# catree/InvCompCamTrack

Hardware: NVIDIA B200
Metric: GN pixel-residuals/s (higher is better)
Workload: dtype f32

## Files before the change

### __graft_entry__.py

```python
import os
import sys

ROOT = os.path.dirname(os.path.abspath(__file__))
if ROOT not in sys.path:
    sys.path.insert(0, ROOT)


def build():
    from invcompcamtrack_b200 import build as b
    b.build_library(force=bool(os.environ.get("ICT_FORCE_BUILD")))
    b.build_drivers()
    from oracle import oracle as O
    O.build("oracle")
    if os.path.isdir("/root/reference"):
        O.build("ref")
    import invcompcamtrack_b200 as ict
    ict.lib()


def smoke():
    import numpy as np
    import invcompcamtrack_b200 as ict
    sys.path.insert(0, os.path.join(ROOT, "tests"))
    from helpers import make_case, oracle_run, gpu_run, check_parity
    from oracle import oracle as O
    if ict.device_count() < 1:
        raise RuntimeError("smoke(): no CUDA device (libictrack has no CPU fallback)")
    ict.lib().ict_set_device(0)
    case = make_case(seed=7, w=320, h=240, psz=8, npts=100, lv_f=2)
    g = gpu_run(ict, case, sum_order=None)
    o = oracle_run(O.OracleLib(), case)
    for k in range(3):
        assert np.array_equal(g["pyr"][0][k], o["pyr"][0][k]), "pyramid differs from the oracle"
    assert np.array_equal(g["pt2d"], o["pt2d"]), "reference reprojection differs from the oracle"
    from helpers import assert_bit_identical
    assert_bit_identical(g, o)
    res = check_parity(g, o, case, min_same_iters=1.0, min_trans_ok=1.0)
    err = float(np.abs(g["p_out"][0] - case["p_gt"]).max())
    assert err < 5e-3, "tracker did not recover the ground-truth motion: %g" % err
    print("smoke ok:", res, "iters", g["iters"][0].tolist(), "err_vs_gt %.2e" % err, "launches", ict.launch_count())
    case32 = make_case(seed=8, w=640, h=384, psz=32, npts=4, lv_f=2, ntracks=8)
    o32 = oracle_run(O.OracleLib(), case32, trace_cap=40)
    gx = gpu_run(ict, case32, trace_cap=40, sum_order=None)
    assert_bit_identical(gx, o32)
    g32 = gpu_run(ict, case32, trace_cap=40, sum_order=0)
    r32 = check_parity(g32, o32, case32, gates=False)
    assert r32["jtr_first"] <= 1e-5, r32
    print("smoke psz32 ok: default kernel (K2r, reference order) bit-identical to the oracle on %d tracks; fast mode "
          "(K2v2) J^T r on identical inputs within %.1e of sum|sd*r| (gate 1e-5), %.0f%% identical iteration counts"
          % (case32["T"], r32["jtr_first"], 100 * r32["frac_same"]))


if __name__ == "__main__":
    build()
    if "--smoke" in sys.argv:
        smoke()
```

### invcompcamtrack_b200/build.py

```python
import os
import subprocess
import sys

HERE = os.path.dirname(os.path.abspath(__file__))
CSRC = os.path.join(HERE, "csrc")
LIB = os.path.join(HERE, "libictrack.so")
NVCC = os.environ.get("NVCC", "/usr/local/cuda/bin/nvcc")
NVCC_FLAGS = ["-gencode", "arch=compute_100a,code=sm_100a", "-lineinfo", "-O3", "-fmad=false", "-std=c++17",
              "-Xcompiler", "-fPIC", "-ccbin", "g++"] + os.environ.get("ICT_EXTRA_NVCC", "").split()
LIB_SOURCES = ["ict_kernels.cu", "ict_kernel_v2.cu", "ict_kernel_v8.cu", "ict_kernel_x.cu", "ict_kernel_x8.cu", "ict_kernel_r.cu", "ict_kernels_big.cu", "ict_hypotheses.cu", "ict_capi.cu"]
LIB_DEPS = LIB_SOURCES + ["ict_kernels.cuh", "ict_device.cuh", "ict_kernel_v2.cuh", "ict_kernel_v8.cuh", "ict_kernel_x.cuh", "ict_knobs.h", os.path.join("..", "..", "include", "ictrack.h")]


def _stale(target, deps):
    if not os.path.exists(target):
        return True
    t = os.path.getmtime(target)
    return any(os.path.getmtime(d) > t for d in deps if os.path.exists(d))


def build_library(force=False, verbose=False):
    deps = [os.path.join(CSRC, d) for d in LIB_DEPS]
    if not force and not _stale(LIB, deps):
        return LIB
    headers = [d for d in deps if not d.endswith(".cu")]
    objdir = os.path.join(HERE, "build")
    os.makedirs(objdir, exist_ok=True)
    jobs = []
    for src in LIB_SOURCES:
        obj = os.path.join(objdir, src.replace(".cu", ".o"))
        if force or _stale(obj, [os.path.join(CSRC, src)] + headers):
            cmd = [NVCC] + NVCC_FLAGS + (["-Xptxas=-v"] if verbose else []) + ["-c", os.path.join(CSRC, src), "-o", obj]
            jobs.append(cmd)
    if jobs:
        from concurrent.futures import ThreadPoolExecutor
        with ThreadPoolExecutor(max_workers=min(len(jobs), os.cpu_count() or 1)) as ex:
            for r in ex.map(lambda c: subprocess.run(c, capture_output=not verbose, text=True), jobs):
                if r.returncode:
                    raise RuntimeError("nvcc failed:\n%s\n%s" % (" ".join(r.args), (r.stderr or "")[-4000:]))
    objs = [os.path.join(objdir, src.replace(".cu", ".o")) for src in LIB_SOURCES]
    subprocess.run([NVCC, "-gencode", "arch=compute_100a,code=sm_100a", "-shared", "-o", LIB] + objs, check=True)
    return LIB


def build_drivers(force=False):
    host = os.path.join(CSRC, "host")
    out = []
    for name in ("run_track", "run_track_nposes"):
        src = os.path.join(host, name + ".cpp")
        if not os.path.exists(src):
            continue
        exe = os.path.join(HERE, "bin", name)
        deps = [src] + [os.path.join(host, f) for f in os.listdir(host)] + [LIB]
        if force or _stale(exe, deps):
            os.makedirs(os.path.dirname(exe), exist_ok=True)
            srcs = [src] + [os.path.join(host, f) for f in ("camera.cpp", "pose.cpp", "odometer.cpp", "utilities.cpp")]
            subprocess.run(["g++", "-O2", "-std=c++14", "-I", host, "-I", os.path.join(HERE, "..", "include"), "-o", exe]
                           + srcs + ["-L", HERE, "-lictrack", "-Wl,-rpath," + HERE, "-Wl,-rpath,$ORIGIN/.."], check=True)
        out.append(exe)
    return out


if __name__ == "__main__":
    force = "--force" in sys.argv
    print(build_library(force=force, verbose="-v" in sys.argv))
    for e in build_drivers(force=force):
        print(e)
```

### invcompcamtrack_b200/csrc/ict_capi.cu

```cuda
#include "ict_kernels.cuh"

#include <cuda.h>
#include <math.h>
#include <stdio.h>
#include <stdlib.h>
#include <string.h>
#include <string>
#include <vector>

using namespace ict;

static thread_local std::string g_err;
static int fail(int code, const std::string& msg) {
  g_err = msg;
  return code;
}
#define CU(expr)                                                                                       \
  do {                                                                                                 \
    cudaError_t _e = (expr);                                                                           \
    if (_e != cudaSuccess)                                                                             \
      return fail(ICT_ERR_CUDA, std::string(#expr) + ": " + cudaGetErrorString(_e));                   \
  } while (0)

static int require_device() {
  int n = 0;
  cudaError_t e = cudaGetDeviceCount(&n);
  if (e != cudaSuccess || n <= 0) {
    cudaGetLastError();
    return fail(ICT_ERR_NO_DEVICE, "no CUDA device: libictrack has no CPU fallback");
  }
  return ICT_OK;
}

struct DevBuf {
  void* p = nullptr;
  size_t cap = 0;
  cudaError_t reserve(size_t bytes) {
    if (bytes <= cap) return cudaSuccess;
    if (p) cudaFree(p);
    p = nullptr;
    cap = 0;
    cudaError_t e = cudaMalloc(&p, bytes);
    if (e == cudaSuccess) cap = bytes;
    return e;
  }
  void release() {
    if (p) cudaFree(p);
    p = nullptr;
    cap = 0;
  }
  template <typename T> T* as() const { return (T*)p; }
};

struct CopyLane {
  cudaStream_t s = nullptr;
  cudaEvent_t copied = nullptr, consumed = nullptr;
  bool have_consumed = false;
  cudaError_t begin() {
    cudaError_t e = cudaSuccess;
    if (!s) {
      e = cudaStreamCreateWithFlags(&s, cudaStreamNonBlocking);
      if (e == cudaSuccess) e = cudaEventCreateWithFlags(&copied, cudaEventDisableTiming);
      if (e == cudaSuccess) e = cudaEventCreateWithFlags(&consumed, cudaEventDisableTiming);
      if (e != cudaSuccess) return e;
    }
    if (have_consumed) e = cudaStreamWaitEvent(s, consumed, 0);
    return e;
  }
  cudaError_t publish(cudaStream_t user) {
    cudaError_t e = cudaEventRecord(copied, s);
    if (e == cudaSuccess) e = cudaStreamWaitEvent(user, copied, 0);
    return e;
  }
  cudaError_t done(cudaStream_t user) {
    if (!s) return cudaSuccess;
    cudaError_t e = cudaEventRecord(consumed, user);
    have_consumed = e == cudaSuccess;
    return e;
  }
  void release() {
    if (s) {
      cudaStreamSynchronize(s);
      cudaEventDestroy(copied);
      cudaEventDestroy(consumed);
      cudaStreamDestroy(s);
      s = nullptr;
    }
  }
};

extern "C" {

void ict_optparam_init(ict_optparam* op, int lv_f, int lv_l, int psz, int maxiter, float normdp_ratio, int donorm,
                       int dopatchnorm, int maxpttrack, int verbosity) {
  memset(op, 0, sizeof(*op));
  op->lv_f = lv_f;
  op->lv_l = lv_l;
  op->psz = psz;
  op->pszd2 = psz / 2;
  op->pszd2m3 = psz + op->pszd2 - 1;
  op->novals = psz * psz;
  op->maxiter = maxiter;
  op->normdp_ratio = normdp_ratio;
  op->donorm = donorm ? 1 : 0;
  op->dopatchnorm = dopatchnorm ? 1 : 0;
  const int r = maxpttrack % 4;
  op->maxpttrack = r > 0 ? maxpttrack + (4 - r) : maxpttrack;
  op->verbosity = verbosity;
}

int ict_version(void) { return ICT_VERSION; }
const char* ict_last_error(void) { return g_err.c_str(); }

int ict_device_count(void) {
  int n = 0;
  if (cudaGetDeviceCount(&n) != cudaSuccess) {
    cudaGetLastError();
    return 0;
  }
  return n;
}

int ict_set_device(int dev) {
  if (require_device()) return ICT_ERR_NO_DEVICE;
  CU(cudaSetDevice(dev));
  return ICT_OK;
}

int64_t ict_launch_count(int reset) { return launch_count(reset); }

int ict_camera_levels(int noscales, const float fc[2], const float cc[2], const int wh[2], int padding,
                      float* out) {
  if (noscales < 1 || noscales > ICT_MAX_LEVELS) return fail(ICT_ERR_BAD_ARG, "noscales out of range");
  for (int i = 0; i < noscales; ++i) {
    const float sc_fct = (float)(1 / pow(2, i));
    float* o = out + 8 * i;
    o[0] = sc_fct * fc[0];
    o[1] = sc_fct * fc[1];
    o[2] = sc_fct * cc[0];
    o[3] = sc_fct * cc[1];
    o[4] = sc_fct * (float)wh[0];
    o[5] = sc_fct * (float)wh[1];
    o[6] = o[4] + 2 * padding;
    o[7] = o[5] + 2 * padding;
  }
  return ICT_OK;
}

static void fill_cam(CamLevels& cam, int noscales, const float fc[2], const float cc[2], const int wh[2],
                     int padding) {
  float lv[8 * ICT_MAX_LEVELS];
  ict_camera_levels(noscales, fc, cc, wh, padding, lv);
  memset(&cam, 0, sizeof(cam));
  for (int l = 0; l < noscales; ++l) {
    cam.fx[l] = lv[8 * l + 0];
    cam.fy[l] = lv[8 * l + 1];
    cam.cx[l] = lv[8 * l + 2];
    cam.cy[l] = lv[8 * l + 3];
    cam.swo[l] = lv[8 * l + 4];
    cam.sho[l] = lv[8 * l + 5];
    cam.width[l] = (int)lv[8 * l + 6];
  }
}

int64_t ict_pyramid_layout(int w, int h, int lv_f, int pad, int64_t* level_off, int* sw, int* sh) {
  if (w <= 0 || h <= 0 || lv_f < 0 || lv_f >= ICT_MAX_LEVELS || pad < 0) return -1;
  if ((w % (1 << lv_f)) || (h % (1 << lv_f))) return -1;
  int64_t tot = 0;
  for (int l = 0; l <= lv_f; ++l) {
    const int a = (w >> l) + 2 * pad, b = (h >> l) + 2 * pad;
    if (level_off) level_off[l] = tot;
    if (sw) sw[l] = a;
    if (sh) sh[l] = b;
    tot += (int64_t)a * b;
  }
  return tot;
}

struct ict_frames {
  int nframes, w, h, lv_f, pad;
  int64_t plane_floats;
  int64_t level_off[ICT_MAX_LEVELS];
  int sw[ICT_MAX_LEVELS], sh[ICT_MAX_LEVELS];
  float *I, *dx, *dy;
  FrameDesc* desc;
  void* tmaps;
  bool tma_ok;
  DevBuf stage;
  CopyLane lane;
  bool view;
};

typedef CUresult (*ict_encode_tiled_fn)(CUtensorMap*, CUtensorMapDataType, cuuint32_t, void*, const cuuint64_t*,
                                        const cuuint64_t*, const cuuint32_t*, const cuuint32_t*, CUtensorMapInterleave,
                                        CUtensorMapSwizzle, CUtensorMapL2promotion, CUtensorMapFloatOOBfill);
static ict_encode_tiled_fn encode_tiled_fn() {
  static ict_encode_tiled_fn fn = nullptr;
  static bool tried = false;
  if (!tried) {
    tried = true;
    void* p = nullptr;
    cudaDriverEntryPointQueryResult qres;
    if (cudaGetDriverEntryPoint("cuTensorMapEncodeTiled", &p, cudaEnableDefault, &qres) == cudaSuccess &&
        qres == cudaDriverEntryPointSuccess)
      fn = (ict_encode_tiled_fn)p;
    else
      cudaGetLastError();
  }
  return fn;
}

#define ICT_TMA_BOX_W 40
#define ICT_TMA_BOX_H 17

static bool frames_make_tmaps(ict_frames* fs) {
  fs->tmaps = nullptr;
  fs->tma_ok = false;
  if (fs->pad != 32) return false;
  ict_encode_tiled_fn enc = encode_tiled_fn();
  if (!enc) return false;
  for (int l = 0; l <= fs->lv_f; ++l)
    if ((fs->sw[l] % 4) || (fs->level_off[l] % 4) || fs->sw[l] < ICT_TMA_BOX_W || fs->sh[l] < ICT_TMA_BOX_H) return false;
  if (fs->plane_floats % 4) return false;
  const size_t per_frame = 3 * ICT_MAX_LEVELS;
  std::vector<CUtensorMap> maps(per_frame * fs->nframes);
  memset(maps.data(), 0, sizeof(CUtensorMap) * maps.size());
  float* planes[3] = {fs->I, fs->dx, fs->dy};
  for (int f = 0; f < fs->nframes; ++f)
    for (int q = 0; q < 3; ++q)
      for (int l = 0; l <= fs->lv_f; ++l) {
        void* base = planes[q] + (size_t)f * fs->plane_floats + fs->level_off[l];
        const cuuint64_t dims[2] = {(cuuint64_t)fs->sw[l], (cuuint64_t)fs->sh[l]};
        const cuuint64_t strides[1] = {(cuuint64_t)fs->sw[l] * sizeof(float)};
        const cuuint32_t box[2] = {ICT_TMA_BOX_W, ICT_TMA_BOX_H};
        const cuuint32_t estr[2] = {1, 1};
        if (enc(&maps[(f * 3 + q) * ICT_MAX_LEVELS + l], CU_TENSOR_MAP_DATA_TYPE_FLOAT32, 2, base, dims, strides, box, estr,
                CU_TENSOR_MAP_INTERLEAVE_NONE, CU_TENSOR_MAP_SWIZZLE_NONE, CU_TENSOR_MAP_L2_PROMOTION_NONE,
                CU_TENSOR_MAP_FLOAT_OOB_FILL_NONE) != CUDA_SUCCESS)
          return false;
      }
  if (cudaMalloc(&fs->tmaps, sizeof(CUtensorMap) * maps.size()) != cudaSuccess) {
    cudaGetLastError();
    fs->tmaps = nullptr;
    return false;
  }
  if (cudaMemcpy(fs->tmaps, maps.data(), sizeof(CUtensorMap) * maps.size(), cudaMemcpyHostToDevice) != cudaSuccess) {
    cudaFree(fs->tmaps);
    fs->tmaps = nullptr;
    return false;
  }
  fs->tma_ok = true;
  return true;
}

ict_frames* ict_frames_create(int nframes, int w, int h, int lv_f, int pad) {
  if (require_device()) return nullptr;
  ict_frames* fs = new ict_frames();
  fs->nframes = nframes; fs->w = w; fs->h = h; fs->lv_f = lv_f; fs->pad = pad;
  fs->I = fs->dx = fs->dy = nullptr;
  fs->desc = nullptr;
  fs->tmaps = nullptr;
  fs->tma_ok = false;
  fs->view = false;
  fs->plane_floats = ict_pyramid_layout(w, h, lv_f, pad, fs->level_off, fs->sw, fs->sh);
  if (fs->plane_floats < 0 || nframes <= 0) {
    fail(ICT_ERR_BAD_ARG, "ict_frames_create: w,h must be divisible by 2^lv_f, nframes > 0");
    delete fs;
    return nullptr;
  }
  const size_t bytes = sizeof(float) * (size_t)fs->plane_floats * nframes;
  if (cudaMalloc(&fs->I, bytes) != cudaSuccess || cudaMalloc(&fs->dx, bytes) != cudaSuccess ||
      cudaMalloc(&fs->dy, bytes) != cudaSuccess || cudaMalloc(&fs->desc, sizeof(FrameDesc) * nframes) != cudaSuccess) {
    fail(ICT_ERR_NOMEM, "ict_frames_create: cudaMalloc failed");
    cudaGetLastError();
    ict_frames_destroy(fs);
    return nullptr;
  }
  frames_make_tmaps(fs);
  std::vector<FrameDesc> d(nframes);
  for (int f = 0; f < nframes; ++f) {
    memset(&d[f], 0, sizeof(FrameDesc));
    d[f].tmap = fs->tmaps ? (const char*)fs->tmaps + sizeof(CUtensorMap) * 3 * ICT_MAX_LEVELS * (size_t)f : nullptr;
    for (int l = 0; l <= lv_f; ++l) {
      d[f].I[l] = fs->I + (size_t)f * fs->plane_floats + fs->level_off[l];
      d[f].dx[l] = fs->dx + (size_t)f * fs->plane_floats + fs->level_off[l];
      d[f].dy[l] = fs->dy + (size_t)f * fs->plane_floats + fs->level_off[l];
    }
  }
  if (cudaMemcpy(fs->desc, d.data(), sizeof(FrameDesc) * nframes, cudaMemcpyHostToDevice) != cudaSuccess) {
    fail(ICT_ERR_CUDA, "ict_frames_create: descriptor upload failed");
    ict_frames_destroy(fs);
    return nullptr;
  }
  return fs;
}

void ict_frames_destroy(ict_frames* fs) {
  if (!fs) return;
  if (fs->I) cudaFree(fs->I);
  if (fs->dx) cudaFree(fs->dx);
  if (fs->dy) cudaFree(fs->dy);
  if (fs->desc) cudaFree(fs->desc);
  if (fs->tmaps) cudaFree(fs->tmaps);
  fs->stage.release();
  fs->lane.release();
  delete fs;
}

ict_frames* ict_frames_create_view(int nframes, int w, int h, int lv_f, int pad) {
  if (require_device()) return nullptr;
  ict_frames* fs = new ict_frames();
  fs->nframes = nframes; fs->w = w; fs->h = h; fs->lv_f = lv_f; fs->pad = pad;
  fs->I = fs->dx = fs->dy = nullptr;
  fs->desc = nullptr;
  fs->tmaps = nullptr;
  fs->tma_ok = true;
  fs->view = true;
  fs->plane_floats = ict_pyramid_layout(w, h, lv_f, pad, fs->level_off, fs->sw, fs->sh);
  if (fs->plane_floats < 0 || nframes <= 0 || cudaMalloc(&fs->desc, sizeof(FrameDesc) * nframes) != cudaSuccess) {
    fail(ICT_ERR_BAD_ARG, "ict_frames_create_view: bad geometry or allocation failure");
    cudaGetLastError();
    delete fs;
    return nullptr;
  }
  cudaMemset(fs->desc, 0, sizeof(FrameDesc) * nframes);
  return fs;
}

int ict_frames_alias(ict_frames* view, int idx, const ict_frames* src, int src_idx) {
  if (!view || !src || !view->view) return fail(ICT_ERR_BAD_ARG, "ict_frames_alias: first argument must be a view store");
  if (idx < 0 || idx >= view->nframes || src_idx < 0 || src_idx >= src->nframes)
    return fail(ICT_ERR_BAD_ARG, "ict_frames_alias: index out of range");
  if (view->w != src->w || view->h != src->h || view->lv_f != src->lv_f || view->pad != src->pad)
    return fail(ICT_ERR_BAD_ARG, "ict_frames_alias: geometry mismatch");
  CU(cudaMemcpyAsync(view->desc + idx, src->desc + src_idx, sizeof(FrameDesc), cudaMemcpyDeviceToDevice, 0));
  view->tma_ok = view->tma_ok && src->tma_ok;
  return ICT_OK;
}

static int frames_range_ok(const ict_frames* fs, int first, int count) {
  if (!fs) return fail(ICT_ERR_BAD_ARG, "null frame store");
  if (first < 0 || count < 0 || first + count > fs->nframes) return fail(ICT_ERR_BAD_ARG, "frame range out of bounds");
  return ICT_OK;
}

static int frames_build(ict_frames* fs, int first, int count, const float* f32, const unsigned char* u8,
                        cudaStream_t st) {
  if (fs->view) return fail(ICT_ERR_BAD_ARG, "a view store owns no pixels: build into the store it aliases");
  CU(launch_pyramid(f32, u8, count, fs->w, fs->h, fs->lv_f, fs->pad, fs->I + (size_t)first * fs->plane_floats,
                    fs->dx + (size_t)first * fs->plane_floats, fs->dy + (size_t)first * fs->plane_floats,
                    fs->plane_floats, fs->level_off, st));
  return ICT_OK;
}

int ict_frames_build_dev(ict_frames* fs, int first, int count, const float* imgs_dev, void* stream) {
  if (frames_range_ok(fs, first, count)) return ICT_ERR_BAD_ARG;
  return frames_build(fs, first, count, imgs_dev, nullptr, (cudaStream_t)stream);
}
int ict_frames_build_dev_u8(ict_frames* fs, int first, int count, const unsigned char* imgs_dev, void* stream) {
  if (frames_range_ok(fs, first, count)) return ICT_ERR_BAD_ARG;
  return frames_build(fs, first, count, nullptr, imgs_dev, (cudaStream_t)stream);
}

int ict_frames_upload(ict_frames* fs, int first, int count, const float* imgs) {
  if (frames_range_ok(fs, first, count)) return ICT_ERR_BAD_ARG;
  const size_t bytes = sizeof(float) * (size_t)fs->w * fs->h * count;
  CU(fs->stage.reserve(bytes));
  CU(cudaMemcpyAsync(fs->stage.p, imgs, bytes, cudaMemcpyHostToDevice, 0));
  return frames_build(fs, first, count, fs->stage.as<float>(), nullptr, 0);
}
int ict_frames_upload_u8(ict_frames* fs, int first, int count, const unsigned char* imgs) {
  if (frames_range_ok(fs, first, count)) return ICT_ERR_BAD_ARG;
  const size_t bytes = (size_t)fs->w * fs->h * count;
  CU(fs->stage.reserve(bytes));
  CU(cudaMemcpyAsync(fs->stage.p, imgs, bytes, cudaMemcpyHostToDevice, 0));
  return frames_build(fs, first, count, nullptr, fs->stage.as<unsigned char>(), 0);
}

int ict_frames_upload_planes(ict_frames* fs, int frame, const float* I, const float* dx, const float* dy) {
  if (frames_range_ok(fs, frame, 1)) return ICT_ERR_BAD_ARG;
  if (fs->view || !I) return fail(ICT_ERR_BAD_ARG, "ict_frames_upload_planes: needs an owning store and an intensity plane set");
  const size_t bytes = sizeof(float) * (size_t)fs->plane_floats, o = (size_t)frame * fs->plane_floats;
  CU(cudaMemcpyAsync(fs->I + o, I, bytes, cudaMemcpyHostToDevice, 0));
  if (dx) CU(cudaMemcpyAsync(fs->dx + o, dx, bytes, cudaMemcpyHostToDevice, 0));
  if (dy) CU(cudaMemcpyAsync(fs->dy + o, dy, bytes, cudaMemcpyHostToDevice, 0));
  CU(cudaStreamSynchronize(0));
  return ICT_OK;
}

int ict_frames_upload_u8_stream(ict_frames* fs, int first, int count, const unsigned char* imgs, void* stream) {
  if (frames_range_ok(fs, first, count)) return ICT_ERR_BAD_ARG;
  cudaStream_t st = (cudaStream_t)stream;
  const size_t per = (size_t)fs->w * fs->h;
  if (fs->stage.cap < per * fs->nframes) {
    CU(cudaDeviceSynchronize());
    CU(fs->stage.reserve(per * fs->nframes));
  }
  unsigned char* dst = fs->stage.as<unsigned char>() + per * first;
  CU(fs->lane.begin());
  CU(cudaMemcpyAsync(dst, imgs, per * count, cudaMemcpyHostToDevice, fs->lane.s));
  CU(fs->lane.publish(st));
  const int rc = frames_build(fs, first, count, nullptr, dst, st);
  if (rc) return rc;
  CU(fs->lane.done(st));
  return ICT_OK;
}

int ict_frames_download(ict_frames* fs, int frame, float* out_I, float* out_dx, float* out_dy) {
  if (frames_range_ok(fs, frame, 1)) return ICT_ERR_BAD_ARG;
  if (fs->view) return fail(ICT_ERR_BAD_ARG, "ict_frames_download: a view store owns no pixels");
  const size_t bytes = sizeof(float) * (size_t)fs->plane_floats, o = (size_t)frame * fs->plane_floats;
  if (out_I) CU(cudaMemcpy(out_I, fs->I + o, bytes, cudaMemcpyDeviceToHost));
  if (out_dx) CU(cudaMemcpy(out_dx, fs->dx + o, bytes, cudaMemcpyDeviceToHost));
  if (out_dy) CU(cudaMemcpy(out_dy, fs->dy + o, bytes, cudaMemcpyDeviceToHost));
  return ICT_OK;
}

int ict_pyramid_build(const float* img, int w, int h, int lv_f, int pad, float* out_I, float* out_dx,
                      float* out_dy) {
  if (require_device()) return ICT_ERR_NO_DEVICE;
  ict_frames* fs = ict_frames_create(1, w, h, lv_f, pad);
  if (!fs) return ICT_ERR_BAD_ARG;
  int rc = ict_frames_upload(fs, 0, 1, img);
  if (rc == ICT_OK) rc = ict_frames_download(fs, 0, out_I, out_dx, out_dy);
  ict_frames_destroy(fs);
  return rc;
}

struct ict_tracker {
  ict_optparam op;
  CamLevels cam;
  float fc[2], cc[2];
  int wh[2];
  int T = 0;
  int64_t total = 0;
  int max_pts = 0;
  std::vector<int64_t> h_off;
  bool have_2d = false;
  int sum_mode = 1;
  int eigen_packet = 4;
  int force_general = 0;
  int knob_no_k2r = 0, knob_seq_launches = 0;
  unsigned robust = 0;
  int keep_state = 0;
  bool state_valid = false;
  int seq_n = 0, seq_step = 0;
  const int *big_rf = nullptr, *big_nf = nullptr;
  DevBuf pt_off, pts, pt3d, norm, p_in, p_out, iters, npix, trace, pt2d, rf, nf, big, teacher, state;
  int teacher_cap = 0;
  static const int ICT_BIG_LANES = 4;
  cudaStream_t big_st[ICT_BIG_LANES] = {};
  cudaEvent_t big_ev[ICT_BIG_LANES + 1] = {};
  DevBuf big_lane[ICT_BIG_LANES];
  CopyLane lane;
  CopyLane lane_in;
};

static bool optparam_ok(const ict_optparam* op) {
  return op && op->psz >= 1 && op->lv_f >= op->lv_l && op->lv_l >= 0 && op->lv_f < ICT_MAX_LEVELS && op->maxpttrack >= 1 &&
         op->maxiter >= 0;
}

ict_tracker* ict_tracker_create(const ict_optparam* op, const float fc[2], const float cc[2], const int wh[2]) {
  if (require_device()) return nullptr;
  if (!optparam_ok(op) || !fc || !cc || !wh) {
    fail(ICT_ERR_BAD_ARG, "ict_tracker_create: bad optparam");
    return nullptr;
  }
  ict_tracker* tr = new ict_tracker();
  tr->op = *op;
  memcpy(tr->fc, fc, sizeof(tr->fc));
  memcpy(tr->cc, cc, sizeof(tr->cc));
  memcpy(tr->wh, wh, sizeof(tr->wh));
  fill_cam(tr->cam, op->lv_f + 1, fc, cc, wh, op->psz);
  return tr;
}

void ict_tracker_destroy(ict_tracker* tr) {
  if (!tr) return;
  DevBuf* b[] = {&tr->pt_off, &tr->pts, &tr->pt3d, &tr->norm, &tr->p_in, &tr->p_out, &tr->iters,
                 &tr->npix, &tr->trace, &tr->pt2d, &tr->rf, &tr->nf, &tr->big, &tr->teacher, &tr->state};
  for (DevBuf* x : b) x->release();
  for (int k = 0; k < ict_tracker::ICT_BIG_LANES; ++k) {
    tr->big_lane[k].release();
    if (tr->big_st[k]) cudaStreamDestroy(tr->big_st[k]);
  }
  for (int k = 0; k <= ict_tracker::ICT_BIG_LANES; ++k)
    if (tr->big_ev[k]) cudaEventDestroy(tr->big_ev[k]);
  tr->lane.release();
  tr->lane_in.release();
  delete tr;
}

int ict_tracker_set_optparam(ict_tracker* tr, const ict_optparam* op) {
  if (!tr || !op) return fail(ICT_ERR_BAD_ARG, "null argument");
  if (op->psz != tr->op.psz || op->lv_f != tr->op.lv_f)
    return fail(ICT_ERR_BAD_ARG, "psz and lv_f are fixed at creation (they size the camera and the pyramids)");
  if (!optparam_ok(op)) return fail(ICT_ERR_BAD_ARG, "ict_tracker_set_optparam: bad optparam (lv_l, maxpttrack or maxiter out of range)");
  tr->op = *op;
  tr->op.pszd2 = op->psz / 2;
  tr->op.pszd2m3 = op->psz + op->psz / 2 - 1;
  tr->op.novals = op->psz * op->psz;
  return ICT_OK;
}

int ict_tracker_set_teacher(ict_tracker* tr, const float* poses, int trace_cap) {
  if (!tr) return fail(ICT_ERR_BAD_ARG, "null argument");
  if (!poses || trace_cap <= 0) {
    tr->teacher_cap = 0;
    return ICT_OK;
  }
  if (tr->T <= 0) return fail(ICT_ERR_BAD_ARG, "no points set");
  const size_t bytes = sizeof(float) * 8 * (size_t)tr->T * trace_cap;
  CU(tr->teacher.reserve(bytes));
  CU(cudaMemcpy(tr->teacher.p, poses, bytes, cudaMemcpyHostToDevice));
  tr->teacher_cap = trace_cap;
  return ICT_OK;
}

int ict_tracker_set_robust(ict_tracker* tr, unsigned flags) {
  if (!tr || (flags & ~(ICT_ROBUST_FULL_STEP | ICT_ROBUST_COMPOSE | ICT_ROBUST_FLOOR)))
    return fail(ICT_ERR_BAD_ARG, "ict_tracker_set_robust: unknown flag");
  tr->robust = flags;
  return ICT_OK;
}

int ict_tracker_set_knob(ict_tracker* tr, const char* name, int value) {
  if (!tr || !name) return fail(ICT_ERR_BAD_ARG, "null argument");
  if (!strcmp(name, "no_k2r")) tr->knob_no_k2r = value ? 1 : 0;
  else if (!strcmp(name, "seq_launches")) tr->knob_seq_launches = value ? 1 : 0;
  else if (!strcmp(name, "keep_state")) { tr->keep_state = value ? 1 : 0; tr->state_valid = false; }
  else return fail(ICT_ERR_BAD_ARG, std::string("unknown knob: ") + name);
  return ICT_OK;
}

int ict_tracker_set_sum_order(ict_tracker* tr, int mode) {
  if (!tr || mode < 0 || mode > 3)
    return fail(ICT_ERR_BAD_ARG, "sum order must be 1 (reference order, 4-float packets, default), 3 (reference order, "
                                 "8-float packets), 0 (fast tree order) or 2");
  tr->sum_mode = (mode == 1 || mode == 3) ? 1 : 0;
  tr->eigen_packet = mode == 3 ? 8 : 4;
  tr->force_general = mode == 2 ? 1 : 0;
  return ICT_OK;
}

static int tracker_reserve(ict_tracker* tr, int T, int64_t total) {
  CU(tr->pt_off.reserve(sizeof(int64_t) * (size_t)(T + 1)));
  CU(tr->pt3d.reserve(sizeof(float) * 3 * (size_t)(total ? total : 1)));
  CU(tr->norm.reserve(sizeof(double) * 4 * (size_t)T));
  CU(tr->pt2d.reserve(sizeof(float) * 2 * (size_t)(total ? total : 1)));
  return ICT_OK;
}

int ict_tracker_set_points(ict_tracker* tr, int T, const int64_t* pt_off, double* pts, int mutate_caller) {
  if (!tr || T <= 0 || !pt_off || !pts) return fail(ICT_ERR_BAD_ARG, "ict_tracker_set_points: bad argument");
  const int64_t total = pt_off[T];
  int max_pts = 0;
  for (int t = 0; t < T; ++t) {
    const int64_t n = pt_off[t + 1] - pt_off[t];
    if (n < 0 || n > 0x7fffffff) return fail(ICT_ERR_BAD_ARG, "pt_off must be non-decreasing");
    if (n > max_pts) max_pts = (int)n;
  }
  if (tracker_reserve(tr, T, total)) return ICT_ERR_CUDA;
  CU(tr->pts.reserve(sizeof(double) * 3 * (size_t)(total ? total : 1)));
  CU(cudaMemcpyAsync(tr->pt_off.p, pt_off, sizeof(int64_t) * (size_t)(T + 1), cudaMemcpyHostToDevice, 0));
  CU(cudaMemcpyAsync(tr->pts.p, pts, sizeof(double) * 3 * (size_t)total, cudaMemcpyHostToDevice, 0));
  const bool mut = mutate_caller && tr->op.donorm;
  CU(launch_set_points(T, tr->pt_off.as<int64_t>(), tr->pts.as<double>(), mut ? tr->pts.as<double>() : nullptr,
                       tr->pt3d.as<float>(), tr->norm.as<double>(), tr->op.donorm, tr->op.maxpttrack, max_pts, 0));
  if (mut) CU(cudaMemcpy(pts, tr->pts.p, sizeof(double) * 3 * (size_t)total, cudaMemcpyDeviceToHost));
  tr->T = T;
  tr->total = total;
  tr->max_pts = max_pts;
  tr->h_off.assign(pt_off, pt_off + T + 1);
  tr->have_2d = false;
  tr->state_valid = false;
  return ICT_OK;
}

int ict_tracker_set_points_stream(ict_tracker* tr, int T, const int64_t* pt_off, const double* pts, void* stream) {
  if (!tr || T <= 0 || !pt_off || !pts) return fail(ICT_ERR_BAD_ARG, "ict_tracker_set_points_stream: bad argument");
  cudaStream_t st = (cudaStream_t)stream;
  const int64_t total = pt_off[T];
  int max_pts = 0;
  for (int t = 0; t < T; ++t) {
    const int64_t n = pt_off[t + 1] - pt_off[t];
    if (n < 0 || n > 0x7fffffff) return fail(ICT_ERR_BAD_ARG, "pt_off must be non-decreasing");
    if (n > max_pts) max_pts = (int)n;
  }
  if (tracker_reserve(tr, T, total)) return ICT_ERR_CUDA;
  CU(tr->pts.reserve(sizeof(double) * 3 * (size_t)(total ? total : 1)));
  CU(tr->lane.begin());
  CU(cudaMemcpyAsync(tr->pt_off.p, pt_off, sizeof(int64_t) * (size_t)(T + 1), cudaMemcpyHostToDevice, tr->lane.s));
  CU(cudaMemcpyAsync(tr->pts.p, pts, sizeof(double) * 3 * (size_t)total, cudaMemcpyHostToDevice, tr->lane.s));
  CU(tr->lane.publish(st));
  CU(launch_set_points(T, tr->pt_off.as<int64_t>(), tr->pts.as<double>(), nullptr, tr->pt3d.as<float>(),
                       tr->norm.as<double>(), tr->op.donorm, tr->op.maxpttrack, max_pts, st));
  CU(tr->lane.done(st));
  tr->T = T;
  tr->total = total;
  tr->max_pts = max_pts;
  tr->h_off.assign(pt_off, pt_off + T + 1);
  tr->have_2d = false;
  tr->state_valid = false;
  return ICT_OK;
}

int ict_tracker_set_points_dev(ict_tracker* tr, int T, const int64_t* pt_off_dev, const double* pts_dev,
                               int64_t total_pts, int max_pts, void* stream) {
  if (!tr || T <= 0 || !pt_off_dev || !pts_dev || max_pts <= 0)
    return fail(ICT_ERR_BAD_ARG, "ict_tracker_set_points_dev: bad argument");
  cudaStream_t st = (cudaStream_t)stream;
  if (tracker_reserve(tr, T, total_pts)) return ICT_ERR_CUDA;
  CU(cudaMemcpyAsync(tr->pt_off.p, pt_off_dev, sizeof(int64_t) * (size_t)(T + 1), cudaMemcpyDeviceToDevice, st));
  CU(launch_set_points(T, tr->pt_off.as<int64_t>(), pts_dev, nullptr, tr->pt3d.as<float>(), tr->norm.as<double>(),
                       tr->op.donorm, tr->op.maxpttrack, max_pts, st));
  tr->T = T;
  tr->total = total_pts;
  tr->max_pts = max_pts;
  tr->h_off.clear();
  tr->have_2d = false;
  tr->state_valid = false;
  return ICT_OK;
}

static int run_tracks(ict_tracker* tr, const ict_frames* fs, const int* rf_dev, const int* nf_dev, int fixed_ref,
                      int fixed_new, const double* p_in_dev, double* p_out_dev, int* iters_dev, float* trace_dev,
                      int trace_cap, long long* npix_dev, cudaStream_t st) {
  if (!tr || !fs) return fail(ICT_ERR_BAD_ARG, "null tracker / frame store");
  if (tr->T <= 0) return fail(ICT_ERR_BAD_ARG, "no points set: call ict_tracker_set_points first");
  if (fs->lv_f != tr->op.lv_f || fs->pad != tr->op.psz || fs->w != tr->wh[0] || fs->h != tr->wh[1])
    return fail(ICT_ERR_BAD_ARG, "frame store does not match the tracker (need lv_f, pad == psz, w, h equal)");
  if (!rf_dev && (fixed_ref < 0 || fixed_ref >= fs->nframes || fixed_new < 0 || fixed_new >= fs->nframes))
    return fail(ICT_ERR_BAD_ARG, "frame index out of range");
  TrackParams prm;
  memset(&prm, 0, sizeof(prm));
  prm.op = tr->op;
  prm.cam = tr->cam;
  prm.frames = fs->desc;
  prm.ref_frame = rf_dev;
  prm.new_frame = nf_dev;
  prm.fixed_ref = fixed_ref;
  prm.fixed_new = fixed_new;
  prm.pt_off = tr->pt_off.as<int64_t>();
  prm.pt3d = tr->pt3d.as<float>();
  prm.norm = tr->norm.as<double>();
  prm.p_in = p_in_dev;
  prm.p_out = p_out_dev;
  prm.iters = iters_dev;
  prm.trace = trace_dev;
  prm.trace_cap = trace_cap;
  prm.teacher = (trace_dev && tr->teacher_cap > 0 && tr->teacher_cap == trace_cap) ? tr->teacher.as<float>() : nullptr;
  prm.npixres = npix_dev;
  prm.pt2d_out = tr->pt2d.as<float>();
  prm.T = tr->T;
  prm.t0 = 0;
  prm.sum_mode = tr->sum_mode;
  prm.eigen_packet = tr->eigen_packet;
  prm.tma_ok = fs->tma_ok ? 1 : 0;
  prm.force_general = tr->force_general;
  prm.seq_n = tr->seq_n;
  prm.seq_step = tr->seq_step;
  prm.knob_no_k2r = tr->knob_no_k2r;
  prm.knob_seq_launches = tr->knob_seq_launches;
  prm.robust = tr->robust;
  if (tr->robust && !(tr->sum_mode == 0 && !tr->force_general && v8_supported(tr->op, tr->max_pts)))
    return fail(ICT_ERR_UNSUPPORTED, "robustness modes need the fast mode (sum order 0), psz 8 and at most 240 points per track");
  if (tr->keep_state) {
    if (!(tr->sum_mode == 1 && !tr->force_general && tr->op.psz == 8 && kx8_supported(tr->op, tr->max_pts)))
      return fail(ICT_ERR_UNSUPPORTED, "keep_state needs the reference summation order, psz 8 and at most 224 points per track");
    const int P = tr->max_pts < tr->op.maxpttrack ? tr->max_pts : tr->op.maxpttrack;
    prm.state_stride = (int64_t)(3 * 64 + 12) * P;
    const size_t bytes = sizeof(float) * (size_t)prm.state_stride * tr->T;
    if (tr->state.cap < bytes) tr->state_valid = false;
    CU(tr->state.reserve(bytes));
    prm.state = tr->state.as<float>();
    prm.state_load = tr->state_valid ? 1 : 0;
  }
  prm.dbg_skip_serial = ict_knob("ICT_DBG_SKIP_SERIAL") ? atoi(ict_knob("ICT_DBG_SKIP_SERIAL")) : 0;
  prm.serial_warp_last = ict_knob("ICT_SERIAL_WARP_LAST") ? 1 : 0;
  prm.v2_lu_setup = ict_knob("ICT_V2_LU") ? 1 : 0;
  if (track_fits_one_cta(tr->op, tr->max_pts, tr->sum_mode, tr->force_general)) {
    CU(launch_track(prm, tr->max_pts, st));
  } else {
    if (tr->h_off.empty()) return fail(ICT_ERR_UNSUPPORTED, "big tracks need host-side pt_off (use ict_tracker_set_points)");
    if (rf_dev) return fail(ICT_ERR_UNSUPPORTED, "big tracks take fixed ref/new frames (use ict_track_sequence or T=1)");
    size_t wb = 0;
    for (int t = 0; t < tr->T; ++t) {
      const size_t w = bigtrack_work_bytes(tr->op, tr->h_off[t + 1] - tr->h_off[t], tr->eigen_packet);
      wb = w > wb ? w : wb;
    }
    int nl = tr->T < ict_tracker::ICT_BIG_LANES ? tr->T : ict_tracker::ICT_BIG_LANES;
    while (nl > 1 && wb * (size_t)nl > ((size_t)2 << 30)) --nl;
    if (nl <= 1) {
      CU(tr->big.reserve(wb));
      for (int t = 0; t < tr->T; ++t) {
        const int64_t n = tr->h_off[t + 1] - tr->h_off[t];
        if (tr->big_rf) { prm.fixed_ref = tr->big_rf[t]; prm.fixed_new = tr->big_nf[t]; }
        CU(launch_track_big(prm, t, n, tr->big.p, st));
      }
    } else {
      for (int k = 0; k < nl; ++k) {
        if (!tr->big_st[k]) CU(cudaStreamCreateWithFlags(&tr->big_st[k], cudaStreamNonBlocking));
        CU(tr->big_lane[k].reserve(wb));
      }
      for (int k = 0; k <= nl; ++k)
        if (!tr->big_ev[k]) CU(cudaEventCreateWithFlags(&tr->big_ev[k], cudaEventDisableTiming));
      CU(cudaEventRecord(tr->big_ev[nl], st));
      for (int k = 0; k < nl; ++k) CU(cudaStreamWaitEvent(tr->big_st[k], tr->big_ev[nl], 0));
      for (int t = 0; t < tr->T; ++t) {
        const int k = t % nl;
        const int64_t n = tr->h_off[t + 1] - tr->h_off[t];
        if (tr->big_rf) { prm.fixed_ref = tr->big_rf[t]; prm.fixed_new = tr->big_nf[t]; }
        CU(launch_track_big(prm, t, n, tr->big_lane[k].p, tr->big_st[k]));
      }
      for (int k = 0; k < nl; ++k) {
        CU(cudaEventRecord(tr->big_ev[k], tr->big_st[k]));
        CU(cudaStreamWaitEvent(st, tr->big_ev[k], 0));
      }
    }
  }
  tr->have_2d = true;
  if (tr->keep_state) tr->state_valid = true;
  return ICT_OK;
}

int ict_track_batch_dev(ict_tracker* tr, const ict_frames* fs, const int* ref_frame_dev, const int* new_frame_dev,
                        const double* p_in_dev, double* p_out_dev, int* iters_dev, float* trace_dev, int trace_cap,
                        int64_t* npixres_dev, void* stream) {
  if (!ref_frame_dev || !new_frame_dev || !p_in_dev || !p_out_dev) return fail(ICT_ERR_BAD_ARG, "null device pointer");
  return run_tracks(tr, fs, ref_frame_dev, new_frame_dev, -1, -1, p_in_dev, p_out_dev, iters_dev, trace_dev,
                    trace_dev ? trace_cap : 0, (long long*)npixres_dev, (cudaStream_t)stream);
}

int ict_track_batch(ict_tracker* tr, const ict_frames* fs, const int* ref_frame, const int* new_frame,
                    const double* p_in, double* p_out, int* iters, float* trace, int trace_cap, int64_t* npixres) {
  if (!tr || !fs || !ref_frame || !new_frame || !p_in || !p_out) return fail(ICT_ERR_BAD_ARG, "null argument");
  const int T = tr->T;
  if (T <= 0) return fail(ICT_ERR_BAD_ARG, "no points set");
  const int L = tr->op.lv_f - tr->op.lv_l + 1;
  for (int t = 0; t < T; ++t)
    if (ref_frame[t] < 0 || ref_frame[t] >= fs->nframes || new_frame[t] < 0 || new_frame[t] >= fs->nframes)
      return fail(ICT_ERR_BAD_ARG, "frame index out of range");
  CU(tr->rf.reserve(sizeof(int) * (size_t)T));
  CU(tr->nf.reserve(sizeof(int) * (size_t)T));
  CU(tr->p_in.reserve(sizeof(double) * 6 * (size_t)T));
  CU(tr->p_out.reserve(sizeof(double) * 6 * (size_t)T));
  CU(tr->iters.reserve(sizeof(int) * (size_t)T * L));
  CU(tr->npix.reserve(sizeof(long long) * (size_t)T));
  if (trace && trace_cap > 0) CU(tr->trace.reserve(sizeof(float) * ICT_TRACE_FLOATS * (size_t)T * trace_cap));
  CU(cudaMemcpyAsync(tr->rf.p, ref_frame, sizeof(int) * (size_t)T, cudaMemcpyHostToDevice, 0));
  CU(cudaMemcpyAsync(tr->nf.p, new_frame, sizeof(int) * (size_t)T, cudaMemcpyHostToDevice, 0));
  CU(cudaMemcpyAsync(tr->p_in.p, p_in, sizeof(double) * 6 * (size_t)T, cudaMemcpyHostToDevice, 0));
  const bool big = !track_fits_one_cta(tr->op, tr->max_pts, tr->sum_mode, tr->force_general);
  int rc;
  if (big) {
    tr->big_rf = ref_frame;
    tr->big_nf = new_frame;
    rc = run_tracks(tr, fs, nullptr, nullptr, ref_frame[0], new_frame[0], tr->p_in.as<double>(), tr->p_out.as<double>(),
                    tr->iters.as<int>(), trace && trace_cap > 0 ? tr->trace.as<float>() : nullptr, trace_cap,
                    tr->npix.as<long long>(), 0);
    tr->big_rf = tr->big_nf = nullptr;
  } else {
    rc = run_tracks(tr, fs, tr->rf.as<int>(), tr->nf.as<int>(), -1, -1, tr->p_in.as<double>(), tr->p_out.as<double>(),
                    tr->iters.as<int>(), trace && trace_cap > 0 ? tr->trace.as<float>() : nullptr, trace_cap,
                    tr->npix.as<long long>(), 0);
  }
  if (rc) return rc;
  CU(cudaMemcpyAsync(p_out, tr->p_out.p, sizeof(double) * 6 * (size_t)T, cudaMemcpyDeviceToHost, 0));
  if (iters) CU(cudaMemcpyAsync(iters, tr->iters.p, sizeof(int) * (size_t)T * L, cudaMemcpyDeviceToHost, 0));
  if (npixres) CU(cudaMemcpyAsync(npixres, tr->npix.p, sizeof(long long) * (size_t)T, cudaMemcpyDeviceToHost, 0));
  if (trace && trace_cap > 0)
    CU(cudaMemcpyAsync(trace, tr->trace.p, sizeof(float) * ICT_TRACE_FLOATS * (size_t)T * trace_cap,
                       cudaMemcpyDeviceToHost, 0));
  CU(cudaStreamSynchronize(0));
  return ICT_OK;
}

int ict_track_batch_stream(ict_tracker* tr, const ict_frames* fs, const int* ref_frame, const int* new_frame,
                           const double* p_in, double* p_out, int* iters, int64_t* npixres, void* stream) {
  if (!tr || !fs || !ref_frame || !new_frame || !p_in || !p_out) return fail(ICT_ERR_BAD_ARG, "null argument");
  cudaStream_t st = (cudaStream_t)stream;
  const int T = tr->T;
  if (T <= 0) return fail(ICT_ERR_BAD_ARG, "no points set");
  if (!track_fits_one_cta(tr->op, tr->max_pts, tr->sum_mode, tr->force_general))
    return fail(ICT_ERR_UNSUPPORTED, "stream variant handles tracks that fit one CTA");
  for (int t = 0; t < T; ++t)
    if (ref_frame[t] < 0 || ref_frame[t] >= fs->nframes || new_frame[t] < 0 || new_frame[t] >= fs->nframes)
      return fail(ICT_ERR_BAD_ARG, "frame index out of range");
  const int L = tr->op.lv_f - tr->op.lv_l + 1;
  CU(tr->rf.reserve(sizeof(int) * (size_t)T));
  CU(tr->nf.reserve(sizeof(int) * (size_t)T));
  CU(tr->p_in.reserve(sizeof(double) * 6 * (size_t)T));
  CU(tr->p_out.reserve(sizeof(double) * 6 * (size_t)T));
  CU(tr->iters.reserve(sizeof(int) * (size_t)T * L));
  CU(tr->npix.reserve(sizeof(long long) * (size_t)T));
  CU(tr->lane_in.begin());
  CU(cudaMemcpyAsync(tr->rf.p, ref_frame, sizeof(int) * (size_t)T, cudaMemcpyHostToDevice, tr->lane_in.s));
  CU(cudaMemcpyAsync(tr->nf.p, new_frame, sizeof(int) * (size_t)T, cudaMemcpyHostToDevice, tr->lane_in.s));
  CU(cudaMemcpyAsync(tr->p_in.p, p_in, sizeof(double) * 6 * (size_t)T, cudaMemcpyHostToDevice, tr->lane_in.s));
  CU(tr->lane_in.publish(st));
  const int rc = run_tracks(tr, fs, tr->rf.as<int>(), tr->nf.as<int>(), -1, -1, tr->p_in.as<double>(),
                            tr->p_out.as<double>(), tr->iters.as<int>(), nullptr, 0, tr->npix.as<long long>(), st);
  if (rc) return rc;
  CU(tr->lane.done(st));
  CU(tr->lane_in.done(st));
  CU(cudaMemcpyAsync(p_out, tr->p_out.p, sizeof(double) * 6 * (size_t)T, cudaMemcpyDeviceToHost, st));
  if (iters) CU(cudaMemcpyAsync(iters, tr->iters.p, sizeof(int) * (size_t)T * L, cudaMemcpyDeviceToHost, st));
  if (npixres) CU(cudaMemcpyAsync(npixres, tr->npix.p, sizeof(long long) * (size_t)T, cudaMemcpyDeviceToHost, st));
  return ICT_OK;
}

int ict_track_sequence(ict_tracker* tr, const ict_frames* fs, int first, int nsteps, int step, const double* p_in,
                       double* poses_out, int* iters, int64_t* npixres) {
  if (!tr || !fs || !p_in || !poses_out || nsteps < 0 || (step != 1 && step != -1))
    return fail(ICT_ERR_BAD_ARG, "ict_track_sequence: bad argument");
  const int T = tr->T;
  if (T <= 0) return fail(ICT_ERR_BAD_ARG, "no points set");
  const int L = tr->op.lv_f - tr->op.lv_l + 1;
  const int last = first + nsteps * step;
  if (first < 0 || first >= fs->nframes || last < 0 || last >= fs->nframes)
    return fail(ICT_ERR_BAD_ARG, "frame range out of bounds");
  CU(tr->p_out.reserve(sizeof(double) * 6 * (size_t)T * (nsteps + 1)));
  CU(tr->iters.reserve(sizeof(int) * (size_t)T * L * (nsteps ? nsteps : 1)));
  CU(tr->npix.reserve(sizeof(long long) * (size_t)T * (nsteps ? nsteps : 1)));
  double* chain = tr->p_out.as<double>();
  CU(cudaMemcpyAsync(chain, p_in, sizeof(double) * 6 * (size_t)T, cudaMemcpyHostToDevice, 0));
  if (nsteps > 1 && track_chain_in_one_launch(tr->op, tr->max_pts, tr->sum_mode, tr->force_general, tr->knob_seq_launches)) {
    tr->seq_n = nsteps;
    tr->seq_step = step;
    int rc = run_tracks(tr, fs, nullptr, nullptr, first, first + step, chain, chain + (size_t)6 * T, tr->iters.as<int>(),
                        nullptr, 0, tr->npix.as<long long>(), 0);
    tr->seq_n = tr->seq_step = 0;
    if (rc) return rc;
  } else {
    for (int k = 0; k < nsteps; ++k) {
      const int fr = first + k * step;
      int rc = run_tracks(tr, fs, nullptr, nullptr, fr, fr + step, chain + (size_t)k * 6 * T,
                          chain + (size_t)(k + 1) * 6 * T, tr->iters.as<int>() + (size_t)k * T * L, nullptr, 0,
                          tr->npix.as<long long>() + (size_t)k * T, 0);
      if (rc) return rc;
    }
  }
  CU(cudaMemcpyAsync(poses_out, chain, sizeof(double) * 6 * (size_t)T * (nsteps + 1), cudaMemcpyDeviceToHost, 0));
  if (iters && nsteps)
    CU(cudaMemcpyAsync(iters, tr->iters.p, sizeof(int) * (size_t)T * L * nsteps, cudaMemcpyDeviceToHost, 0));
  if (npixres && nsteps)
    CU(cudaMemcpyAsync(npixres, tr->npix.p, sizeof(long long) * (size_t)T * nsteps, cudaMemcpyDeviceToHost, 0));
  CU(cudaStreamSynchronize(0));
  return ICT_OK;
}

int ict_tracker_reproject(ict_tracker* tr, const double* p_in, float* pt2d_out) {
  if (!tr || !p_in) return fail(ICT_ERR_BAD_ARG, "null argument");
  if (tr->T <= 0) return fail(ICT_ERR_BAD_ARG, "no points set");
  CU(tr->p_in.reserve(sizeof(double) * 6 * (size_t)tr->T));
  CU(cudaMemcpyAsync(tr->p_in.p, p_in, sizeof(double) * 6 * (size_t)tr->T, cudaMemcpyHostToDevice, 0));
  TrackParams prm;
  memset(&prm, 0, sizeof(prm));
  prm.op = tr->op;
  prm.cam = tr->cam;
  prm.pt_off = tr->pt_off.as<int64_t>();
  prm.pt3d = tr->pt3d.as<float>();
  prm.norm = tr->norm.as<double>();
  prm.p_in = tr->p_in.as<double>();
  prm.pt2d_out = tr->pt2d.as<float>();
  prm.T = tr->T;
  CU(launch_reproject(prm, 0));
  tr->have_2d = true;
  if (pt2d_out) CU(cudaMemcpy(pt2d_out, tr->pt2d.p, sizeof(float) * 2 * (size_t)tr->total, cudaMemcpyDeviceToHost));
  return ICT_OK;
}

int ict_tracker_get_2dpoints(ict_tracker* tr, float* out) {
  if (!tr || !out) return fail(ICT_ERR_BAD_ARG, "null argument");
  if (!tr->have_2d) return fail(ICT_ERR_BAD_ARG, "no SetPose has run yet");
  CU(cudaMemcpy(out, tr->pt2d.p, sizeof(float) * 2 * (size_t)tr->total, cudaMemcpyDeviceToHost));
  return ICT_OK;
}

int ict_track_pair(const ict_optparam* op, const float fc[2], const float cc[2], const int wh[2], const float* imgA,
                   const float* imgB, double* pt3d, int npts, const double p_in[6], double p_out[6], int* iters,
                   float* trace, int trace_cap) {
  if (require_device()) return ICT_ERR_NO_DEVICE;
  if (!op || !imgA || !imgB || !pt3d || npts <= 0) return fail(ICT_ERR_BAD_ARG, "ict_track_pair: bad argument");
  ict_frames* fs = ict_frames_create(2, wh[0], wh[1], op->lv_f, op->psz);
  if (!fs) return ICT_ERR_BAD_ARG;
  ict_tracker* tr = ict_tracker_create(op, fc, cc, wh);
  int rc = tr ? ICT_OK : ICT_ERR_BAD_ARG;
  if (rc == ICT_OK) rc = ict_frames_upload(fs, 0, 1, imgA);
  if (rc == ICT_OK) rc = ict_frames_upload(fs, 1, 1, imgB);
  const int64_t off[2] = {0, npts};
  if (rc == ICT_OK) rc = ict_tracker_set_points(tr, 1, off, pt3d, 1);
  const int rf = 0, nf = 1;
  if (rc == ICT_OK) rc = ict_track_batch(tr, fs, &rf, &nf, p_in, p_out, iters, trace, trace_cap, nullptr);
  ict_tracker_destroy(tr);
  ict_frames_destroy(fs);
  return rc;
}

int ict_pose_hypotheses(const float fc[2], const float cc[2], int npts, const double* pt2d, const double* pt3d, int nsamples,
                        const int* sample_idx, const double p_init[6], double inlthresh, int maxiter, double* out_pose,
                        int* out_status, int* out_ninl, unsigned char* out_inlmask) {
  if (require_device()) return ICT_ERR_NO_DEVICE;
  if (!fc || !cc || !pt2d || !pt3d || !sample_idx || !p_init || !out_pose || !out_status || npts < 4 || nsamples < 0 ||
      !(inlthresh > 0) || maxiter < 1)
    return fail(ICT_ERR_BAD_ARG, "ict_pose_hypotheses: bad argument");
  if (nsamples == 0) return ICT_OK;
  DevBuf d2, d3, ds, dp, dst, dn, dm;
  cudaError_t e = d2.reserve(sizeof(double) * 2 * npts);
  if (e == cudaSuccess) e = d3.reserve(sizeof(double) * 3 * npts);
  if (e == cudaSuccess) e = ds.reserve(sizeof(int) * 4 * (size_t)nsamples);
  if (e == cudaSuccess) e = dp.reserve(sizeof(double) * 6 * (size_t)nsamples);
  if (e == cudaSuccess) e = dst.reserve(sizeof(int) * (size_t)nsamples);
  if (e == cudaSuccess) e = dn.reserve(sizeof(int) * (size_t)nsamples);
  if (e == cudaSuccess) e = dm.reserve((size_t)nsamples * npts);
  if (e == cudaSuccess) e = cudaMemcpyAsync(d2.p, pt2d, sizeof(double) * 2 * npts, cudaMemcpyHostToDevice, 0);
  if (e == cudaSuccess) e = cudaMemcpyAsync(d3.p, pt3d, sizeof(double) * 3 * npts, cudaMemcpyHostToDevice, 0);
  if (e == cudaSuccess) e = cudaMemcpyAsync(ds.p, sample_idx, sizeof(int) * 4 * (size_t)nsamples, cudaMemcpyHostToDevice, 0);
  const double fcd[2] = {fc[0], fc[1]}, ccd[2] = {cc[0], cc[1]};
  if (e == cudaSuccess)
    e = launch_hypotheses(fcd, ccd, npts, d2.as<double>(), d3.as<double>(), nsamples, ds.as<int>(), p_init, inlthresh, maxiter,
                          dp.as<double>(), dst.as<int>(), dn.as<int>(), dm.as<unsigned char>(), 0);
  if (e == cudaSuccess) e = cudaMemcpyAsync(out_pose, dp.p, sizeof(double) * 6 * (size_t)nsamples, cudaMemcpyDeviceToHost, 0);
  if (e == cudaSuccess) e = cudaMemcpyAsync(out_status, dst.p, sizeof(int) * (size_t)nsamples, cudaMemcpyDeviceToHost, 0);
  if (e == cudaSuccess && out_ninl) e = cudaMemcpyAsync(out_ninl, dn.p, sizeof(int) * (size_t)nsamples, cudaMemcpyDeviceToHost, 0);
  if (e == cudaSuccess && out_inlmask) e = cudaMemcpyAsync(out_inlmask, dm.p, (size_t)nsamples * npts, cudaMemcpyDeviceToHost, 0);
  if (e == cudaSuccess) e = cudaStreamSynchronize(0);
  int rc = ICT_OK;
  if (e != cudaSuccess) rc = fail(ICT_ERR_CUDA, std::string("ict_pose_hypotheses: ") + cudaGetErrorString(e));
  DevBuf* all[] = {&d2, &d3, &ds, &dp, &dst, &dn, &dm};
  for (DevBuf* b : all) b->release();
  return rc;
}

int ict_get_patches(const ict_frames* fs, int frame, int level, const ict_optparam* op, int npatch, const float* mids,
                    float* out_I, float* out_dx, float* out_dy) {
  if (!fs || !op || !mids || npatch < 0) return fail(ICT_ERR_BAD_ARG, "ict_get_patches: null argument");
  if (frames_range_ok(fs, frame, 1)) return ICT_ERR_BAD_ARG;
  if (fs->view || !fs->I) return fail(ICT_ERR_BAD_ARG, "ict_get_patches: needs a store that owns its pixels (not a view)");
  if (level < 0 || level > fs->lv_f) return fail(ICT_ERR_BAD_ARG, "ict_get_patches: level out of range");
  if (op->psz < 1 || op->psz > fs->pad) return fail(ICT_ERR_BAD_ARG, "ict_get_patches: psz must be 1..padding of the store");
  if (npatch == 0) return ICT_OK;
  const float swo = (float)(fs->sw[level] - 2 * fs->pad), sho = (float)(fs->sh[level] - 2 * fs->pad);
  for (int i = 0; i < npatch; ++i)
    if (!(mids[2 * i] >= 0 && mids[2 * i + 1] >= 0 && mids[2 * i] <= swo && mids[2 * i + 1] <= sho))
      return fail(ICT_ERR_BAD_ARG, "ict_get_patches: a centre lies outside [0, swo] x [0, sho] of the level");
  const size_t n = (size_t)op->psz * op->psz, tot = n * npatch;
  DevBuf dm, dout;
  cudaError_t e = dm.reserve(sizeof(float) * 2 * npatch);
  if (e == cudaSuccess) e = dout.reserve(sizeof(float) * 3 * tot);
  float* o = dout.as<float>();
  if (e == cudaSuccess) e = cudaMemcpyAsync(dm.p, mids, sizeof(float) * 2 * npatch, cudaMemcpyHostToDevice, 0);
  const size_t po = (size_t)frame * fs->plane_floats + fs->level_off[level];
  if (e == cudaSuccess)
    e = launch_get_patches(fs->I + po, fs->dx + po, fs->dy + po, fs->sw[level], op->psz, op->psz / 2, op->dopatchnorm ? 1 : 0,
                           npatch, dm.as<float>(), out_I ? o : nullptr, out_dx ? o + tot : nullptr, out_dy ? o + 2 * tot : nullptr, 0);
  if (e == cudaSuccess && out_I) e = cudaMemcpyAsync(out_I, o, sizeof(float) * tot, cudaMemcpyDeviceToHost, 0);
  if (e == cudaSuccess && out_dx) e = cudaMemcpyAsync(out_dx, o + tot, sizeof(float) * tot, cudaMemcpyDeviceToHost, 0);
  if (e == cudaSuccess && out_dy) e = cudaMemcpyAsync(out_dy, o + 2 * tot, sizeof(float) * tot, cudaMemcpyDeviceToHost, 0);
  if (e == cudaSuccess) e = cudaStreamSynchronize(0);
  int rc = ICT_OK;
  if (e != cudaSuccess) rc = fail(ICT_ERR_CUDA, std::string("ict_get_patches: ") + cudaGetErrorString(e));
  dm.release();
  dout.release();
  return rc;
}

int ict_ncc_score(ict_tracker* tr, const ict_frames* fs, int frame_b, int frame_r, int frame_f, int nback, int nfwd,
                  const float* pt2d_back, const float* pt2d_refe, const float* pt2d_forw, float* out_corr) {
  if (!tr || !fs || !pt2d_back || !pt2d_refe || !pt2d_forw || !out_corr) return fail(ICT_ERR_BAD_ARG, "null argument");
  if (tr->T <= 0 || tr->h_off.empty()) return fail(ICT_ERR_BAD_ARG, "no points set");
  if (fs->view || !fs->I) return fail(ICT_ERR_BAD_ARG, "ict_ncc_score: needs a store that owns its pixels (not a view)");
  if (fs->lv_f != tr->op.lv_f || fs->pad != tr->op.psz || fs->w != tr->wh[0] || fs->h != tr->wh[1])
    return fail(ICT_ERR_BAD_ARG, "frame store does not match the tracker (need lv_f, pad == psz, w, h equal)");
  if (nback < 0 || nfwd < 0 || nback + nfwd == 0) return fail(ICT_ERR_BAD_ARG, "ict_ncc_score: nback + nfwd must be positive");
  if (frames_range_ok(fs, frame_b, 1) || frames_range_ok(fs, frame_r, 1) || frames_range_ok(fs, frame_f, 1))
    return ICT_ERR_BAD_ARG;
  const size_t total = (size_t)tr->total;
  DevBuf in, out;
  int rc = ICT_OK;
  cudaError_t e = in.reserve(sizeof(float) * 6 * total);
  if (e == cudaSuccess) e = out.reserve(sizeof(float) * total);
  float* d = in.as<float>();
  if (e == cudaSuccess) e = cudaMemcpyAsync(d, pt2d_back, sizeof(float) * 2 * total, cudaMemcpyHostToDevice, 0);
  if (e == cudaSuccess) e = cudaMemcpyAsync(d + 2 * total, pt2d_refe, sizeof(float) * 2 * total, cudaMemcpyHostToDevice, 0);
  if (e == cudaSuccess) e = cudaMemcpyAsync(d + 4 * total, pt2d_forw, sizeof(float) * 2 * total, cudaMemcpyHostToDevice, 0);
  const int l = tr->op.lv_l;
  const size_t fo = (size_t)fs->plane_floats;
  if (e == cudaSuccess)
    e = launch_ncc(tr->op, tr->cam, fs->I + frame_b * fo + fs->level_off[l], fs->I + frame_r * fo + fs->level_off[l],
                   fs->I + frame_f * fo + fs->level_off[l], nback, nfwd, tr->pt_off.as<int64_t>(), tr->T, d, d + 2 * total,
                   d + 4 * total, out.as<float>(), 0);
  if (e == cudaSuccess) e = cudaMemcpy(out_corr, out.p, sizeof(float) * total, cudaMemcpyDeviceToHost);
  if (e != cudaSuccess) rc = fail(ICT_ERR_CUDA, std::string("ict_ncc_score: ") + cudaGetErrorString(e));
  in.release();
  out.release();
  return rc;
}

}
```

### invcompcamtrack_b200/csrc/ict_kernel_r.cu

```cuda
#include <cuda.h>

#include "ict_kernels.cuh"
#include "ict_device.cuh"
#include "ict_kernel_x.cuh"

namespace ict {

void count_launch_external();

#define KR_WROW 40
#define KR_WIN_BYTES (17 * KR_WROW * 4)
#define KR_SLOT_BYTES 2816
#define KR_NSLOT 5

#define KR_MAXU 16
#define KR_SD_BYTES_PER_POINT (6 * 1024 * 4)

__device__ __forceinline__ void tma_load_2d(void* dst, const void* tmap, int x, int y, unsigned long long* bar) {
  asm volatile(
      "cp.async.bulk.tensor.2d.shared::cluster.global.tile.mbarrier::complete_tx::bytes [%0], [%1, {%2, %3}], [%4];" ::"r"(
          ict_saddr(dst)),
      "l"(tmap), "r"(x), "r"(y), "r"(ict_saddr(bar))
      : "memory");
}
__device__ __forceinline__ void mbar_expect_tx_only(unsigned long long* b, unsigned bytes) {
  asm volatile("mbarrier.expect_tx.relaxed.cta.shared::cta.b64 [%0], %1;" ::"r"(ict_saddr(b)), "r"(bytes) : "memory");
}
__device__ __forceinline__ void mbar_wait_backoff(unsigned long long* b, unsigned parity) {
  unsigned done = 0;
  for (int tries = 0;; ++tries) {
    asm volatile(
        "{\n"
        ".reg .pred P1;\n"
        "mbarrier.try_wait.parity.shared::cta.b64 P1, [%1], %2;\n"
        "selp.u32 %0, 1, 0, P1;\n"
        "}\n"
        : "=r"(done)
        : "r"(ict_saddr(b)), "r"(parity)
        : "memory");
    if (done) break;
    if (tries >= 4) __nanosleep(40);
  }
}
__device__ __forceinline__ void fence_proxy_async() { asm volatile("fence.proxy.async.shared::cta;" ::: "memory"); }
__device__ __forceinline__ void tmap_acquire(const void* tmap) {
  asm volatile("fence.proxy.tensormap::generic.acquire.sys [%0], 128;" ::"l"(tmap) : "memory");
}

struct __align__(16) KrShared {
  unsigned long long win_full[KR_MAXU];
  unsigned long long slot_free[KR_MAXU];
  unsigned long long gat_full[2];
  unsigned pd_flag[KR_MAXU];
  unsigned b_flag;
  unsigned pad_[3];
  float G[12];
  float p[8];
  float sum[8];
  float dp[8];
  float Hsum[24];
  Lu6 f;
  float4 npl[8];
  float4 rpl[8];
  int nx[8], ny[8], nvis[8];
  int rx[8], ry[8], rvis[8];
  float X[8], Y[8], Z[8], Xc[8], Yc[8], Zc[8];
  int cont[2], it, nv;
};

__device__ __forceinline__ void kr_patch_place(float mx, float my, int* x0, int* y0, float4* w) {
  const int pos0 = (int)ceilf(mx + .00001f);
  const int pos1 = (int)ceilf(my + .00001f);
  const int pos2 = (int)floorf(mx);
  const int pos3 = (int)floorf(my);
  const float r0 = mx - (float)pos2;
  const float r1 = my - (float)pos3;
  w->x = r0 * r1;
  w->y = (1 - r0) * r1;
  w->z = r0 * (1 - r1);
  w->w = (1 - r0) * (1 - r1);
  *x0 = pos0 + 16;
  *y0 = pos1 + 16;
}

__device__ __forceinline__ void kr_sample16(const float* win, int lane, const float4 w, float* out) {
  float a0 = win[lane + 1], b0 = win[lane];
#pragma unroll
  for (int r = 0; r < 16; ++r) {
    const float a1 = win[(r + 1) * KR_WROW + lane + 1], b1 = win[(r + 1) * KR_WROW + lane];
    out[r] = ((w.x * a1 + w.y * b1) + w.z * a0) + w.w * b0;
    a0 = a1;
    b0 = b1;
  }
}

__device__ __forceinline__ unsigned ld_acquire_s(const unsigned* p) {
  unsigned v;
  asm volatile("ld.acquire.cta.shared.u32 %0, [%1];" : "=r"(v) : "r"(ict_saddr(p)) : "memory");
  return v;
}
__device__ __forceinline__ void st_release_s(unsigned* p, unsigned v) {
  asm volatile("st.release.cta.shared.u32 [%0], %1;" ::"r"(ict_saddr(p)), "r"(v) : "memory");
}

struct KrRows8 {
  float4 v[8];
};
__device__ __forceinline__ float4 lds128v(const float4* p) {
  float4 v;
  asm volatile("ld.shared.v4.f32 {%0, %1, %2, %3}, [%4];" : "=f"(v.x), "=f"(v.y), "=f"(v.z), "=f"(v.w) : "r"(ict_saddr(p)));
  return v;
}
struct KrLoad8 {
  float4 a[8], b[8];
};
__device__ __forceinline__ void kr_load8(const float4* a4, int astride, const float4* b4, int bstride, KrLoad8& o) {
#pragma unroll
  for (int r = 0; r < 8; ++r) { o.a[r] = lds128v(a4 + r * astride); o.b[r] = lds128v(b4 + r * bstride); }
}
__device__ __forceinline__ void kr_mul8(const KrLoad8& l, KrRows8& o) {
#pragma unroll
  for (int r = 0; r < 8; ++r)
    o.v[r] = make_float4(l.a[r].x * l.b[r].x, l.a[r].y * l.b[r].y, l.a[r].z * l.b[r].z, l.a[r].w * l.b[r].w);
}
__device__ __forceinline__ void kr_add8(const KrRows8& p, float& acc) {
#pragma unroll
  for (int r = 0; r < 8; ++r) {
    acc = acc + p.v[r].x;
    acc = acc + p.v[r].y;
    acc = acc + p.v[r].z;
    acc = acc + p.v[r].w;
  }
}

template <int NPROD, int UPP>
__global__ void __launch_bounds__((NPROD + 2) * 32, NPROD == 4 ? 2 : 1) k_track_r(const TrackParams prm) {
  extern __shared__ unsigned char smem_raw[];
  const int t = blockIdx.x + prm.t0;
  const ict_optparam& op = prm.op;
  const int tid = threadIdx.x, nt = blockDim.x, lane = tid & 31, warp = tid >> 5;
  const int64_t off = prm.pt_off[t];
  const int n_in = (int)(prm.pt_off[t + 1] - off);
  const int P = min(n_in, op.maxpttrack);
  const int U = 2 * P;
  const bool donorm = op.donorm != 0;

  unsigned char* base = smem_raw + ((128u - (ict_saddr(smem_raw) & 127u)) & 127u);
  float* s_sd = reinterpret_cast<float*>(base);
  const int Pcap = prm.r_pcap;
  unsigned char* s_slots = base + (size_t)Pcap * KR_SD_BYTES_PER_POINT;
  KrShared& S = *reinterpret_cast<KrShared*>(s_slots + KR_NSLOT * KR_SLOT_BYTES);
  float(*s_AB)[12] = reinterpret_cast<float(*)[12]>(s_slots);

  const int rf = prm.ref_frame ? prm.ref_frame[t] : prm.fixed_ref;
  const int nf = prm.new_frame ? prm.new_frame[t] : prm.fixed_new;
  const char* tm_ref = reinterpret_cast<const char*>(prm.frames[rf].tmap);
  const char* tm_new = reinterpret_cast<const char*>(prm.frames[nf].tmap);
  const bool chainA = warp == 0, prod = warp >= 2;
  const int pw = warp - 2;

  {
    const float4 z4 = make_float4(0.f, 0.f, 0.f, 0.f);
    float4* sd4 = reinterpret_cast<float4*>(s_sd);
    for (int e = tid; e < P * (KR_SD_BYTES_PER_POINT / 16); e += nt) sd4[e] = z4;
    const float* q = prm.pt3d + 3 * off;
    for (int i = tid; i < P; i += nt) {
      S.X[i] = q[i];
      S.Y[i] = q[n_in + i];
      S.Z[i] = q[2 * (int64_t)n_in + i];
    }
  }
  if (tid == 0)
    setpose_se3(prm.p_in + 6 * (int64_t)t, donorm, prm.norm + 4 * (int64_t)t, prm.norm[4 * (int64_t)t + 3], S.p, S.G);
  if (tid >= 32 && tid < 32 + KR_MAXU) {
    mbar_init(&S.win_full[tid - 32], 1);
    S.pd_flag[tid - 32] = 0u;
    mbar_init(&S.slot_free[tid - 32], 2);

  }
  if (tid == 64) {
    mbar_init(&S.gat_full[0], 1);
    mbar_init(&S.gat_full[1], 1);
    S.b_flag = 0u;

  }
  mbar_fence_init();
  __syncthreads();
  for (int i = tid; i < P; i += nt) {
    const float X = S.X[i], Y = S.Y[i], Z = S.Z[i];
    const float xc = S.G[0] * X + S.G[1] * Y + S.G[2] * Z + S.G[3];
    const float yc = S.G[4] * X + S.G[5] * Y + S.G[6] * Z + S.G[7];
    const float zc = S.G[8] * X + S.G[9] * Y + S.G[10] * Z + S.G[11];
    S.Xc[i] = xc;
    S.Yc[i] = yc;
    S.Zc[i] = zc;
    if (prm.pt2d_out) {
      const int l = op.lv_l;
      prm.pt2d_out[2 * off + i] = (xc / zc) * prm.cam.fx[l] + prm.cam.cx[l];
      prm.pt2d_out[2 * off + n_in + i] = (yc / zc) * prm.cam.fy[l] + prm.cam.cy[l];
    }
  }
  __syncthreads();

  float* trace = prm.trace ? prm.trace + (int64_t)t * prm.trace_cap * ICT_TRACE_FLOATS : nullptr;
  int trace_n = 0;
  float normdp_init = 1e-10f;
  int nvsum = 0;
  unsigned gi = 0;
  unsigned lvl = 0;
  float refv[UPP][16];
#pragma unroll
  for (int s = 0; s < UPP; ++s)
#pragma unroll
    for (int r = 0; r < 16; ++r) refv[s][r] = 0.0f;
  const int perm = 4 * (lane & 7) + (lane >> 3);

  for (int sl = op.lv_f; sl >= op.lv_l; --sl, ++lvl) {
    const float fx = prm.cam.fx[sl], fy = prm.cam.fy[sl], cx = prm.cam.cx[sl], cy = prm.cam.cy[sl];
    const float swo = prm.cam.swo[sl], sho = prm.cam.sho[sl];
    const void* tmI = tm_ref + 128 * (0 * ICT_MAX_LEVELS + sl);
    const void* tmDx = tm_ref + 128 * (1 * ICT_MAX_LEVELS + sl);
    const void* tmDy = tm_ref + 128 * (2 * ICT_MAX_LEVELS + sl);
    const void* tmN = tm_new + 128 * (0 * ICT_MAX_LEVELS + sl);

    long long lt0 = 0, lt1 = 0, lt2 = 0, lt3 = 0, lt4 = 0;
    if (chainA && trace) lt0 = clock64();
    if (warp == 0) {
      tmap_acquire(tmI);
      tmap_acquire(tmDx);
      tmap_acquire(tmDy);
      tmap_acquire(tmN);
    } else if (prod && lane == 0) {
      tmap_acquire(tmN);
    }

    auto place_and_issue = [&]() {
      int v = 0;
      if (lane < P) {
        const float X = S.X[lane], Y = S.Y[lane], Z = S.Z[lane];
        const float tx = S.G[0] * X + S.G[1] * Y + S.G[2] * Z + S.G[3];
        const float ty = S.G[4] * X + S.G[5] * Y + S.G[6] * Z + S.G[7];
        const float tz = S.G[8] * X + S.G[9] * Y + S.G[10] * Z + S.G[11];
        const float mx = (tx / tz) * fx + cx, my = (ty / tz) * fy + cy;
        v = (mx >= 0) & (my >= 0) & (mx <= swo) & (my <= sho);
        int x0 = 0, y0 = 0;
        float4 w = make_float4(0.f, 0.f, 0.f, 0.f);
        if (v) kr_patch_place(mx, my, &x0, &y0, &w);
        S.npl[lane] = w;
        S.nx[lane] = x0;
        S.ny[lane] = y0;
        S.nvis[lane] = v;
      }
      const int nv = __popc(__ballot_sync(0xffffffffu, v));
      if (lane == 0) S.nv = nv;
      __syncwarp();
      if (lane < U && lane < KR_NSLOT) {
        const int pp = lane >> 1, half = lane & 1;
        if (S.nvis[pp]) {
          fence_proxy_async();
          mbar_expect_tx(&S.win_full[lane], KR_WIN_BYTES);
          tma_load_2d(s_slots + lane * KR_SLOT_BYTES, tmN, (S.nx[pp] - 1) & ~3, S.ny[pp] - 1 + 16 * half, &S.win_full[lane]);
        } else {
          mbar_arrive(&S.win_full[lane]);
        }
      }
    };

    if (tid < P) {
      const int i = tid;
      const float xc = S.Xc[i], yc = S.Yc[i], zc = S.Zc[i];
      const float mx = (xc / zc) * fx + cx, my = (yc / zc) * fy + cy;
      const int vis = (mx >= 0) & (my >= 0) & (mx <= swo) & (my <= sho);
      int x0 = 0, y0 = 0;
      float4 w = make_float4(0.f, 0.f, 0.f, 0.f);
      if (vis) {
        kr_patch_place(mx, my, &x0, &y0, &w);
        float c[10];
        sd_coefs(xc, yc, zc, fx, fy, c);
        float* ab = s_AB[i];
        ab[0] = c[0]; ab[1] = 0.0f; ab[2] = c[2]; ab[3] = c[4]; ab[4] = c[6]; ab[5] = c[8];
        ab[6] = 0.0f; ab[7] = c[1]; ab[8] = c[3]; ab[9] = c[5]; ab[10] = c[7]; ab[11] = c[9];
      }
      S.rpl[i] = w;
      S.rx[i] = x0;
      S.ry[i] = y0;
      S.rvis[i] = vis;
    }
    fence_proxy_async();
    __syncthreads();
    if (warp == 0) {
      if (lane < U && S.rvis[lane >> 1]) {
        const int pp = lane >> 1, half = lane & 1;
        unsigned char* dst = reinterpret_cast<unsigned char*>(s_sd) + (size_t)pp * KR_SD_BYTES_PER_POINT + half * 3 * KR_SLOT_BYTES;
        const int x = (S.rx[pp] - 1) & ~3, y = S.ry[pp] - 1 + 16 * half;
        fence_proxy_async();
        unsigned long long* bar = &S.gat_full[pp >> 2];
        mbar_expect_tx_only(bar, 3u * KR_WIN_BYTES);
        tma_load_2d(dst, tmI, x, y, bar);
        tma_load_2d(dst + KR_SLOT_BYTES, tmDx, x, y, bar);
        tma_load_2d(dst + 2 * KR_SLOT_BYTES, tmDy, x, y, bar);
      }
      __syncwarp();
      if (lane < 2) mbar_arrive(&S.gat_full[lane]);
    }
    if (chainA && trace) lt1 = clock64();
    float gx[UPP][16], gy[UPP][16];
    if (prod) {
      mbar_wait(&S.gat_full[0], lvl & 1);
      mbar_wait(&S.gat_full[1], lvl & 1);
#pragma unroll
      for (int s = 0; s < UPP; ++s) {
        const int u = pw + NPROD * s;
        if (u < U && S.rvis[u >> 1]) {
          const int pp = u >> 1, half = u & 1;
          const float* win = s_sd + (size_t)pp * (KR_SD_BYTES_PER_POINT / 4) + half * 3 * (KR_SLOT_BYTES / 4) +
                             ((S.rx[pp] - 1) & 3);
          const float4 w = S.rpl[pp];
          kr_sample16(win, lane, w, refv[s]);
          kr_sample16(win + KR_SLOT_BYTES / 4, lane, w, gx[s]);
          kr_sample16(win + 2 * (KR_SLOT_BYTES / 4), lane, w, gy[s]);
        }
      }
    }
    __syncthreads();
    if (prod) {
#pragma unroll
      for (int s = 0; s < UPP; ++s) {
        const int u = pw + NPROD * s;
        if (u < U && S.rvis[u >> 1]) {
          const int pp = u >> 1, half = u & 1;
          float ab[12];
#pragma unroll
          for (int k = 0; k < 12; ++k) ab[k] = s_AB[pp][k];
          float* dst = s_sd + (size_t)pp * 6 * 1024 + half * 16 * 32 + perm;
#pragma unroll
          for (int r = 0; r < 16; ++r) {
            float sd[6];
            kx_sd(gx[s][r], gy[s][r], ab, sd);
#pragma unroll
            for (int k = 0; k < 6; ++k) dst[k * 1024 + r * 32] = sd[k];
          }
        }
      }
    }
    __syncthreads();

    if (chainA && trace) lt2 = clock64();
    if (warp < 3) {
      const int c = lane & 7, g = min(lane >> 3, 2);
      auto qidx = [](int a, int b) { return a * 6 - (a * (a - 1)) / 2 + (b - a); };
      const float4* sd4 = reinterpret_cast<const float4*>(s_sd) + c;
      if (warp == 0) {
        const int px = 2 * g, py = 2 * g + 1;
        const float4* X4 = sd4 + px * 256;
        const float4* Y4 = sd4 + py * 256;
        float a1 = -0.0f, a2 = -0.0f, a3 = -0.0f;
        for (int i = 0; i < P; ++i) {
#pragma unroll 8
          for (int r = 0; r < 32; ++r) {
            const float4 x = X4[i * 1536 + r * 8], y = Y4[i * 1536 + r * 8];
            a1 = a1 + x.x * x.x; a2 = a2 + x.x * y.x; a3 = a3 + y.x * y.x;
            a1 = a1 + x.y * x.y; a2 = a2 + x.y * y.y; a3 = a3 + y.y * y.y;
            a1 = a1 + x.z * x.z; a2 = a2 + x.z * y.z; a3 = a3 + y.z * y.z;
            a1 = a1 + x.w * x.w; a2 = a2 + x.w * y.w; a3 = a3 + y.w * y.w;
          }
        }
        const float r1 = kx_finish(a1), r2 = kx_finish(a2), r3 = kx_finish(a3);
        if ((lane & 7) == 0 && lane < 24) {
          S.Hsum[qidx(px, px)] = r1;
          S.Hsum[qidx(px, py)] = r2;
          S.Hsum[qidx(py, py)] = r3;
        }
      } else {
        const int px = (g < 2 ? 0 : 2) + (warp - 1), pz = g == 0 ? 2 : 4;
        const float4* X4 = sd4 + px * 256;
        const float4* Z4 = sd4 + pz * 256;
        const float4* W4 = Z4 + 256;
        float a1 = -0.0f, a2 = -0.0f;
        for (int i = 0; i < P; ++i) {
#pragma unroll 8
          for (int r = 0; r < 32; ++r) {
            const float4 x = X4[i * 1536 + r * 8], z = Z4[i * 1536 + r * 8], w = W4[i * 1536 + r * 8];
            a1 = a1 + x.x * z.x; a2 = a2 + x.x * w.x;
            a1 = a1 + x.y * z.y; a2 = a2 + x.y * w.y;
            a1 = a1 + x.z * z.z; a2 = a2 + x.z * w.z;
            a1 = a1 + x.w * z.w; a2 = a2 + x.w * w.w;
          }
        }
        const float r1 = kx_finish(a1), r2 = kx_finish(a2);
        if ((lane & 7) == 0 && lane < 24) {
          S.Hsum[qidx(px, pz)] = r1;
          S.Hsum[qidx(px, pz + 1)] = r2;
        }
      }
    }
    fence_proxy_async();
    __syncthreads();
    if (chainA && trace) lt3 = clock64();
    if (chainA) {
      lu6_factor_warp(S.Hsum, S.f);

      normdp_init = 1e-10f;
      const int cont0 = (0 < op.maxiter) & ((1e-10f / 1e-10f) > op.normdp_ratio);
      if (lane == 0) {
        S.it = 0;
        S.cont[gi & 1u] = cont0;
      }
      if (cont0) place_and_issue();
      if (trace) lt4 = clock64();
    }
    __syncthreads();

    int it = 0;
    while (S.cont[gi & 1u]) {
      const unsigned par = gi & 1u;
      if (prod) {
#pragma unroll
        for (int s = 0; s < UPP; ++s) {
          const int u = pw + NPROD * s;
          if (u < U) {
            const int pp = u >> 1, half = u & 1;
            float* win = reinterpret_cast<float*>(s_slots + (u % KR_NSLOT) * KR_SLOT_BYTES);
            const int vis = S.nvis[pp];
            if (u >= KR_NSLOT) {
              if (lane == 0) {
                mbar_wait_relaxed(&S.slot_free[u - KR_NSLOT], par);
                if (vis) {
                  fence_proxy_async();
                  mbar_expect_tx(&S.win_full[u], KR_WIN_BYTES);
                  tma_load_2d(win, tmN, (S.nx[pp] - 1) & ~3, S.ny[pp] - 1 + 16 * half, &S.win_full[u]);
                } else {
                  mbar_arrive(&S.win_full[u]);
                }
              }
              __syncwarp();
            }
            if (vis) {
              const float4 w = S.npl[pp];
              const float* wsh = win + ((S.nx[pp] - 1) & 3);
              mbar_wait_backoff(&S.win_full[u], par);
              float a[17], b[17];
#pragma unroll
              for (int r = 0; r < 17; ++r) {
                a[r] = wsh[r * KR_WROW + lane + 1];
                b[r] = wsh[r * KR_WROW + lane];
              }
              __syncwarp();
#pragma unroll
              for (int r = 0; r < 16; ++r) {
                const float pn = ((w.x * a[r + 1] + w.y * b[r + 1]) + w.z * a[r]) + w.w * b[r];
                win[r * KR_WROW + perm] = refv[s][r] - pn;
              }
            } else {
#pragma unroll
              for (int r = 0; r < 16; ++r) win[r * KR_WROW + perm] = 0.0f;
            }
            __syncwarp();
            if (lane == 0) st_release_s(&S.pd_flag[u], gi + 1u);
          }
        }
      } else {
        const int c = lane & 7;
        const int k = chainA ? (lane >> 3) : 4 + ((lane >> 3) & 1);
        const float4* sdk = reinterpret_cast<const float4*>(s_sd) + k * 256 + c;
        float acc = -0.0f;
        long long t_c0 = 0, t_c1 = 0, w0 = 0;
        const unsigned want = gi + 1u;
        if (chainA && trace) t_c0 = clock64();
        while (ld_acquire_s(&S.pd_flag[0]) != want) {}
        if (chainA && trace) w0 = clock64() - t_c0;
#pragma unroll 1
        for (int u = 0; u < U; ++u) {
          const float4* pd4 = reinterpret_cast<const float4*>(s_slots + (u % KR_NSLOT) * KR_SLOT_BYTES) + c;
          const float4* sd4 = sdk + (u >> 1) * 1536 + (u & 1) * 128;
          unsigned nf = want;
#pragma unroll
          for (int h = 0; h < 2; ++h) {
            float4 sv[8], dv[8];
#pragma unroll
            for (int r = 0; r < 8; ++r) {
              sv[r] = sd4[(8 * h + r) * 8];
              dv[r] = pd4[(8 * h + r) * (KR_WROW / 4)];
            }
            if (h == 1 && u + 1 < U) nf = ld_acquire_s(&S.pd_flag[u + 1]);
#pragma unroll
            for (int r = 0; r < 8; ++r) {
              acc = acc + sv[r].x * dv[r].x;
              acc = acc + sv[r].y * dv[r].y;
              acc = acc + sv[r].z * dv[r].z;
              acc = acc + sv[r].w * dv[r].w;
            }
          }
          __syncwarp();
          if (lane == 0) mbar_arrive(&S.slot_free[u]);
          while (nf != want) nf = ld_acquire_s(&S.pd_flag[u + 1]);
        }
        const float res = kx_finish(acc);
        if (!chainA) {
          if ((lane & 7) == 0 && lane < 16) S.sum[4 + (lane >> 3)] = res;
          __syncwarp();
          if (lane == 0) st_release_s(&S.b_flag, want);
        } else {
          if ((lane & 7) == 0) S.sum[lane >> 3] = res;
          float lu[36];
#pragma unroll
          for (int j = 0; j < 36; ++j) lu[j] = S.f.lu[j];
          const int lu_rank = S.f.rank;
          while (ld_acquire_s(&S.b_flag) != want) {}
          if (trace) t_c1 = clock64();
          __syncwarp();
          float sumsd[6], dp[6], pr[6], Gr[12];
#pragma unroll
          for (int j = 0; j < 6; ++j) sumsd[j] = S.sum[j];
          lu6_solve_regs(lu, lu_rank, S.f.pr, S.f.qd, S.sum, S.dp);
          __syncwarp();
          const long long t_s1 = trace ? clock64() : 0;
#pragma unroll
          for (int j = 0; j < 6; ++j) { dp[j] = S.dp[j]; pr[j] = S.p[j] + dp[j]; }
          Gr[3] = Gr[7] = Gr[11] = 0.0f;
          se3_exp_f(Gr, pr);
          const long long t_s2 = trace ? clock64() : 0;
          const float normdp = ((fabsf(dp[0]) + fabsf(dp[2])) + (fabsf(dp[1]) + fabsf(dp[3]))) +
                               (fabsf(dp[4]) + fabsf(dp[5]));
          __syncwarp();
          if (lane < 6) S.p[lane] = pr[lane];
          if (lane < 12) S.G[lane] = Gr[lane];
          if (it == 0) normdp_init = normdp;
          const int cont = (it + 1 < op.maxiter) & ((normdp / normdp_init) > op.normdp_ratio);
          nvsum += S.nv;
          if (lane == 0) {
            if (trace && trace_n < prm.trace_cap) {
              float* rec = trace + (int64_t)ICT_TRACE_FLOATS * trace_n;
              rec[0] = (float)sl;
              rec[1] = (float)it;
              for (int j = 0; j < 6; ++j) { rec[2 + j] = sumsd[j]; rec[8 + j] = dp[j]; }
              rec[14] = normdp;
              rec[15] = (float)S.nv;
              for (int j = 16; j < ICT_TRACE_FLOATS; ++j) rec[j] = 0.0f;
              rec[16] = (float)w0;
              rec[17] = (float)(t_s1 - t_c1);
              if (it != 0) rec[18] = (float)(t_s2 - t_s1);
              if (it == 0) {
                rec[19] = (float)(lt1 - lt0);
                rec[20] = (float)(lt2 - lt1);
                rec[21] = (float)(lt3 - lt2);
                rec[18] = (float)(lt4 - lt3);
              }
              rec[22] = (float)(clock64() - t_c1);
              rec[23] = (float)(t_c1 - t_c0);
            }
            S.it = it + 1;
            S.cont[(gi + 1u) & 1u] = cont;
          }
          if (trace && trace_n < prm.trace_cap) ++trace_n;
          __syncwarp();
          if (cont) place_and_issue();
        }
      }
      __syncthreads();
      ++it;
      ++gi;
    }
    if (chainA && lane == 0 && prm.iters) prm.iters[(int64_t)t * (op.lv_f - op.lv_l + 1) + (op.lv_f - sl)] = S.it;
  }

  if (chainA && lane == 0) {
    getpose_se3(S.p, S.G, donorm, prm.norm + 4 * (int64_t)t, prm.norm[4 * (int64_t)t + 3], prm.p_out + 6 * (int64_t)t);
    if (prm.npixres) prm.npixres[t] = (long long)nvsum * 1024;
    if (trace)
      for (int k = trace_n; k < prm.trace_cap; ++k) {
        float* rec = trace + (int64_t)ICT_TRACE_FLOATS * k;
        for (int j = 0; j < ICT_TRACE_FLOATS; ++j) rec[j] = 0.0f;
        rec[0] = -1.0f;
      }
  }
}

static int kr_pcap(const ict_optparam& op, int max_pts) { return max_pts < op.maxpttrack ? max_pts : op.maxpttrack; }

size_t kr_smem_bytes(const ict_optparam& op, int max_pts) {
  return (size_t)kr_pcap(op, max_pts) * KR_SD_BYTES_PER_POINT + KR_NSLOT * KR_SLOT_BYTES + sizeof(KrShared) + 128;
}

bool kr_supported(const ict_optparam& op, int max_pts, int tma_ok) {
  const int P = kr_pcap(op, max_pts);
  return tma_ok && op.psz == 32 && !op.dopatchnorm && P >= 1 && P <= 8 &&
         kr_smem_bytes(op, max_pts) <= (size_t)ICT_TRACK_SMEM_LIMIT;
}

template <int NPROD, int UPP>
static cudaError_t launch_track_r_t(const TrackParams& prm, size_t smem, cudaStream_t stream) {
  static bool attr_dev[64] = {};
  int dev_ = 0;
  cudaGetDevice(&dev_);
  bool& attr_set = attr_dev[dev_ & 63];
  if (!attr_set) {
    cudaError_t e = cudaFuncSetAttribute(k_track_r<NPROD, UPP>, cudaFuncAttributeMaxDynamicSharedMemorySize, ICT_TRACK_SMEM_LIMIT);
    if (e == cudaSuccess)
      e = cudaFuncSetAttribute(k_track_r<NPROD, UPP>, cudaFuncAttributePreferredSharedMemoryCarveout, 100);
    if (e != cudaSuccess) return e;
    attr_set = true;
  }
  k_track_r<NPROD, UPP><<<prm.T, (NPROD + 2) * 32, smem, stream>>>(prm);
  count_launch_external();
  return cudaGetLastError();
}

cudaError_t launch_track_r(const TrackParams& prm_in, int max_pts, cudaStream_t stream) {
  if (prm_in.T <= 0) return cudaSuccess;
  if (!kr_supported(prm_in.op, max_pts, prm_in.tma_ok)) return cudaErrorInvalidConfiguration;
  TrackParams prm = prm_in;
  prm.r_pcap = kr_pcap(prm.op, max_pts);
  const size_t smem = kr_smem_bytes(prm.op, max_pts);
  if (prm.r_pcap <= 4) return launch_track_r_t<4, 2>(prm, smem, stream);
  return launch_track_r_t<8, 2>(prm, smem, stream);
}

}
```

### invcompcamtrack_b200/csrc/ict_kernels.cu

```cuda
#include "ict_kernels.cuh"
#include "ict_device.cuh"

#include <atomic>
#include <cstdlib>

namespace ict {

static std::atomic<long long> g_launches{0};
int64_t launch_count(int reset) {
  long long v = g_launches.load();
  if (reset) g_launches.store(0);
  return v;
}
#define COUNT_LAUNCH() g_launches.fetch_add(1)
void count_launch_external() { g_launches.fetch_add(1); }

template <typename SrcT>
__global__ void __launch_bounds__(256) k_pyr_level0(const SrcT* __restrict__ src, int w, int h, int pad,
                                                    float* __restrict__ I, float* __restrict__ dx,
                                                    float* __restrict__ dy, int64_t plane_stride) {
  const int sw = w + 2 * pad, sh = h + 2 * pad;
  const int X = blockIdx.x * blockDim.x + threadIdx.x;
  const int Y = blockIdx.y * blockDim.y + threadIdx.y;
  if (X >= sw || Y >= sh) return;
  const SrcT* s = src + (int64_t)blockIdx.z * w * h;
  const int x = X - pad, y = Y - pad;
  const int xc = min(max(x, 0), w - 1), yc = min(max(y, 0), h - 1);
  const float v = (float)s[(int64_t)yc * w + xc];
  const bool inside = (x >= 0) & (x < w) & (y >= 0) & (y < h);
  float gx = 0.0f, gy = 0.0f;
  if (inside) {
    if (x > 0 && x < w - 1) gx = (float)s[(int64_t)y * w + x + 1] - (float)s[(int64_t)y * w + x - 1];
    if (y > 0 && y < h - 1) gy = (float)s[(int64_t)(y + 1) * w + x] - (float)s[(int64_t)(y - 1) * w + x];
  }
  const int64_t o = (int64_t)blockIdx.z * plane_stride + (int64_t)Y * sw + X;
  I[o] = v;
  dx[o] = gx;
  dy[o] = gy;
}

__device__ __forceinline__ float mean4(const float* __restrict__ Ip, int swp, int pad, int x, int y) {
  const float* r0 = Ip + (int64_t)(2 * y + pad) * swp + 2 * x + pad;
  const float2 a = make_float2(__ldg(r0), __ldg(r0 + 1));
  const float2 c = make_float2(__ldg(r0 + swp), __ldg(r0 + swp + 1));
  return ((a.x + a.y) + (c.x + c.y)) * 0.25f;
}

__global__ void __launch_bounds__(256) k_pyr_levelN(float* __restrict__ I, float* __restrict__ dx,
                                                    float* __restrict__ dy, int64_t plane_stride, int64_t off_prev,
                                                    int swp, int64_t off_cur, int lw, int lh, int pad) {
  const int sw = lw + 2 * pad, sh = lh + 2 * pad;
  const int X = blockIdx.x * blockDim.x + threadIdx.x;
  const int Y = blockIdx.y * blockDim.y + threadIdx.y;
  if (X >= sw || Y >= sh) return;
  const float* Ip = I + (int64_t)blockIdx.z * plane_stride + off_prev;
  const int x = X - pad, y = Y - pad;
  const int xc = min(max(x, 0), lw - 1), yc = min(max(y, 0), lh - 1);
  const float v = mean4(Ip, swp, pad, xc, yc);
  const bool inside = (x >= 0) & (x < lw) & (y >= 0) & (y < lh);
  float gx = 0.0f, gy = 0.0f;
  if (inside) {
    if (x > 0 && x < lw - 1) gx = mean4(Ip, swp, pad, x + 1, y) - mean4(Ip, swp, pad, x - 1, y);
    if (y > 0 && y < lh - 1) gy = mean4(Ip, swp, pad, x, y + 1) - mean4(Ip, swp, pad, x, y - 1);
  }
  const int64_t o = (int64_t)blockIdx.z * plane_stride + off_cur + (int64_t)Y * sw + X;
  I[o] = v;
  dx[o] = gx;
  dy[o] = gy;
}

__device__ __forceinline__ void ld4(const float* p, float* v) {
  const float4 t = __ldg(reinterpret_cast<const float4*>(p));
  v[0] = t.x; v[1] = t.y; v[2] = t.z; v[3] = t.w;
}
__device__ __forceinline__ void ld4(const unsigned char* p, float* v) {
  const uchar4 t = __ldg(reinterpret_cast<const uchar4*>(p));
  v[0] = (float)t.x; v[1] = (float)t.y; v[2] = (float)t.z; v[3] = (float)t.w;
}

template <typename SrcT>
__global__ void __launch_bounds__(256) k_pyr_level0_v4(const SrcT* __restrict__ src, int w, int h, int pad,
                                                       float* __restrict__ I, float* __restrict__ dx,
                                                       float* __restrict__ dy, int64_t plane_stride) {
  const int sw = w + 2 * pad, sh = h + 2 * pad;
  const int X = (blockIdx.x * blockDim.x + threadIdx.x) * 4;
  const int Y = blockIdx.y * blockDim.y + threadIdx.y;
  if (X >= sw || Y >= sh) return;
  const SrcT* s = src + (int64_t)blockIdx.z * w * h;
  const int x = X - pad, y = Y - pad;
  const int yc = min(max(y, 0), h - 1);
  const bool yin = (y >= 0) & (y < h);
  float vi[4], gx[4] = {0.f, 0.f, 0.f, 0.f}, gy[4] = {0.f, 0.f, 0.f, 0.f};
  if (x < 0 || x >= w) {
    const float e = (float)s[(int64_t)yc * w + (x < 0 ? 0 : w - 1)];
    vi[0] = vi[1] = vi[2] = vi[3] = e;
  } else {
    const SrcT* row = s + (int64_t)yc * w + x;
    ld4(row, vi);
    if (yin) {
      const float left = x > 0 ? (float)row[-1] : 0.0f, right = x + 4 < w ? (float)row[4] : 0.0f;
      gx[0] = x > 0 ? vi[1] - left : 0.0f;
      gx[1] = vi[2] - vi[0];
      gx[2] = vi[3] - vi[1];
      gx[3] = x + 4 < w ? right - vi[2] : 0.0f;
      if (y > 0 && y < h - 1) {
        float up[4], dn[4];
        ld4(row - w, up);
        ld4(row + w, dn);
#pragma unroll
        for (int k = 0; k < 4; ++k) gy[k] = dn[k] - up[k];
      }
    }
  }
  const int64_t o = (int64_t)blockIdx.z * plane_stride + (int64_t)Y * sw + X;
  *reinterpret_cast<float4*>(I + o) = make_float4(vi[0], vi[1], vi[2], vi[3]);
  *reinterpret_cast<float4*>(dx + o) = make_float4(gx[0], gx[1], gx[2], gx[3]);
  *reinterpret_cast<float4*>(dy + o) = make_float4(gy[0], gy[1], gy[2], gy[3]);
}

__device__ __forceinline__ void mean4x4(const float* __restrict__ Ip, int swp, int pad, int x, int y, float* v) {
  const float* r0 = Ip + (int64_t)(2 * y + pad) * swp + 2 * x + pad;
  float a[8], c[8];
  ld4(r0, a); ld4(r0 + 4, a + 4);
  ld4(r0 + swp, c); ld4(r0 + swp + 4, c + 4);
#pragma unroll
  for (int k = 0; k < 4; ++k) v[k] = ((a[2 * k] + a[2 * k + 1]) + (c[2 * k] + c[2 * k + 1])) * 0.25f;
}

__global__ void __launch_bounds__(256) k_pyr_levelN_v4(float* __restrict__ I, float* __restrict__ dx,
                                                       float* __restrict__ dy, int64_t plane_stride, int64_t off_prev,
                                                       int swp, int64_t off_cur, int lw, int lh, int pad) {
  const int sw = lw + 2 * pad, sh = lh + 2 * pad;
  const int X = (blockIdx.x * blockDim.x + threadIdx.x) * 4;
  const int Y = blockIdx.y * blockDim.y + threadIdx.y;
  if (X >= sw || Y >= sh) return;
  const float* Ip = I + (int64_t)blockIdx.z * plane_stride + off_prev;
  const int x = X - pad, y = Y - pad;
  const int yc = min(max(y, 0), lh - 1);
  const bool yin = (y >= 0) & (y < lh);
  float vi[4], gx[4] = {0.f, 0.f, 0.f, 0.f}, gy[4] = {0.f, 0.f, 0.f, 0.f};
  if (x < 0 || x >= lw) {
    const float e = mean4(Ip, swp, pad, x < 0 ? 0 : lw - 1, yc);
    vi[0] = vi[1] = vi[2] = vi[3] = e;
  } else {
    mean4x4(Ip, swp, pad, x, yc, vi);
    if (yin) {
      gx[0] = x > 0 ? vi[1] - mean4(Ip, swp, pad, x - 1, y) : 0.0f;
      gx[1] = vi[2] - vi[0];
      gx[2] = vi[3] - vi[1];
      gx[3] = x + 4 < lw ? mean4(Ip, swp, pad, x + 4, y) - vi[2] : 0.0f;
      if (y > 0 && y < lh - 1) {
        float up[4], dn[4];
        mean4x4(Ip, swp, pad, x, y - 1, up);
        mean4x4(Ip, swp, pad, x, y + 1, dn);
#pragma unroll
        for (int k = 0; k < 4; ++k) gy[k] = dn[k] - up[k];
      }
    }
  }
  const int64_t o = (int64_t)blockIdx.z * plane_stride + off_cur + (int64_t)Y * sw + X;
  *reinterpret_cast<float4*>(I + o) = make_float4(vi[0], vi[1], vi[2], vi[3]);
  *reinterpret_cast<float4*>(dx + o) = make_float4(gx[0], gx[1], gx[2], gx[3]);
  *reinterpret_cast<float4*>(dy + o) = make_float4(gy[0], gy[1], gy[2], gy[3]);
}

cudaError_t launch_pyramid(const float* src_f32, const unsigned char* src_u8, int count, int w, int h, int lv_f,
                           int pad, float* I, float* dx, float* dy, int64_t plane_floats,
                           const int64_t* level_off, cudaStream_t stream) {
  if (count <= 0) return cudaSuccess;
  const dim3 blk(32, 8, 1);
  const bool vec = (pad % 4 == 0) && ((w >> lv_f) % 4 == 0) && (plane_floats % 4 == 0) &&
                   (((uintptr_t)I | (uintptr_t)dx | (uintptr_t)dy) % 16 == 0) &&
                   (src_u8 ? ((uintptr_t)src_u8 % 4 == 0) : ((uintptr_t)src_f32 % 16 == 0));
  for (int z0 = 0; z0 < count; z0 += 65535) {
    const int zc = min(count - z0, 65535);
    float* Iz = I + (int64_t)z0 * plane_floats;
    float* dxz = dx + (int64_t)z0 * plane_floats;
    float* dyz = dy + (int64_t)z0 * plane_floats;
    {
      const int sw = w + 2 * pad, sh = h + 2 * pad;
      if (vec) {
        const dim3 grd((sw / 4 + 31) / 32, (sh + 7) / 8, zc);
        if (src_u8)
          k_pyr_level0_v4<unsigned char><<<grd, blk, 0, stream>>>(src_u8 + (int64_t)z0 * w * h, w, h, pad, Iz, dxz, dyz,
                                                                   plane_floats);
        else
          k_pyr_level0_v4<float><<<grd, blk, 0, stream>>>(src_f32 + (int64_t)z0 * w * h, w, h, pad, Iz, dxz, dyz,
                                                           plane_floats);
      } else {
        const dim3 grd((sw + 31) / 32, (sh + 7) / 8, zc);
        if (src_u8)
          k_pyr_level0<unsigned char><<<grd, blk, 0, stream>>>(src_u8 + (int64_t)z0 * w * h, w, h, pad, Iz, dxz, dyz,
                                                                plane_floats);
        else
          k_pyr_level0<float><<<grd, blk, 0, stream>>>(src_f32 + (int64_t)z0 * w * h, w, h, pad, Iz, dxz, dyz,
                                                        plane_floats);
      }
      COUNT_LAUNCH();
    }
    for (int l = 1; l <= lv_f; ++l) {
      const int lw = w >> l, lh = h >> l;
      const int sw = lw + 2 * pad, sh = lh + 2 * pad;
      if (vec) {
        const dim3 grd((sw / 4 + 31) / 32, (sh + 7) / 8, zc);
        k_pyr_levelN_v4<<<grd, blk, 0, stream>>>(Iz, dxz, dyz, plane_floats, level_off[l - 1],
                                                 (w >> (l - 1)) + 2 * pad, level_off[l], lw, lh, pad);
      } else {
        const dim3 grd((sw + 31) / 32, (sh + 7) / 8, zc);
        k_pyr_levelN<<<grd, blk, 0, stream>>>(Iz, dxz, dyz, plane_floats, level_off[l - 1], (w >> (l - 1)) + 2 * pad,
                                              level_off[l], lw, lh, pad);
      }
      COUNT_LAUNCH();
    }
  }
  return cudaGetLastError();
}

#define ICT_SEQ_LIMIT 8192

__global__ void __launch_bounds__(256) k_set_points(int T, const int64_t* __restrict__ pt_off,
                                                    const double* pts, double* pts_mut,
                                                    float* __restrict__ pt3d, double* __restrict__ norm,
                                                    int donorm, int maxpttrack) {
  const int t = blockIdx.x;
  if (t >= T) return;
  const int64_t off = pt_off[t];
  const int n_in = (int)(pt_off[t + 1] - off);
  const int P = min(n_in, maxpttrack);
  const double* p1 = pts + 3 * off;
  const double* p2 = p1 + n_in;
  const double* p3 = p2 + n_in;
  float* q1 = pt3d + 3 * off;
  float* q2 = q1 + n_in;
  float* q3 = q2 + n_in;
  __shared__ double s_norm[4];
  __shared__ double s_red[3][8];
  const int tid = threadIdx.x, nt = blockDim.x;
  if (!donorm) {
    for (int i = tid; i < P; i += nt) {
      q1[i] = (float)p1[i];
      q2[i] = (float)p2[i];
      q3[i] = (float)p3[i];
    }
    if (tid < 4) norm[4 * (int64_t)t + tid] = 0.0;
    return;
  }
  if (P <= ICT_SEQ_LIMIT) {
    if (tid == 0) {
      const double nd = (double)P;
      double m0 = 0, m1 = 0, m2 = 0, var = 0;
      for (int i = 0; i < P; ++i) m0 += p1[i];
      for (int i = 0; i < P; ++i) m1 += p2[i];
      for (int i = 0; i < P; ++i) m2 += p3[i];
      m0 /= nd;
      m1 /= nd;
      m2 /= nd;
      for (int i = 0; i < P; ++i) {
        const double a = p1[i] - m0, b = p2[i] - m1, c = p3[i] - m2;
        var += a * a + b * b + c * c;
      }
      var /= nd;
      s_norm[0] = m0; s_norm[1] = m1; s_norm[2] = m2; s_norm[3] = var;
    }
  } else {
    double a[3] = {0, 0, 0};
    for (int i = tid; i < P; i += nt) { a[0] += p1[i]; a[1] += p2[i]; a[2] += p3[i]; }
    for (int k = 0; k < 3; ++k) {
      for (int o = 16; o > 0; o >>= 1) a[k] += __shfl_down_sync(0xffffffffu, a[k], o);
      if ((tid & 31) == 0) s_red[k][tid >> 5] = a[k];
    }
    __syncthreads();
    if (tid == 0)
      for (int k = 0; k < 3; ++k) {
        double s = 0;
        for (int wv = 0; wv < (nt >> 5); ++wv) s += s_red[k][wv];
        s_norm[k] = s / (double)P;
      }
    __syncthreads();
    double v = 0;
    for (int i = tid; i < P; i += nt) {
      const double x = p1[i] - s_norm[0], y = p2[i] - s_norm[1], z = p3[i] - s_norm[2];
      v += x * x + y * y + z * z;
    }
    for (int o = 16; o > 0; o >>= 1) v += __shfl_down_sync(0xffffffffu, v, o);
    __syncthreads();
    if ((tid & 31) == 0) s_red[0][tid >> 5] = v;
    __syncthreads();
    if (tid == 0) {
      double s = 0;
      for (int wv = 0; wv < (nt >> 5); ++wv) s += s_red[0][wv];
      s_norm[3] = s / (double)P;
    }
  }
  __syncthreads();
  const double m0 = s_norm[0], m1 = s_norm[1], m2 = s_norm[2], var = s_norm[3];
  for (int i = tid; i < P; i += nt) {
    const double a = p1[i] - m0, b = p2[i] - m1, c = p3[i] - m2;
    q1[i] = (float)(a / var);
    q2[i] = (float)(b / var);
    q3[i] = (float)(c / var);
    if (pts_mut) {
      pts_mut[3 * off + i] = a;
      pts_mut[3 * off + n_in + i] = b;
      pts_mut[3 * off + 2 * (int64_t)n_in + i] = c;
    }
  }
  if (tid < 4) norm[4 * (int64_t)t + tid] = s_norm[tid];
}

cudaError_t launch_set_points(int T, const int64_t* pt_off, const double* pts, double* pts_mut, float* pt3d,
                              double* norm, int donorm, int maxpttrack, int max_pts, cudaStream_t stream) {
  (void)max_pts;
  if (T <= 0) return cudaSuccess;
  k_set_points<<<T, 256, 0, stream>>>(T, pt_off, pts, pts_mut, pt3d, norm, donorm, maxpttrack);
  COUNT_LAUNCH();
  return cudaGetLastError();
}

struct TrackShared {
  float G[12];
  float p[6];
  float Hsum[21];
  float part[32 * 21];
  Lu6 lu;
  float normdp, normdp_init;
  int cont, it, nvis;
  long long npix;
};

template <int PSZ>
__device__ __forceinline__ void elem_split(int e, int n, int psz, int& i, int& r, int& c) {
  if constexpr (PSZ > 0) {
    i = e / (PSZ * PSZ);
    const int rem = e - i * (PSZ * PSZ);
    r = rem / PSZ;
    c = rem - r * PSZ;
  } else {
    i = e / n;
    const int rem = e - i * n;
    r = rem / psz;
    c = rem - r * psz;
  }
}

template <bool EX, int W>
__device__ __forceinline__ void patch_means(const float* buf, float* s_mean, const int* s_vis, int visbit, int P,
                                            int n, int tid, int nt) {
  if (EX) {
    for (int i = tid; i < P; i += nt) {
      if (!(s_vis[i] & visbit)) continue;
      const float* b = buf + i * n;
      s_mean[i] = eigen_sum_serial<W>([&](int e) { return b[e]; }, n) / n;
    }
  } else {
    const int lane = tid & 31, warp = tid >> 5, nw = nt >> 5;
    for (int i = warp; i < P; i += nw) {
      if (!(s_vis[i] & visbit)) continue;
      float s = 0.0f;
      for (int k = lane; k < n; k += 32) s = s + buf[i * n + k];
      s = warp_sum(s);
      if (lane == 0) s_mean[i] = s / n;
    }
  }
}

template <int PSZ, int MODE>
__global__ void __launch_bounds__(256) k_track(const TrackParams prm) {
  constexpr bool PN = (MODE & 1) != 0;
  constexpr bool EX = (MODE & 2) != 0;
  constexpr int PK = (MODE & 4) ? 8 : 4;
  constexpr int NCH = 2 * PK;
  extern __shared__ __align__(16) float smem[];
  __shared__ TrackShared S;
  __shared__ float s_chain[21 * NCH];

  const int t = blockIdx.x + prm.t0;
  const ict_optparam& op = prm.op;
  const int tid = threadIdx.x, nt = blockDim.x, lane = tid & 31, warp = tid >> 5, nw = nt >> 5;
  const int psz = PSZ > 0 ? PSZ : op.psz;
  const int n = PSZ > 0 ? PSZ * PSZ : op.novals;
  const int pszd2 = op.pszd2;
  const int64_t off = prm.pt_off[t];
  const int n_in = (int)(prm.pt_off[t + 1] - off);
  const int P = min(n_in, op.maxpttrack);
  const int E = P * n;
  const int Nfull = op.maxpttrack * n;
  const int Epad = (E + 3) & ~3;
  const bool donorm = op.donorm != 0;
  const bool patchnorm = PN && (op.dopatchnorm != 0);

  float* s_ref = smem;
  float* s_gx = s_ref + Epad;
  float* s_gy = s_gx + Epad;
  float* s_new = s_gy + Epad;
  float* s_ptf = MODE ? s_new + Epad : s_new;
  float* s_X = s_ptf;
  float* s_Y = s_X + P;
  float* s_Z = s_Y + P;
  float* s_Xc = s_Z + P;
  float* s_Yc = s_Xc + P;
  float* s_Zc = s_Yc + P;
  float* s_coef = s_Zc + P;
  float* s_w = s_coef + 10 * P;
  float* s_mean = s_w + 4 * P;
  int* s_base = (int*)(s_mean + P);
  int* s_vis = s_base + P;

  const int rf = prm.ref_frame ? prm.ref_frame[t] : prm.fixed_ref;
  const int nf = prm.new_frame ? prm.new_frame[t] : prm.fixed_new;
  const FrameDesc* fr_ref = prm.frames + rf;
  const FrameDesc* fr_new = prm.frames + nf;

  for (int e = tid; e < Epad; e += nt) { s_ref[e] = 0.0f; s_gx[e] = 0.0f; s_gy[e] = 0.0f; }
  {
    const float* q = prm.pt3d + 3 * off;
    for (int i = tid; i < P; i += nt) {
      s_X[i] = q[i];
      s_Y[i] = q[n_in + i];
      s_Z[i] = q[2 * (int64_t)n_in + i];
      s_vis[i] = 0;
#pragma unroll
      for (int k = 0; k < 10; ++k) s_coef[k * P + i] = 0.0f;
    }
  }
  if (tid == 0) {
    setpose_se3(prm.p_in + 6 * (int64_t)t, donorm, prm.norm + 4 * (int64_t)t, prm.norm[4 * (int64_t)t + 3], S.p,
                S.G);
    S.npix = 0;
    S.nvis = 0;
  }
  __syncthreads();
  for (int i = tid; i < P; i += nt) {
    const float X = s_X[i], Y = s_Y[i], Z = s_Z[i];
    const float xc = S.G[0] * X + S.G[1] * Y + S.G[2] * Z + S.G[3];
    const float yc = S.G[4] * X + S.G[5] * Y + S.G[6] * Z + S.G[7];
    const float zc = S.G[8] * X + S.G[9] * Y + S.G[10] * Z + S.G[11];
    s_Xc[i] = xc;
    s_Yc[i] = yc;
    s_Zc[i] = zc;
    if (prm.pt2d_out) {
      const int l = op.lv_l;
      prm.pt2d_out[2 * off + i] = (xc / zc) * prm.cam.fx[l] + prm.cam.cx[l];
      prm.pt2d_out[2 * off + n_in + i] = (yc / zc) * prm.cam.fy[l] + prm.cam.cy[l];
    }
  }
  __syncthreads();

  float* trace = prm.trace ? prm.trace + (int64_t)t * prm.trace_cap * ICT_TRACE_FLOATS : nullptr;
  int trace_n = 0;

  auto sd_at = [&](int q, int e) -> float {
    const int i = PSZ > 0 ? e / (PSZ * PSZ) : e / n;
    const float gx = s_gx[e], gy = s_gy[e];
    switch (q) {
      case 0: return gx * s_coef[0 * P + i];
      case 1: return gy * s_coef[1 * P + i];
      case 2: return gx * s_coef[2 * P + i] + gy * s_coef[3 * P + i];
      case 3: return gx * s_coef[4 * P + i] + gy * s_coef[5 * P + i];
      case 4: return gx * s_coef[6 * P + i] + gy * s_coef[7 * P + i];
      default: return gx * s_coef[8 * P + i] + gy * s_coef[9 * P + i];
    }
  };

  for (int sl = op.lv_f; sl >= op.lv_l; --sl) {
    const float fx = prm.cam.fx[sl], fy = prm.cam.fy[sl], cx = prm.cam.cx[sl], cy = prm.cam.cy[sl];
    const float swo = prm.cam.swo[sl], sho = prm.cam.sho[sl];
    const int width = prm.cam.width[sl];
    const float* __restrict__ Iref = fr_ref->I[sl];
    const float* __restrict__ Dxr = fr_ref->dx[sl];
    const float* __restrict__ Dyr = fr_ref->dy[sl];
    const float* __restrict__ Inew = fr_new->I[sl];

    for (int i = tid; i < P; i += nt) {
      const float xc = s_Xc[i], yc = s_Yc[i], zc = s_Zc[i];
      const float mx = (xc / zc) * fx + cx;
      const float my = (yc / zc) * fy + cy;
      const bool out = !((mx >= 0) & (my >= 0) & (mx <= swo) & (my <= sho));
      if (out) {
        s_vis[i] = 0;
      } else {
        s_vis[i] = 1;
        const PatchPlace q = patch_place(mx, my, pszd2, width);
        s_base[i] = q.base;
        s_w[i] = q.w0; s_w[P + i] = q.w1; s_w[2 * P + i] = q.w2; s_w[3 * P + i] = q.w3;
        float c[10];
        sd_coefs(xc, yc, zc, fx, fy, c);
#pragma unroll
        for (int k = 0; k < 10; ++k) s_coef[k * P + i] = c[k];
      }
    }
    __syncthreads();
    for (int e = tid; e < E; e += nt) {
      int i, r, c;
      elem_split<PSZ>(e, n, psz, i, r, c);
      if (s_vis[i] & 1) {
        const int addr = s_base[i] + r * width + c;
        const float w0 = s_w[i], w1 = s_w[P + i], w2 = s_w[2 * P + i], w3 = s_w[3 * P + i];
        s_ref[e] = bilin4(Iref, addr, width, w0, w1, w2, w3);
        s_gx[e] = bilin4(Dxr, addr, width, w0, w1, w2, w3);
        s_gy[e] = bilin4(Dyr, addr, width, w0, w1, w2, w3);
      }
    }
    if (patchnorm) {
      __syncthreads();
      patch_means<EX, PK>(s_ref, s_mean, s_vis, 1, P, n, tid, nt);
      __syncthreads();
      for (int e = tid; e < E; e += nt) {
        const int i = e / n;
        if (s_vis[i] & 1) s_ref[e] = s_ref[e] - s_mean[i];
      }
    }
    if (EX) {
      __syncthreads();
      const int as2 = (Nfull / NCH) * NCH;
      for (int qc = tid; qc < 21 * NCH; qc += nt) {
        const int q = qc / NCH, c = qc % NCH;
        int a = 0, b = 0, k = 0;
        for (int aa = 0; aa < 6; ++aa)
          for (int bb = aa; bb < 6; ++bb) { if (k == q) { a = aa; b = bb; } ++k; }
        s_chain[qc] = eigen_chain<PK>([&](int e) { return sd_at(a, e) * sd_at(b, e); }, c, as2, E);
      }
      __syncthreads();
      if (tid < 21) {
        int a = 0, b = 0, k = 0;
        for (int aa = 0; aa < 6; ++aa)
          for (int bb = aa; bb < 6; ++bb) { if (k == tid) { a = aa; b = bb; } ++k; }
        S.Hsum[tid] = eigen_finish<PK>(s_chain + NCH * tid, [&](int e) { return sd_at(a, e) * sd_at(b, e); }, Nfull, E);
      }
    } else {
      float acc[21];
#pragma unroll
      for (int k = 0; k < 21; ++k) acc[k] = 0.0f;
      for (int e = tid; e < E; e += nt) {
        int i, r, c;
        elem_split<PSZ>(e, n, psz, i, r, c);
        float cf[10], sd[6];
#pragma unroll
        for (int k = 0; k < 10; ++k) cf[k] = s_coef[k * P + i];
        sd_values(s_gx[e], s_gy[e], cf, sd);
        int k = 0;
#pragma unroll
        for (int a = 0; a < 6; ++a)
#pragma unroll
          for (int b = a; b < 6; ++b) { acc[k] = acc[k] + sd[a] * sd[b]; ++k; }
      }
#pragma unroll
      for (int k = 0; k < 21; ++k) {
        const float v = warp_sum(acc[k]);
        if (lane == 0) S.part[warp * 21 + k] = v;
      }
      __syncthreads();
      if (tid < 21) {
        float s = S.part[tid];
        for (int wv = 1; wv < nw; ++wv) s = s + S.part[wv * 21 + tid];
        S.Hsum[tid] = s;
      }
    }
    __syncthreads();
    if (warp == 0) lu6_factor_warp(S.Hsum, S.lu);
    if (tid == 0) {
      S.normdp_init = 1e-10f;
      S.normdp = 1e-10f;
      S.it = 0;
      S.cont = (0 < op.maxiter) & ((S.normdp / S.normdp_init) > op.normdp_ratio);
    }
    __syncthreads();

    while (S.cont) {
      for (int i = tid; i < P; i += nt) {
        const float X = s_X[i], Y = s_Y[i], Z = s_Z[i];
        const float tx = S.G[0] * X + S.G[1] * Y + S.G[2] * Z + S.G[3];
        const float ty = S.G[4] * X + S.G[5] * Y + S.G[6] * Z + S.G[7];
        const float tz = S.G[8] * X + S.G[9] * Y + S.G[10] * Z + S.G[11];
        const float mx = (tx / tz) * fx + cx;
        const float my = (ty / tz) * fy + cy;
        const bool out = !((mx >= 0) & (my >= 0) & (mx <= swo) & (my <= sho));
        if (out) {
          s_vis[i] &= ~2;
        } else {
          s_vis[i] |= 2;
          const PatchPlace q = patch_place(mx, my, pszd2, width);
          s_base[i] = q.base;
          s_w[i] = q.w0; s_w[P + i] = q.w1; s_w[2 * P + i] = q.w2; s_w[3 * P + i] = q.w3;
          atomicAdd(&S.nvis, 1);
        }
      }
      __syncthreads();
      if (patchnorm) {
        for (int e = tid; e < E; e += nt) {
          int i, r, c;
          elem_split<PSZ>(e, n, psz, i, r, c);
          if (s_vis[i] & 2)
            s_new[e] = bilin4(Inew, s_base[i] + r * width + c, width, s_w[i], s_w[P + i], s_w[2 * P + i],
                              s_w[3 * P + i]);
        }
        __syncthreads();
        patch_means<EX, PK>(s_new, s_mean, s_vis, 2, P, n, tid, nt);
        __syncthreads();
      }
      if (EX) {
        for (int e = tid; e < E; e += nt) {
          int i, r, c;
          elem_split<PSZ>(e, n, psz, i, r, c);
          float pd = 0.0f;
          if (s_vis[i] & 2) {
            float pn;
            if (patchnorm)
              pn = s_new[e] - s_mean[i];
            else
              pn = bilin4(Inew, s_base[i] + r * width + c, width, s_w[i], s_w[P + i], s_w[2 * P + i], s_w[3 * P + i]);
            pd = s_ref[e] - pn;
          }
          s_new[e] = pd;
        }
        __syncthreads();
        const int as2 = (Nfull / NCH) * NCH;
        if (tid < 6 * NCH) {
          const int q = tid / NCH, c = tid % NCH;
          s_chain[tid] = eigen_chain<PK>([&](int e) { return sd_at(q, e) * s_new[e]; }, c, as2, E);
        }
        __syncthreads();
        if (tid < 6)
          S.part[tid] = eigen_finish<PK>(s_chain + NCH * tid, [&](int e) { return sd_at(tid, e) * s_new[e]; }, Nfull, E);
      } else {
        float acc[6];
#pragma unroll
        for (int k = 0; k < 6; ++k) acc[k] = 0.0f;
        for (int e = tid; e < E; e += nt) {
          int i, r, c;
          elem_split<PSZ>(e, n, psz, i, r, c);
          if (s_vis[i] & 2) {
            float pn;
            if (patchnorm)
              pn = s_new[e] - s_mean[i];
            else
              pn = bilin4(Inew, s_base[i] + r * width + c, width, s_w[i], s_w[P + i], s_w[2 * P + i], s_w[3 * P + i]);
            const float pd = s_ref[e] - pn;
            float cf[10], sd[6];
#pragma unroll
            for (int k = 0; k < 10; ++k) cf[k] = s_coef[k * P + i];
            sd_values(s_gx[e], s_gy[e], cf, sd);
#pragma unroll
            for (int k = 0; k < 6; ++k) acc[k] = acc[k] + sd[k] * pd;
          }
        }
#pragma unroll
        for (int k = 0; k < 6; ++k) {
          const float v = warp_sum(acc[k]);
          if (lane == 0) S.part[warp * 6 + k] = v;
        }
      }
      __syncthreads();
      if (tid == 0) {
        float sumsd[6], dp[6];
        for (int k = 0; k < 6; ++k) {
          float s = S.part[k];
          if (!EX)
            for (int wv = 1; wv < nw; ++wv) s = s + S.part[wv * 6 + k];
          sumsd[k] = s;
        }
        lu6_solve(S.lu, sumsd, dp);
        for (int k = 0; k < 6; ++k) S.p[k] += dp[k];
        se3_exp<float>(S.G, S.p);
        const float normdp = ((fabsf(dp[0]) + fabsf(dp[2])) + (fabsf(dp[1]) + fabsf(dp[3]))) +
                             (fabsf(dp[4]) + fabsf(dp[5]));
        if (S.it == 0) S.normdp_init = normdp;
        S.normdp = normdp;
        if (trace && trace_n < prm.trace_cap) {
          float* rec = trace + (int64_t)ICT_TRACE_FLOATS * trace_n++;
          rec[0] = (float)sl;
          rec[1] = (float)S.it;
          for (int k = 0; k < 6; ++k) { rec[2 + k] = sumsd[k]; rec[8 + k] = dp[k]; }
          rec[14] = normdp;
          rec[15] = (float)S.nvis;
          for (int k = 16; k < ICT_TRACE_FLOATS; ++k) rec[k] = 0.0f;
        }
        S.npix += (long long)S.nvis * n;
        S.nvis = 0;
        S.it += 1;
        S.cont = (S.it < op.maxiter) & ((S.normdp / S.normdp_init) > op.normdp_ratio);
      }
      __syncthreads();
    }
    if (tid == 0 && prm.iters) prm.iters[(int64_t)t * (op.lv_f - op.lv_l + 1) + (op.lv_f - sl)] = S.it;
  }

  if (tid == 0) {
    getpose_se3(S.p, S.G, donorm, prm.norm + 4 * (int64_t)t, prm.norm[4 * (int64_t)t + 3],
                prm.p_out + 6 * (int64_t)t);
    if (prm.npixres) prm.npixres[t] = S.npix;
    if (trace)
      for (int k = trace_n; k < prm.trace_cap; ++k) {
        float* rec = trace + (int64_t)ICT_TRACE_FLOATS * k;
        for (int j = 0; j < ICT_TRACE_FLOATS; ++j) rec[j] = 0.0f;
        rec[0] = -1.0f;
      }
  }
}

__global__ void __launch_bounds__(128) k_reproject(const TrackParams prm) {
  __shared__ float s_p[6], s_G[12];
  const int t = blockIdx.x + prm.t0;
  const ict_optparam& op = prm.op;
  const int64_t off = prm.pt_off[t];
  const int n_in = (int)(prm.pt_off[t + 1] - off);
  const int P = min(n_in, op.maxpttrack);
  if (threadIdx.x == 0)
    setpose_se3(prm.p_in + 6 * (int64_t)t, op.donorm != 0, prm.norm + 4 * (int64_t)t, prm.norm[4 * (int64_t)t + 3], s_p,
                s_G);
  __syncthreads();
  const float* q = prm.pt3d + 3 * off;
  const int l = op.lv_l;
  for (int i = threadIdx.x; i < P; i += blockDim.x) {
    const float X = q[i], Y = q[n_in + i], Z = q[2 * (int64_t)n_in + i];
    const float xc = s_G[0] * X + s_G[1] * Y + s_G[2] * Z + s_G[3];
    const float yc = s_G[4] * X + s_G[5] * Y + s_G[6] * Z + s_G[7];
    const float zc = s_G[8] * X + s_G[9] * Y + s_G[10] * Z + s_G[11];
    prm.pt2d_out[2 * off + i] = (xc / zc) * prm.cam.fx[l] + prm.cam.cx[l];
    prm.pt2d_out[2 * off + n_in + i] = (yc / zc) * prm.cam.fy[l] + prm.cam.cy[l];
  }
}

cudaError_t launch_reproject(const TrackParams& prm, cudaStream_t stream) {
  if (prm.T <= 0) return cudaSuccess;
  k_reproject<<<prm.T, 128, 0, stream>>>(prm);
  COUNT_LAUNCH();
  return cudaGetLastError();
}


struct FastShared {
  float G[12];
  float p[6];
  float sum[8];
  float dp[6];
  float part[8 * 24];
  float Hsum[21];
  Lu6 lu;
  float normdp, normdp_init, lvl_cycles;
  int cont, it;
  long long npix;
};

template <int PSZ, int KTMAX, int MINB>
__global__ void __launch_bounds__(256, MINB) k_track_fast(const TrackParams prm) {
  constexpr int N = PSZ * PSZ;
  constexpr int KT = (N / 32 < KTMAX) ? N / 32 : KTMAX;
  constexpr int GE = 32 * KT;
  constexpr int GPP = N / GE;
  extern __shared__ __align__(16) float smem[];
  __shared__ FastShared S;

  const int t = blockIdx.x + prm.t0;
  const ict_optparam& op = prm.op;
  const int tid = threadIdx.x, nt = blockDim.x, lane = tid & 31, warp = tid >> 5, nw = nt >> 5;
  const int pszd2 = PSZ / 2;
  const int64_t off = prm.pt_off[t];
  const int n_in = (int)(prm.pt_off[t + 1] - off);
  const int P = min(n_in, op.maxpttrack);
  const int E = P * N;
  const bool donorm = op.donorm != 0;

  float* s_ref = smem;
  float* s_gx = s_ref + E;
  float* s_gy = s_gx + E;
  float* s_X = s_gy + E;
  float* s_Y = s_X + P;
  float* s_Z = s_Y + P;
  float* s_Xc = s_Z + P;
  float* s_Yc = s_Xc + P;
  float* s_Zc = s_Yc + P;
  float* s_coef = s_Zc + P;

  const int rf = prm.ref_frame ? prm.ref_frame[t] : prm.fixed_ref;
  const int nf = prm.new_frame ? prm.new_frame[t] : prm.fixed_new;
  const FrameDesc* fr_ref = prm.frames + rf;
  const FrameDesc* fr_new = prm.frames + nf;

  const int swarp = prm.serial_warp_last ? nw - 1 : 0;

  const int G_all = P * GPP;
  const int gpw = (G_all + nw - 1) / nw;
  const int g_lo = min(warp * gpw, G_all), g_hi = min(g_lo + gpw, G_all);

  for (int e = tid; e < E; e += nt) { s_ref[e] = 0.0f; s_gx[e] = 0.0f; s_gy[e] = 0.0f; }
  {
    const float* q = prm.pt3d + 3 * off;
    for (int i = tid; i < P; i += nt) {
      s_X[i] = q[i];
      s_Y[i] = q[n_in + i];
      s_Z[i] = q[2 * (int64_t)n_in + i];
#pragma unroll
      for (int k = 0; k < 10; ++k) s_coef[i * 10 + k] = 0.0f;
    }
  }
  if (tid == 0) {
    setpose_se3(prm.p_in + 6 * (int64_t)t, donorm, prm.norm + 4 * (int64_t)t, prm.norm[4 * (int64_t)t + 3], S.p,
                S.G);
    S.npix = 0;
  }
  __syncthreads();
  for (int i = tid; i < P; i += nt) {
    const float X = s_X[i], Y = s_Y[i], Z = s_Z[i];
    const float xc = S.G[0] * X + S.G[1] * Y + S.G[2] * Z + S.G[3];
    const float yc = S.G[4] * X + S.G[5] * Y + S.G[6] * Z + S.G[7];
    const float zc = S.G[8] * X + S.G[9] * Y + S.G[10] * Z + S.G[11];
    s_Xc[i] = xc;
    s_Yc[i] = yc;
    s_Zc[i] = zc;
    if (prm.pt2d_out) {
      const int l = op.lv_l;
      prm.pt2d_out[2 * off + i] = (xc / zc) * prm.cam.fx[l] + prm.cam.cx[l];
      prm.pt2d_out[2 * off + n_in + i] = (yc / zc) * prm.cam.fy[l] + prm.cam.cy[l];
    }
  }
  __syncthreads();

  float* trace = prm.trace ? prm.trace + (int64_t)t * prm.trace_cap * ICT_TRACE_FLOATS : nullptr;
  int trace_n = 0;

  for (int sl = op.lv_f; sl >= op.lv_l; --sl) {
    const float fx = prm.cam.fx[sl], fy = prm.cam.fy[sl], cx = prm.cam.cx[sl], cy = prm.cam.cy[sl];
    const float swo = prm.cam.swo[sl], sho = prm.cam.sho[sl];
    const int width = prm.cam.width[sl];
    const float* __restrict__ Iref = fr_ref->I[sl];
    const float* __restrict__ Dxr = fr_ref->dx[sl];
    const float* __restrict__ Dyr = fr_ref->dy[sl];
    const float* __restrict__ Inew = fr_new->I[sl];

    {
      float acc[21];
#pragma unroll
      for (int k = 0; k < 21; ++k) acc[k] = 0.0f;
      int cur = -1;
      bool vis = false;
      PatchPlace pl = {0, 0.f, 0.f, 0.f, 0.f};
      float cf[10];
#pragma unroll
      for (int k = 0; k < 10; ++k) cf[k] = 0.0f;
      float sxx = 0.0f, sxy = 0.0f, syy = 0.0f;
      for (int g = g_lo; g < g_hi; ++g) {
        const int i = g / GPP, gp = g - i * GPP;
        if (i != cur) {
          fold_hessian(acc, cf, sxx, sxy, syy);
          sxx = sxy = syy = 0.0f;
          cur = i;
          const float xc = s_Xc[i], yc = s_Yc[i], zc = s_Zc[i];
          const float mx = (xc / zc) * fx + cx, my = (yc / zc) * fy + cy;
          vis = (mx >= 0) & (my >= 0) & (mx <= swo) & (my <= sho);
          if (vis) {
            pl = patch_place(mx, my, pszd2, width);
            sd_coefs(xc, yc, zc, fx, fy, cf);
            if (gp == 0) {
#pragma unroll
              for (int k = 0; k < 10; ++k)
                if (lane == k) s_coef[i * 10 + k] = cf[k];
            }
          } else {
#pragma unroll
            for (int k = 0; k < 10; ++k) cf[k] = s_coef[i * 10 + k];
          }
        }
        const int ebase = i * N + gp * GE + lane;
        if (vis) {
          if (PSZ == 32) {
            const int a0 = pl.base + (gp * KT) * width + lane;
            float ci = __ldg(Iref + a0 - width), di = __ldg(Iref + a0 - width - 1);
            float cx_ = __ldg(Dxr + a0 - width), dx_ = __ldg(Dxr + a0 - width - 1);
            float cy_ = __ldg(Dyr + a0 - width), dy_ = __ldg(Dyr + a0 - width - 1);
#pragma unroll
            for (int j = 0; j < KT; ++j) {
              const int a = a0 + j * width;
              const float ai = __ldg(Iref + a), bi = __ldg(Iref + a - 1);
              const float ax = __ldg(Dxr + a), bx = __ldg(Dxr + a - 1);
              const float ay = __ldg(Dyr + a), by = __ldg(Dyr + a - 1);
              s_ref[ebase + 32 * j] = ((pl.w0 * ai + pl.w1 * bi) + pl.w2 * ci) + pl.w3 * di;
              s_gx[ebase + 32 * j] = ((pl.w0 * ax + pl.w1 * bx) + pl.w2 * cx_) + pl.w3 * dx_;
              s_gy[ebase + 32 * j] = ((pl.w0 * ay + pl.w1 * by) + pl.w2 * cy_) + pl.w3 * dy_;
              ci = ai; di = bi; cx_ = ax; dx_ = bx; cy_ = ay; dy_ = by;
            }
          } else {
#pragma unroll
            for (int j = 0; j < KT; ++j) {
              const int q = gp * GE + 32 * j + lane, r = q / PSZ, c = q - r * PSZ;
              const int a = pl.base + r * width + c;
              s_ref[ebase + 32 * j] = bilin4(Iref, a, width, pl.w0, pl.w1, pl.w2, pl.w3);
              s_gx[ebase + 32 * j] = bilin4(Dxr, a, width, pl.w0, pl.w1, pl.w2, pl.w3);
              s_gy[ebase + 32 * j] = bilin4(Dyr, a, width, pl.w0, pl.w1, pl.w2, pl.w3);
            }
          }
        }
#pragma unroll
        for (int j = 0; j < KT; ++j) {
          const float gx = s_gx[ebase + 32 * j], gy = s_gy[ebase + 32 * j];
          sxx = sxx + gx * gx;
          sxy = sxy + gx * gy;
          syy = syy + gy * gy;
        }
      }
      fold_hessian(acc, cf, sxx, sxy, syy);
      warp_sum_store<21>(acc, &S.part[warp * 24]);
    }
    __syncthreads();
    if (warp == swarp) {
      const long long t_lv0 = trace ? clock64() : 0;
      if (lane < 21) {
        float v[8];
#pragma unroll
        for (int wv = 0; wv < 8; ++wv) v[wv] = wv < nw ? S.part[wv * 24 + lane] : 0.0f;
        float s = v[0];
#pragma unroll
        for (int wv = 1; wv < 8; ++wv) s = wv < nw ? s + v[wv] : s;
        S.Hsum[lane] = s;
      }
      __syncwarp();
      lu6_factor_warp(S.Hsum, S.lu);
      if (lane == 0) {
        S.normdp_init = 1e-10f;
        S.normdp = 1e-10f;
        S.it = 0;
        S.cont = (0 < op.maxiter) & ((S.normdp / S.normdp_init) > op.normdp_ratio);
        S.lvl_cycles = (float)(clock64() - t_lv0);
      }
    }
    __syncthreads();

    while (S.cont) {
      const long long t_it0 = trace ? clock64() : 0;
      float Gm[12];
#pragma unroll
      for (int k = 0; k < 12; ++k) Gm[k] = S.G[k];
      float acc[6];
#pragma unroll
      for (int k = 0; k < 6; ++k) acc[k] = 0.0f;
      int nvis = 0;
      int cur = -1;
      bool vis = false;
      PatchPlace pl = {0, 0.f, 0.f, 0.f, 0.f};
      float cf[10];
#pragma unroll
      for (int k = 0; k < 10; ++k) cf[k] = 0.0f;
      float ax = 0.0f, ay = 0.0f;
      for (int g = g_lo; g < g_hi; ++g) {
        const int i = g / GPP, gp = g - i * GPP;
        if (i != cur) {
          fold_jtr(acc, cf, ax, ay);
          ax = ay = 0.0f;
          cur = i;
          const float X = s_X[i], Y = s_Y[i], Z = s_Z[i];
          const float tx = Gm[0] * X + Gm[1] * Y + Gm[2] * Z + Gm[3];
          const float ty = Gm[4] * X + Gm[5] * Y + Gm[6] * Z + Gm[7];
          const float tz = Gm[8] * X + Gm[9] * Y + Gm[10] * Z + Gm[11];
          const float mx = (tx / tz) * fx + cx, my = (ty / tz) * fy + cy;
          vis = (mx >= 0) & (my >= 0) & (mx <= swo) & (my <= sho);
          if (vis) {
            pl = patch_place(mx, my, pszd2, width);
#pragma unroll
            for (int k = 0; k < 10; ++k) cf[k] = s_coef[i * 10 + k];
            nvis += (gp == 0);
          }
        }
        if (!vis) continue;
        const int ebase = i * N + gp * GE + lane;
        if (PSZ == 32) {
          const int a0 = pl.base + (gp * KT) * width + lane;
          float c_ = __ldg(Inew + a0 - width), d_ = __ldg(Inew + a0 - width - 1);
#pragma unroll
          for (int j = 0; j < KT; ++j) {
            const float a_ = __ldg(Inew + a0 + j * width), b_ = __ldg(Inew + a0 + j * width - 1);
            const float pn = ((pl.w0 * a_ + pl.w1 * b_) + pl.w2 * c_) + pl.w3 * d_;
            c_ = a_; d_ = b_;
            const float pd = s_ref[ebase + 32 * j] - pn;
            ax = ax + s_gx[ebase + 32 * j] * pd;
            ay = ay + s_gy[ebase + 32 * j] * pd;
          }
        } else {
#pragma unroll
          for (int j = 0; j < KT; ++j) {
            const int q = gp * GE + 32 * j + lane, r = q / PSZ, c = q - r * PSZ;
            const float pn = bilin4(Inew, pl.base + r * width + c, width, pl.w0, pl.w1, pl.w2, pl.w3);
            const float pd = s_ref[ebase + 32 * j] - pn;
            ax = ax + s_gx[ebase + 32 * j] * pd;
            ay = ay + s_gy[ebase + 32 * j] * pd;
          }
        }
      }
      fold_jtr(acc, cf, ax, ay);
      warp_sum6_store(acc, &S.part[warp * 24]);
      if (lane == 0) S.part[warp * 24 + 6] = (float)nvis;
      const long long t_par = trace ? clock64() : 0;
      __syncthreads();
      if (warp == swarp) {
        const long long t_ser0 = trace ? clock64() : 0;
        if (lane < 7) {
          float v[8];
#pragma unroll
          for (int wv = 0; wv < 8; ++wv) v[wv] = wv < nw ? S.part[wv * 24 + lane] : 0.0f;
          float s = v[0];
#pragma unroll
          for (int wv = 1; wv < 8; ++wv) s = wv < nw ? s + v[wv] : s;
          S.sum[lane] = s;
        }
        __syncwarp();
        const bool fullrank = S.lu.rank == 6;
        if (fullrank) {
          const float x = lu6_solve_warp_rcp(S.lu, S.sum);
          if (lane < 6) S.dp[lane] = x;
          __syncwarp();
        }
        if (lane == 0 && prm.dbg_skip_serial) {
          S.it += 1;
          S.cont = S.it < op.maxiter;
        } else if (lane == 0) {
          if (!fullrank) lu6_solve(S.lu, S.sum, S.dp);
          float dp[6], pr[6], Gr[12];
#pragma unroll
          for (int k = 0; k < 6; ++k) { dp[k] = S.dp[k]; pr[k] = S.p[k] + dp[k]; S.p[k] = pr[k]; }
          Gr[3] = Gr[7] = Gr[11] = 0.0f;
          se3_exp_f32_series(Gr, pr);
#pragma unroll
          for (int k = 0; k < 12; ++k) S.G[k] = Gr[k];
          const float normdp = ((fabsf(dp[0]) + fabsf(dp[2])) + (fabsf(dp[1]) + fabsf(dp[3]))) +
                               (fabsf(dp[4]) + fabsf(dp[5]));
          if (S.it == 0) S.normdp_init = normdp;
          S.normdp = normdp;
          const int nv = (int)S.sum[6];
          if (trace && trace_n < prm.trace_cap) {
            float* rec = trace + (int64_t)ICT_TRACE_FLOATS * trace_n++;
            rec[0] = (float)sl;
            rec[1] = (float)S.it;
            for (int k = 0; k < 6; ++k) { rec[2 + k] = S.sum[k]; rec[8 + k] = dp[k]; }
            rec[14] = normdp;
            rec[15] = (float)nv;
            for (int k = 16; k < ICT_TRACE_FLOATS; ++k) rec[k] = 0.0f;
            rec[21] = S.lvl_cycles;
            rec[22] = (float)(clock64() - t_ser0);
            rec[23] = (float)(t_par - t_it0);
          }
          S.npix += (long long)nv * N;
          S.it += 1;
          S.cont = (S.it < op.maxiter) & ((S.normdp / S.normdp_init) > op.normdp_ratio);
        }
      }
      __syncthreads();
    }
    if (tid == 0 && prm.iters) prm.iters[(int64_t)t * (op.lv_f - op.lv_l + 1) + (op.lv_f - sl)] = S.it;
  }

  if (tid == 0) {
    getpose_se3(S.p, S.G, donorm, prm.norm + 4 * (int64_t)t, prm.norm[4 * (int64_t)t + 3],
                prm.p_out + 6 * (int64_t)t);
    if (prm.npixres) prm.npixres[t] = S.npix;
    if (trace)
      for (int k = trace_n; k < prm.trace_cap; ++k) {
        float* rec = trace + (int64_t)ICT_TRACE_FLOATS * k;
        for (int j = 0; j < ICT_TRACE_FLOATS; ++j) rec[j] = 0.0f;
        rec[0] = -1.0f;
      }
  }
}

static size_t fast_smem_bytes(const ict_optparam& op, int max_pts) {
  const size_t P = (size_t)(max_pts < op.maxpttrack ? max_pts : op.maxpttrack);
  return sizeof(float) * (3 * P * op.novals + 16 * P);
}

template <int PSZ, int KTMAX, int MINB>
static cudaError_t launch_track_fast_v(const TrackParams& prm, size_t smem, int nt, cudaStream_t stream) {
  static bool attr_dev[64] = {};
  int dev_ = 0;
  cudaGetDevice(&dev_);
  bool& attr_set = attr_dev[dev_ & 63];
  if (!attr_set) {
    cudaError_t e = cudaFuncSetAttribute(k_track_fast<PSZ, KTMAX, MINB>, cudaFuncAttributeMaxDynamicSharedMemorySize,
                                         ICT_TRACK_SMEM_LIMIT);
    if (e == cudaSuccess)
      e = cudaFuncSetAttribute(k_track_fast<PSZ, KTMAX, MINB>, cudaFuncAttributePreferredSharedMemoryCarveout, 100);
    if (e != cudaSuccess) return e;
    attr_set = true;
  }
  k_track_fast<PSZ, KTMAX, MINB><<<prm.T, nt, smem, stream>>>(prm);
  COUNT_LAUNCH();
  return cudaGetLastError();
}

template <int PSZ>
static cudaError_t launch_track_fast_t(const TrackParams& prm, size_t smem, int nt, cudaStream_t stream) {
  static int variant = -1;
  if (variant < 0) {
    const char* e = ict_knob("ICT_FAST_VARIANT");
    variant = e ? atoi(e) : 4;
  }
  if (PSZ == 32) {
    switch (variant) {
      case 0: return launch_track_fast_v<PSZ, 4, 4>(prm, smem, nt, stream);
      case 1: return launch_track_fast_v<PSZ, 4, 3>(prm, smem, nt, stream);
      case 2: return launch_track_fast_v<PSZ, 8, 4>(prm, smem, nt, stream);
      case 3: return launch_track_fast_v<PSZ, 8, 3>(prm, smem, nt, stream);
      case 5: return launch_track_fast_v<PSZ, 16, 3>(prm, smem, nt, stream);
      default: return launch_track_fast_v<PSZ, 16, 4>(prm, smem, nt, stream);
    }
  }
  return launch_track_fast_v<PSZ, 4, 4>(prm, smem, nt, stream);
}

size_t track_smem_bytes(const ict_optparam& op, int max_pts, int sum_mode) {
  const int P = max_pts < op.maxpttrack ? max_pts : op.maxpttrack;
  const size_t E = (size_t)P * op.novals;
  const size_t Epad = (E + 3) & ~(size_t)3;
  const size_t planes = (op.dopatchnorm || sum_mode) ? 4 : 3;
  return sizeof(float) * (planes * Epad + (size_t)23 * P) + 16;
}

template <int PSZ, int MODE>
static cudaError_t launch_track_t(const TrackParams& prm, size_t smem, int nt, cudaStream_t stream) {
  static bool attr_dev[64] = {};
  int dev_ = 0;
  cudaGetDevice(&dev_);
  bool& attr_set = attr_dev[dev_ & 63];
  if (!attr_set) {
    cudaError_t e = cudaFuncSetAttribute(k_track<PSZ, MODE>, cudaFuncAttributeMaxDynamicSharedMemorySize,
                                         ICT_TRACK_SMEM_LIMIT);
    if (e != cudaSuccess) return e;
    attr_set = true;
  }
  k_track<PSZ, MODE><<<prm.T, nt, smem, stream>>>(prm);
  COUNT_LAUNCH();
  return cudaGetLastError();
}

template <int PSZ>
static cudaError_t launch_track_p(const TrackParams& prm, size_t smem, int nt, int mode, cudaStream_t stream) {
  switch (mode) {
    case 0: return launch_track_t<PSZ, 0>(prm, smem, nt, stream);
    case 1: return launch_track_t<PSZ, 1>(prm, smem, nt, stream);
    case 2: return launch_track_t<PSZ, 2>(prm, smem, nt, stream);
    case 3: return launch_track_t<PSZ, 3>(prm, smem, nt, stream);
    case 6: return launch_track_t<PSZ, 6>(prm, smem, nt, stream);
    default: return launch_track_t<PSZ, 7>(prm, smem, nt, stream);
  }
}

bool track_fits_one_cta(const ict_optparam& op, int max_pts, int sum_mode, int force_general) {
  if (track_smem_bytes(op, max_pts, sum_mode) <= (size_t)ICT_TRACK_SMEM_LIMIT) return true;
  if (force_general) return false;
  if (sum_mode) return !ict_knob("ICT_EXACT_V1") && kx8_supported(op, max_pts);
  return !ict_knob("ICT_FAST_V1") && v8_supported(op, max_pts);
}

bool track_chain_in_one_launch(const ict_optparam& op, int max_pts, int sum_mode, int force_general, int per_frame_launches) {
  return sum_mode == 0 && !force_general && !per_frame_launches && !ict_knob("ICT_FAST_V1") &&
         v8_supported(op, max_pts);
}

cudaError_t launch_track(const TrackParams& prm, int max_pts, cudaStream_t stream) {
  if (prm.T <= 0) return cudaSuccess;
  if (prm.seq_n > 1 && !track_chain_in_one_launch(prm.op, max_pts, prm.sum_mode, prm.force_general, prm.knob_seq_launches))
    return cudaErrorInvalidConfiguration;
  const size_t smem = track_smem_bytes(prm.op, max_pts, prm.sum_mode);
  if (!track_fits_one_cta(prm.op, max_pts, prm.sum_mode, prm.force_general)) return cudaErrorInvalidConfiguration;
  const int P = max_pts < prm.op.maxpttrack ? max_pts : prm.op.maxpttrack;
  const long long E = (long long)P * prm.op.novals;
  int nt = E >= 2048 ? 256 : (E >= 512 ? 128 : 64);
  const int mode = (prm.op.dopatchnorm ? 1 : 0) | (prm.sum_mode ? 2 : 0) | (prm.sum_mode && prm.eigen_packet == 8 ? 4 : 0);
  if (const char* e = ict_knob("ICT_NT")) nt = atoi(e);
  if ((mode & 2) == 0 && !prm.force_general && !ict_knob("ICT_FAST_V1") && v8_supported(prm.op, max_pts))
    return launch_track_v8(prm, max_pts, stream);
  if (mode == 0 && !prm.force_general && prm.op.psz == 32 && !ict_knob("ICT_FAST_V1") &&
      v2_smem_bytes(prm.op, max_pts) <= (size_t)ICT_TRACK_SMEM_LIMIT)
    return launch_track_v2(prm, max_pts, stream);
  if (mode == 0 && !prm.force_general && (prm.op.psz == 8 || prm.op.psz == 16 || prm.op.psz == 32)) {
    const size_t fsm = fast_smem_bytes(prm.op, max_pts);
    switch (prm.op.psz) {
      case 8: return launch_track_fast_t<8>(prm, fsm, nt, stream);
      case 16: return launch_track_fast_t<16>(prm, fsm, nt, stream);
      default: return launch_track_fast_t<32>(prm, fsm, nt, stream);
    }
  }
  if ((mode & 2) && !prm.force_general && !ict_knob("ICT_EXACT_V1") && kx8_supported(prm.op, max_pts))
    return launch_track_x8(prm, max_pts, stream);
  if (mode == 2 && !prm.force_general && !prm.knob_no_k2r && !ict_knob("ICT_EXACT_V1") &&
      kr_supported(prm.op, max_pts, prm.tma_ok))
    return launch_track_r(prm, max_pts, stream);
  if (mode == 2 && !prm.force_general && prm.op.psz == 32 && !ict_knob("ICT_EXACT_V1") &&
      kx_smem_bytes(prm.op, max_pts) <= (size_t)ICT_TRACK_SMEM_LIMIT)
    return launch_track_x(prm, max_pts, stream);
  const int ntx = (mode & 2) && nt < 192 ? 192 : nt;
  switch (prm.op.psz) {
    case 8: return launch_track_p<8>(prm, smem, ntx, mode, stream);
    case 16: return launch_track_p<16>(prm, smem, ntx, mode, stream);
    case 32: return launch_track_p<32>(prm, smem, ntx, mode, stream);
    default: return launch_track_p<0>(prm, smem, ntx, mode, stream);
  }
}

}
```

### invcompcamtrack_b200/csrc/ict_kernels.cuh

```cuda
#pragma once
#include <cuda_runtime.h>
#include <stdint.h>
#include "../../include/ictrack.h"
#include "ict_knobs.h"

namespace ict {

struct CamLevels {
  float fx[ICT_MAX_LEVELS], fy[ICT_MAX_LEVELS], cx[ICT_MAX_LEVELS], cy[ICT_MAX_LEVELS];
  float swo[ICT_MAX_LEVELS], sho[ICT_MAX_LEVELS];
  int width[ICT_MAX_LEVELS];
};

struct FrameDesc {
  const float* I[ICT_MAX_LEVELS];
  const float* dx[ICT_MAX_LEVELS];
  const float* dy[ICT_MAX_LEVELS];
  const void* tmap;
};

struct TrackParams {
  ict_optparam op;
  CamLevels cam;
  const FrameDesc* frames;
  const int* ref_frame;
  const int* new_frame;
  int fixed_ref, fixed_new;
  const int64_t* pt_off;
  const float* pt3d;
  const double* norm;
  const double* p_in;
  double* p_out;
  int* iters;
  float* trace;
  int trace_cap;
  const float* teacher;
  long long* npixres;
  float* pt2d_out;
  int T;
  int t0;
  int serial_warp_last;
  int dbg_skip_serial;
  int v2_lu_setup;
  int force_general;
  int seq_n, seq_step;
  float* state;
  int64_t state_stride;
  int state_load;
  unsigned robust;
  int knob_no_k2r;
  int knob_seq_launches;
  int tma_ok;
  int r_pcap;
  int sum_mode;
  int eigen_packet;
};

#define ICT_TRACK_SMEM_LIMIT (227 * 1024 - 8192)

cudaError_t launch_pyramid(const float* src_f32, const unsigned char* src_u8, int count, int w, int h, int lv_f,
                           int pad, float* I, float* dx, float* dy, int64_t plane_floats,
                           const int64_t* level_off, cudaStream_t stream);

cudaError_t launch_set_points(int T, const int64_t* pt_off, const double* pts, double* pts_mut, float* pt3d,
                              double* norm, int donorm, int maxpttrack, int max_pts, cudaStream_t stream);

size_t track_smem_bytes(const ict_optparam& op, int max_pts, int sum_mode);
bool track_fits_one_cta(const ict_optparam& op, int max_pts, int sum_mode, int force_general);
bool track_chain_in_one_launch(const ict_optparam& op, int max_pts, int sum_mode, int force_general, int per_frame_launches);
cudaError_t launch_track(const TrackParams& prm, int max_pts, cudaStream_t stream);

size_t v2_smem_bytes(const ict_optparam& op, int max_pts);
cudaError_t launch_track_v2(const TrackParams& prm, int max_pts, cudaStream_t stream);

bool v8_supported(const ict_optparam& op, int max_pts);
size_t v8_smem_bytes(const ict_optparam& op, int max_pts);
cudaError_t launch_track_v8(const TrackParams& prm, int max_pts, cudaStream_t stream);

size_t kx_smem_bytes(const ict_optparam& op, int max_pts);
cudaError_t launch_track_x(const TrackParams& prm, int max_pts, cudaStream_t stream);

bool kr_supported(const ict_optparam& op, int max_pts, int tma_ok);
size_t kr_smem_bytes(const ict_optparam& op, int max_pts);
cudaError_t launch_track_r(const TrackParams& prm, int max_pts, cudaStream_t stream);

bool kx8_supported(const ict_optparam& op, int max_pts);
size_t kx8_smem_bytes(const ict_optparam& op, int max_pts);
cudaError_t launch_track_x8(const TrackParams& prm, int max_pts, cudaStream_t stream);

cudaError_t launch_reproject(const TrackParams& prm, cudaStream_t stream);

struct BigTrackWork;
size_t bigtrack_work_bytes(const ict_optparam& op, int64_t npts, int eigen_packet);
cudaError_t launch_track_big(const TrackParams& prm, int t, int64_t npts, void* work, cudaStream_t stream);

cudaError_t launch_ncc(const ict_optparam& op, const CamLevels& cam, const float* img_b, const float* img_r,
                       const float* img_f, int nback, int nfwd, const int64_t* pt_off, int T, const float* pb,
                       const float* pr, const float* pf, float* out, cudaStream_t stream);

cudaError_t launch_get_patches(const float* I, const float* dx, const float* dy, int width, int psz, int pszd2,
                               int patchnorm, int npatch, const float* mids, float* out_I, float* out_dx, float* out_dy,
                               cudaStream_t stream);

cudaError_t launch_hypotheses(const double fc[2], const double cc[2], int npts, const double* pt2d, const double* pt3d,
                              int nsamples, const int* sample, const double p_init[6], double inlthresh, int maxiter,
                              double* pose, int* status, int* ninl, unsigned char* mask, cudaStream_t stream);

int64_t launch_count(int reset);

}
```

Measured before the change: 167.0 billion.

## Add two-slot TMEM-backed persistent tracking kernel K2t with ticket scheduling

Measured after the change: 171.6 billion (median of 6 runs). +2.8%, better.

```diff
diff --git a/__graft_entry__.py b/__graft_entry__.py
--- a/__graft_entry__.py
+++ b/__graft_entry__.py
@@ -46,7 +46,7 @@
     g32 = gpu_run(ict, case32, trace_cap=40, sum_order=0)
     r32 = check_parity(g32, o32, case32, gates=False)
     assert r32["jtr_first"] <= 1e-5, r32
-    print("smoke psz32 ok: default kernel (K2r, reference order) bit-identical to the oracle on %d tracks; fast mode "
+    print("smoke psz32 ok: default kernel (K2t, reference order) bit-identical to the oracle on %d tracks; fast mode "
           "(K2v2) J^T r on identical inputs within %.1e of sum|sd*r| (gate 1e-5), %.0f%% identical iteration counts"
           % (case32["T"], r32["jtr_first"], 100 * r32["frac_same"]))
 
diff --git a/invcompcamtrack_b200/build.py b/invcompcamtrack_b200/build.py
--- a/invcompcamtrack_b200/build.py
+++ b/invcompcamtrack_b200/build.py
@@ -8,8 +8,8 @@
 NVCC = os.environ.get("NVCC", "/usr/local/cuda/bin/nvcc")
 NVCC_FLAGS = ["-gencode", "arch=compute_100a,code=sm_100a", "-lineinfo", "-O3", "-fmad=false", "-std=c++17",
               "-Xcompiler", "-fPIC", "-ccbin", "g++"] + os.environ.get("ICT_EXTRA_NVCC", "").split()
-LIB_SOURCES = ["ict_kernels.cu", "ict_kernel_v2.cu", "ict_kernel_v8.cu", "ict_kernel_x.cu", "ict_kernel_x8.cu", "ict_kernel_r.cu", "ict_kernels_big.cu", "ict_hypotheses.cu", "ict_capi.cu"]
-LIB_DEPS = LIB_SOURCES + ["ict_kernels.cuh", "ict_device.cuh", "ict_kernel_v2.cuh", "ict_kernel_v8.cuh", "ict_kernel_x.cuh", "ict_knobs.h", os.path.join("..", "..", "include", "ictrack.h")]
+LIB_SOURCES = ["ict_kernels.cu", "ict_kernel_v2.cu", "ict_kernel_v8.cu", "ict_kernel_x.cu", "ict_kernel_x8.cu", "ict_kernel_r.cu", "ict_kernel_rt.cu", "ict_kernels_big.cu", "ict_hypotheses.cu", "ict_capi.cu"]
+LIB_DEPS = LIB_SOURCES + ["ict_kernels.cuh", "ict_device.cuh", "ict_kernel_v2.cuh", "ict_kernel_v8.cuh", "ict_kernel_x.cuh", "ict_kernel_r.cuh", "ict_knobs.h", os.path.join("..", "..", "include", "ictrack.h")]
 
 
 def _stale(target, deps):
diff --git a/invcompcamtrack_b200/csrc/ict_capi.cu b/invcompcamtrack_b200/csrc/ict_capi.cu
--- a/invcompcamtrack_b200/csrc/ict_capi.cu
+++ b/invcompcamtrack_b200/csrc/ict_capi.cu
@@ -440,13 +440,14 @@
   int sum_mode = 1;
   int eigen_packet = 4;
   int force_general = 0;
-  int knob_no_k2r = 0, knob_seq_launches = 0;
+  int knob_no_k2r = 0, knob_no_k2t = 0, knob_seq_launches = 0;
   unsigned robust = 0;
   int keep_state = 0;
   bool state_valid = false;
   int seq_n = 0, seq_step = 0;
   const int *big_rf = nullptr, *big_nf = nullptr;
   DevBuf pt_off, pts, pt3d, norm, p_in, p_out, iters, npix, trace, pt2d, rf, nf, big, teacher, state;
+  DevBuf ticket;
   int teacher_cap = 0;
   static const int ICT_BIG_LANES = 4;
   cudaStream_t big_st[ICT_BIG_LANES] = {};
@@ -479,7 +480,7 @@
 void ict_tracker_destroy(ict_tracker* tr) {
   if (!tr) return;
   DevBuf* b[] = {&tr->pt_off, &tr->pts, &tr->pt3d, &tr->norm, &tr->p_in, &tr->p_out, &tr->iters,
-                 &tr->npix, &tr->trace, &tr->pt2d, &tr->rf, &tr->nf, &tr->big, &tr->teacher, &tr->state};
+                 &tr->npix, &tr->trace, &tr->pt2d, &tr->rf, &tr->nf, &tr->big, &tr->teacher, &tr->state, &tr->ticket};
   for (DevBuf* x : b) x->release();
   for (int k = 0; k < ict_tracker::ICT_BIG_LANES; ++k) {
     tr->big_lane[k].release();
@@ -528,6 +529,7 @@
 int ict_tracker_set_knob(ict_tracker* tr, const char* name, int value) {
   if (!tr || !name) return fail(ICT_ERR_BAD_ARG, "null argument");
   if (!strcmp(name, "no_k2r")) tr->knob_no_k2r = value ? 1 : 0;
+  else if (!strcmp(name, "no_k2t")) tr->knob_no_k2t = value ? 1 : 0;
   else if (!strcmp(name, "seq_launches")) tr->knob_seq_launches = value ? 1 : 0;
   else if (!strcmp(name, "keep_state")) { tr->keep_state = value ? 1 : 0; tr->state_valid = false; }
   else return fail(ICT_ERR_BAD_ARG, std::string("unknown knob: ") + name);
@@ -662,6 +664,9 @@
   prm.seq_n = tr->seq_n;
   prm.seq_step = tr->seq_step;
   prm.knob_no_k2r = tr->knob_no_k2r;
+  prm.knob_no_k2t = tr->knob_no_k2t;
+  CU(tr->ticket.reserve(sizeof(unsigned)));
+  prm.rt_ticket = tr->ticket.as<unsigned>();
   prm.knob_seq_launches = tr->knob_seq_launches;
   prm.robust = tr->robust;
   if (tr->robust && !(tr->sum_mode == 0 && !tr->force_general && v8_supported(tr->op, tr->max_pts)))
diff --git a/invcompcamtrack_b200/csrc/ict_kernel_r.cu b/invcompcamtrack_b200/csrc/ict_kernel_r.cu
--- a/invcompcamtrack_b200/csrc/ict_kernel_r.cu
+++ b/invcompcamtrack_b200/csrc/ict_kernel_r.cu
@@ -3,105 +3,11 @@
 #include "ict_kernels.cuh"
 #include "ict_device.cuh"
 #include "ict_kernel_x.cuh"
+#include "ict_kernel_r.cuh"
 
 namespace ict {
 
 void count_launch_external();
-
-#define KR_WROW 40
-#define KR_WIN_BYTES (17 * KR_WROW * 4)
-#define KR_SLOT_BYTES 2816
-#define KR_NSLOT 5
-
-#define KR_MAXU 16
-#define KR_SD_BYTES_PER_POINT (6 * 1024 * 4)
-
-__device__ __forceinline__ void tma_load_2d(void* dst, const void* tmap, int x, int y, unsigned long long* bar) {
-  asm volatile(
-      "cp.async.bulk.tensor.2d.shared::cluster.global.tile.mbarrier::complete_tx::bytes [%0], [%1, {%2, %3}], [%4];" ::"r"(
-          ict_saddr(dst)),
-      "l"(tmap), "r"(x), "r"(y), "r"(ict_saddr(bar))
-      : "memory");
-}
-__device__ __forceinline__ void mbar_expect_tx_only(unsigned long long* b, unsigned bytes) {
-  asm volatile("mbarrier.expect_tx.relaxed.cta.shared::cta.b64 [%0], %1;" ::"r"(ict_saddr(b)), "r"(bytes) : "memory");
-}
-__device__ __forceinline__ void mbar_wait_backoff(unsigned long long* b, unsigned parity) {
-  unsigned done = 0;
-  for (int tries = 0;; ++tries) {
-    asm volatile(
-        "{\n"
-        ".reg .pred P1;\n"
-        "mbarrier.try_wait.parity.shared::cta.b64 P1, [%1], %2;\n"
-        "selp.u32 %0, 1, 0, P1;\n"
-        "}\n"
-        : "=r"(done)
-        : "r"(ict_saddr(b)), "r"(parity)
-        : "memory");
-    if (done) break;
-    if (tries >= 4) __nanosleep(40);
-  }
-}
-__device__ __forceinline__ void fence_proxy_async() { asm volatile("fence.proxy.async.shared::cta;" ::: "memory"); }
-__device__ __forceinline__ void tmap_acquire(const void* tmap) {
-  asm volatile("fence.proxy.tensormap::generic.acquire.sys [%0], 128;" ::"l"(tmap) : "memory");
-}
-
-struct __align__(16) KrShared {
-  unsigned long long win_full[KR_MAXU];
-  unsigned long long slot_free[KR_MAXU];
-  unsigned long long gat_full[2];
-  unsigned pd_flag[KR_MAXU];
-  unsigned b_flag;
-  unsigned pad_[3];
-  float G[12];
-  float p[8];
-  float sum[8];
-  float dp[8];
-  float Hsum[24];
-  Lu6 f;
-  float4 npl[8];
-  float4 rpl[8];
-  int nx[8], ny[8], nvis[8];
-  int rx[8], ry[8], rvis[8];
-  float X[8], Y[8], Z[8], Xc[8], Yc[8], Zc[8];
-  int cont[2], it, nv;
-};
-
-__device__ __forceinline__ void kr_patch_place(float mx, float my, int* x0, int* y0, float4* w) {
-  const int pos0 = (int)ceilf(mx + .00001f);
-  const int pos1 = (int)ceilf(my + .00001f);
-  const int pos2 = (int)floorf(mx);
-  const int pos3 = (int)floorf(my);
-  const float r0 = mx - (float)pos2;
-  const float r1 = my - (float)pos3;
-  w->x = r0 * r1;
-  w->y = (1 - r0) * r1;
-  w->z = r0 * (1 - r1);
-  w->w = (1 - r0) * (1 - r1);
-  *x0 = pos0 + 16;
-  *y0 = pos1 + 16;
-}
-
-__device__ __forceinline__ void kr_sample16(const float* win, int lane, const float4 w, float* out) {
-  float a0 = win[lane + 1], b0 = win[lane];
-#pragma unroll
-  for (int r = 0; r < 16; ++r) {
-    const float a1 = win[(r + 1) * KR_WROW + lane + 1], b1 = win[(r + 1) * KR_WROW + lane];
-    out[r] = ((w.x * a1 + w.y * b1) + w.z * a0) + w.w * b0;
-    a0 = a1;
-    b0 = b1;
-  }
-}
-
-__device__ __forceinline__ unsigned ld_acquire_s(const unsigned* p) {
-  unsigned v;
-  asm volatile("ld.acquire.cta.shared.u32 %0, [%1];" : "=r"(v) : "r"(ict_saddr(p)) : "memory");
-  return v;
-}
-__device__ __forceinline__ void st_release_s(unsigned* p, unsigned v) {
-  asm volatile("st.release.cta.shared.u32 [%0], %1;" ::"r"(ict_saddr(p)), "r"(v) : "memory");
-}
 
 struct KrRows8 {
   float4 v[8];
diff --git a/invcompcamtrack_b200/csrc/ict_kernel_r.cuh b/invcompcamtrack_b200/csrc/ict_kernel_r.cuh
--- /dev/null
+++ b/invcompcamtrack_b200/csrc/ict_kernel_r.cuh
@@ -0,0 +1,101 @@
+#pragma once
+#include "ict_device.cuh"
+
+namespace ict {
+
+#define KR_WROW 40
+#define KR_WIN_BYTES (17 * KR_WROW * 4)
+#define KR_SLOT_BYTES 2816
+#define KR_NSLOT 5
+
+#define KR_MAXU 16
+#define KR_SD_BYTES_PER_POINT (6 * 1024 * 4)
+
+__device__ __forceinline__ void tma_load_2d(void* dst, const void* tmap, int x, int y, unsigned long long* bar) {
+  asm volatile(
+      "cp.async.bulk.tensor.2d.shared::cluster.global.tile.mbarrier::complete_tx::bytes [%0], [%1, {%2, %3}], [%4];" ::"r"(
+          ict_saddr(dst)),
+      "l"(tmap), "r"(x), "r"(y), "r"(ict_saddr(bar))
+      : "memory");
+}
+__device__ __forceinline__ void mbar_expect_tx_only(unsigned long long* b, unsigned bytes) {
+  asm volatile("mbarrier.expect_tx.relaxed.cta.shared::cta.b64 [%0], %1;" ::"r"(ict_saddr(b)), "r"(bytes) : "memory");
+}
+__device__ __forceinline__ void mbar_wait_backoff(unsigned long long* b, unsigned parity) {
+  unsigned done = 0;
+  for (int tries = 0;; ++tries) {
+    asm volatile(
+        "{\n"
+        ".reg .pred P1;\n"
+        "mbarrier.try_wait.parity.shared::cta.b64 P1, [%1], %2;\n"
+        "selp.u32 %0, 1, 0, P1;\n"
+        "}\n"
+        : "=r"(done)
+        : "r"(ict_saddr(b)), "r"(parity)
+        : "memory");
+    if (done) break;
+    if (tries >= 4) __nanosleep(40);
+  }
+}
+__device__ __forceinline__ void fence_proxy_async() { asm volatile("fence.proxy.async.shared::cta;" ::: "memory"); }
+__device__ __forceinline__ void tmap_acquire(const void* tmap) {
+  asm volatile("fence.proxy.tensormap::generic.acquire.sys [%0], 128;" ::"l"(tmap) : "memory");
+}
+
+struct __align__(16) KrShared {
+  unsigned long long win_full[KR_MAXU];
+  unsigned long long slot_free[KR_MAXU];
+  unsigned long long gat_full[2];
+  unsigned pd_flag[KR_MAXU];
+  unsigned b_flag;
+  unsigned pad_[3];
+  float G[12];
+  float p[8];
+  float sum[8];
+  float dp[8];
+  float Hsum[24];
+  Lu6 f;
+  float4 npl[8];
+  float4 rpl[8];
+  int nx[8], ny[8], nvis[8];
+  int rx[8], ry[8], rvis[8];
+  float X[8], Y[8], Z[8], Xc[8], Yc[8], Zc[8];
+  int cont[2], it, nv;
+};
+
+__device__ __forceinline__ void kr_patch_place(float mx, float my, int* x0, int* y0, float4* w) {
+  const int pos0 = (int)ceilf(mx + .00001f);
+  const int pos1 = (int)ceilf(my + .00001f);
+  const int pos2 = (int)floorf(mx);
+  const int pos3 = (int)floorf(my);
+  const float r0 = mx - (float)pos2;
+  const float r1 = my - (float)pos3;
+  w->x = r0 * r1;
+  w->y = (1 - r0) * r1;
+  w->z = r0 * (1 - r1);
+  w->w = (1 - r0) * (1 - r1);
+  *x0 = pos0 + 16;
+  *y0 = pos1 + 16;
+}
+
+__device__ __forceinline__ void kr_sample16(const float* win, int lane, const float4 w, float* out) {
+  float a0 = win[lane + 1], b0 = win[lane];
+#pragma unroll
+  for (int r = 0; r < 16; ++r) {
+    const float a1 = win[(r + 1) * KR_WROW + lane + 1], b1 = win[(r + 1) * KR_WROW + lane];
+    out[r] = ((w.x * a1 + w.y * b1) + w.z * a0) + w.w * b0;
+    a0 = a1;
+    b0 = b1;
+  }
+}
+
+__device__ __forceinline__ unsigned ld_acquire_s(const unsigned* p) {
+  unsigned v;
+  asm volatile("ld.acquire.cta.shared.u32 %0, [%1];" : "=r"(v) : "r"(ict_saddr(p)) : "memory");
+  return v;
+}
+__device__ __forceinline__ void st_release_s(unsigned* p, unsigned v) {
+  asm volatile("st.release.cta.shared.u32 [%0], %1;" ::"r"(ict_saddr(p)), "r"(v) : "memory");
+}
+
+}
diff --git a/invcompcamtrack_b200/csrc/ict_kernel_rt.cu b/invcompcamtrack_b200/csrc/ict_kernel_rt.cu
--- /dev/null
+++ b/invcompcamtrack_b200/csrc/ict_kernel_rt.cu
@@ -0,0 +1,617 @@
+#include <cuda.h>
+
+#include "ict_kernels.cuh"
+#include "ict_device.cuh"
+#include "ict_kernel_x.cuh"
+#include "ict_kernel_r.cuh"
+
+namespace ict {
+
+void count_launch_external();
+
+#define KT_PMAX 4
+#define KT_NPROD 4
+#define KT_UPP 2
+#define KT_SLOT_WARPS (KT_NPROD + 2)
+#define KT_THREADS (2 * KT_SLOT_WARPS * 32)
+#define KT_TMEM_COLS 512
+#define KT_AB_BYTES 256
+#define KT_SLOT_BYTES_RAW (KT_PMAX * KR_SD_BYTES_PER_POINT + KT_AB_BYTES + sizeof(KrShared))
+#define KT_SLOT_STRIDE ((KT_SLOT_BYTES_RAW + 127) / 128 * 128)
+#define KT_SMEM_BYTES (2 * KT_SLOT_STRIDE + 128)
+static_assert(KT_SMEM_BYTES <= ICT_TRACK_SMEM_LIMIT, "two track slots must fit one CTA");
+
+__device__ __forceinline__ void slot_sync(int slot) {
+  asm volatile("bar.sync %0, %1;" ::"r"(1 + slot), "n"(KT_SLOT_WARPS * 32) : "memory");
+}
+
+__device__ __forceinline__ void tm_ld32(unsigned taddr, unsigned (&s)[32]) {
+  asm volatile(
+      "tcgen05.ld.sync.aligned.32x32b.x32.b32 {%0, %1, %2, %3, %4, %5, %6, %7, %8, %9, %10, %11, %12, %13, %14, %15, %16, "
+      "%17, %18, %19, %20, %21, %22, %23, %24, %25, %26, %27, %28, %29, %30, %31}, [%32];"
+      : "=r"(s[0]), "=r"(s[1]), "=r"(s[2]), "=r"(s[3]), "=r"(s[4]), "=r"(s[5]), "=r"(s[6]), "=r"(s[7]), "=r"(s[8]),
+        "=r"(s[9]), "=r"(s[10]), "=r"(s[11]), "=r"(s[12]), "=r"(s[13]), "=r"(s[14]), "=r"(s[15]), "=r"(s[16]),
+        "=r"(s[17]), "=r"(s[18]), "=r"(s[19]), "=r"(s[20]), "=r"(s[21]), "=r"(s[22]), "=r"(s[23]), "=r"(s[24]),
+        "=r"(s[25]), "=r"(s[26]), "=r"(s[27]), "=r"(s[28]), "=r"(s[29]), "=r"(s[30]), "=r"(s[31])
+      : "r"(taddr));
+}
+__device__ __forceinline__ void tm_ld16(unsigned taddr, unsigned (&s)[16]) {
+  asm volatile(
+      "tcgen05.ld.sync.aligned.32x32b.x16.b32 {%0, %1, %2, %3, %4, %5, %6, %7, %8, %9, %10, %11, %12, %13, %14, %15}, [%16];"
+      : "=r"(s[0]), "=r"(s[1]), "=r"(s[2]), "=r"(s[3]), "=r"(s[4]), "=r"(s[5]), "=r"(s[6]), "=r"(s[7]), "=r"(s[8]),
+        "=r"(s[9]), "=r"(s[10]), "=r"(s[11]), "=r"(s[12]), "=r"(s[13]), "=r"(s[14]), "=r"(s[15])
+      : "r"(taddr));
+}
+__device__ __forceinline__ void tm_st32(unsigned taddr, const float4 (&v)[8]) {
+  asm volatile(
+      "tcgen05.st.sync.aligned.32x32b.x32.b32 [%0], {%1, %2, %3, %4, %5, %6, %7, %8, %9, %10, %11, %12, %13, %14, %15, %16, "
+      "%17, %18, %19, %20, %21, %22, %23, %24, %25, %26, %27, %28, %29, %30, %31, %32};" ::"r"(taddr),
+      "f"(v[0].x), "f"(v[0].y), "f"(v[0].z), "f"(v[0].w), "f"(v[1].x), "f"(v[1].y), "f"(v[1].z), "f"(v[1].w),
+      "f"(v[2].x), "f"(v[2].y), "f"(v[2].z), "f"(v[2].w), "f"(v[3].x), "f"(v[3].y), "f"(v[3].z), "f"(v[3].w),
+      "f"(v[4].x), "f"(v[4].y), "f"(v[4].z), "f"(v[4].w), "f"(v[5].x), "f"(v[5].y), "f"(v[5].z), "f"(v[5].w),
+      "f"(v[6].x), "f"(v[6].y), "f"(v[6].z), "f"(v[6].w), "f"(v[7].x), "f"(v[7].y), "f"(v[7].z), "f"(v[7].w)
+      : "memory");
+}
+__device__ __forceinline__ void tm_wait_ld() { asm volatile("tcgen05.wait::ld.sync.aligned;" ::: "memory"); }
+__device__ __forceinline__ void tm_wait_st() { asm volatile("tcgen05.wait::st.sync.aligned;" ::: "memory"); }
+__device__ __forceinline__ void tm_fence_before() { asm volatile("tcgen05.fence::before_thread_sync;" ::: "memory"); }
+__device__ __forceinline__ void tm_fence_after() { asm volatile("tcgen05.fence::after_thread_sync;" ::: "memory"); }
+
+__device__ __forceinline__ float4 kt_lds128(const float4* p) {
+  float4 v;
+  asm volatile("ld.shared.v4.f32 {%0, %1, %2, %3}, [%4];" : "=f"(v.x), "=f"(v.y), "=f"(v.z), "=f"(v.w) : "r"(ict_saddr(p)));
+  return v;
+}
+
+__device__ __forceinline__ void kt_add4(const unsigned (&s)[16], const float4 (&d)[4], float& acc) {
+#pragma unroll
+  for (int r = 0; r < 4; ++r) {
+    acc = acc + __uint_as_float(s[4 * r]) * d[r].x;
+    acc = acc + __uint_as_float(s[4 * r + 1]) * d[r].y;
+    acc = acc + __uint_as_float(s[4 * r + 2]) * d[r].z;
+    acc = acc + __uint_as_float(s[4 * r + 3]) * d[r].w;
+  }
+}
+
+__global__ void __launch_bounds__(KT_THREADS, 1) k_track_rt(const TrackParams prm) {
+  extern __shared__ unsigned char smem_raw[];
+  __shared__ unsigned s_taddr;
+  __shared__ int s_ticket[2];
+  const ict_optparam& op = prm.op;
+  const int lane = threadIdx.x & 31;
+  const int slot = threadIdx.x / (KT_SLOT_WARPS * 32);
+  const int warp = (threadIdx.x >> 5) - KT_SLOT_WARPS * slot;
+  const int tid = threadIdx.x - KT_SLOT_WARPS * 32 * slot, nt = KT_SLOT_WARPS * 32;
+  const bool donorm = op.donorm != 0;
+
+  unsigned char* base = smem_raw + ((128u - (ict_saddr(smem_raw) & 127u)) & 127u) + (size_t)slot * KT_SLOT_STRIDE;
+  float* s_sd = reinterpret_cast<float*>(base);
+  float(*s_AB)[12] = reinterpret_cast<float(*)[12]>(base + (size_t)KT_PMAX * KR_SD_BYTES_PER_POINT);
+  KrShared& S = *reinterpret_cast<KrShared*>(base + (size_t)KT_PMAX * KR_SD_BYTES_PER_POINT + KT_AB_BYTES);
+  unsigned char* s_win = base;
+  static_assert(2 * KT_PMAX * KR_SLOT_BYTES <= KR_SD_BYTES_PER_POINT, "the windows of a track fit point 0's sd plane");
+  const bool chainA = warp == 0, prod = warp >= 2;
+  const int pw = warp - 2;
+
+  if (threadIdx.x < 32) {
+    asm volatile("tcgen05.alloc.cta_group::1.sync.aligned.shared::cta.b32 [%0], %1;" ::"r"(ict_saddr(&s_taddr)),
+                 "n"(KT_TMEM_COLS)
+                 : "memory");
+    asm volatile("tcgen05.relinquish_alloc_permit.cta_group::1.sync.aligned;" ::: "memory");
+  }
+  if (tid >= 32 && tid < 32 + KR_MAXU) {
+    mbar_init(&S.win_full[tid - 32], 1);
+    S.pd_flag[tid - 32] = 0u;
+  }
+  if (tid == 64) {
+    mbar_init(&S.gat_full[0], 1);
+    mbar_init(&S.gat_full[1], 1);
+    S.b_flag = 0u;
+  }
+  mbar_fence_init();
+  tm_fence_before();
+  __syncthreads();
+  tm_fence_after();
+  const unsigned tl = s_taddr + ((32u * ((threadIdx.x >> 5) & 3u)) << 16);
+
+  unsigned gi = 0;
+  unsigned lvl = 0;
+  unsigned upar = 0;
+  const int perm = 4 * (lane & 7) + (lane >> 3);
+
+  for (;;) {
+    if (tid == 0) s_ticket[slot] = (int)atomicAdd(prm.rt_ticket, 1u);
+    slot_sync(slot);
+    const int tk = s_ticket[slot];
+    if (tk >= prm.T) break;
+    const int t = tk + prm.t0;
+    const int64_t off = prm.pt_off[t];
+    const int n_in = (int)(prm.pt_off[t + 1] - off);
+    const int P = min(n_in, op.maxpttrack);
+    const int U = 2 * P;
+    const int rf = prm.ref_frame ? prm.ref_frame[t] : prm.fixed_ref;
+    const int nf = prm.new_frame ? prm.new_frame[t] : prm.fixed_new;
+
+    {
+      const float4 z4 = make_float4(0.f, 0.f, 0.f, 0.f);
+      float4* sd4 = reinterpret_cast<float4*>(s_sd);
+      for (int e = tid; e < P * (KR_SD_BYTES_PER_POINT / 16); e += nt) sd4[e] = z4;
+      const float* q = prm.pt3d + 3 * off;
+      for (int i = tid; i < P; i += nt) {
+        S.X[i] = q[i];
+        S.Y[i] = q[n_in + i];
+        S.Z[i] = q[2 * (int64_t)n_in + i];
+      }
+    }
+    if (tid == 0)
+      setpose_se3(prm.p_in + 6 * (int64_t)t, donorm, prm.norm + 4 * (int64_t)t, prm.norm[4 * (int64_t)t + 3], S.p, S.G);
+    slot_sync(slot);
+    for (int i = tid; i < P; i += nt) {
+      const float X = S.X[i], Y = S.Y[i], Z = S.Z[i];
+      const float xc = S.G[0] * X + S.G[1] * Y + S.G[2] * Z + S.G[3];
+      const float yc = S.G[4] * X + S.G[5] * Y + S.G[6] * Z + S.G[7];
+      const float zc = S.G[8] * X + S.G[9] * Y + S.G[10] * Z + S.G[11];
+      S.Xc[i] = xc;
+      S.Yc[i] = yc;
+      S.Zc[i] = zc;
+      if (prm.pt2d_out) {
+        const int l = op.lv_l;
+        prm.pt2d_out[2 * off + i] = (xc / zc) * prm.cam.fx[l] + prm.cam.cx[l];
+        prm.pt2d_out[2 * off + n_in + i] = (yc / zc) * prm.cam.fy[l] + prm.cam.cy[l];
+      }
+    }
+    slot_sync(slot);
+
+    const bool trace = prm.trace != nullptr;
+    int trace_n = 0;
+    float normdp_init = 1e-10f;
+    int nvsum = 0;
+    const unsigned umask = (1u << U) - 1u;
+    float refv[KT_UPP][16];
+#pragma unroll
+    for (int s = 0; s < KT_UPP; ++s)
+#pragma unroll
+      for (int r = 0; r < 16; ++r) refv[s][r] = 0.0f;
+
+    for (int sl = op.lv_f; sl >= op.lv_l; --sl, ++lvl) {
+      const float fx = prm.cam.fx[sl], fy = prm.cam.fy[sl], cx = prm.cam.cx[sl], cy = prm.cam.cy[sl];
+      const float swo = prm.cam.swo[sl], sho = prm.cam.sho[sl];
+      const char* tm_ref = reinterpret_cast<const char*>(prm.frames[rf].tmap);
+      const char* tm_new = reinterpret_cast<const char*>(prm.frames[nf].tmap);
+      const void* tmI = tm_ref + 128 * (0 * ICT_MAX_LEVELS + sl);
+      const void* tmDx = tm_ref + 128 * (1 * ICT_MAX_LEVELS + sl);
+      const void* tmDy = tm_ref + 128 * (2 * ICT_MAX_LEVELS + sl);
+      const void* tmN = tm_new + 128 * (0 * ICT_MAX_LEVELS + sl);
+
+      long long lt0 = 0, lt1 = 0, lt2 = 0, lt3 = 0, lt4 = 0;
+      if (chainA && trace) lt0 = clock64();
+      if (warp == 0) {
+        tmap_acquire(tmI);
+        tmap_acquire(tmDx);
+        tmap_acquire(tmDy);
+        tmap_acquire(tmN);
+      } else if (prod && lane == 0) {
+        tmap_acquire(tmN);
+      }
+
+      auto place_and_issue = [&]() {
+        int v = 0;
+        if (lane < P) {
+          const float X = S.X[lane], Y = S.Y[lane], Z = S.Z[lane];
+          const float tx = S.G[0] * X + S.G[1] * Y + S.G[2] * Z + S.G[3];
+          const float ty = S.G[4] * X + S.G[5] * Y + S.G[6] * Z + S.G[7];
+          const float tz = S.G[8] * X + S.G[9] * Y + S.G[10] * Z + S.G[11];
+          const float mx = (tx / tz) * fx + cx, my = (ty / tz) * fy + cy;
+          v = (mx >= 0) & (my >= 0) & (mx <= swo) & (my <= sho);
+          int x0 = 0, y0 = 0;
+          float4 w = make_float4(0.f, 0.f, 0.f, 0.f);
+          if (v) kr_patch_place(mx, my, &x0, &y0, &w);
+          S.npl[lane] = w;
+          S.nx[lane] = x0;
+          S.ny[lane] = y0;
+          S.nvis[lane] = v;
+        }
+        const int nv = __popc(__ballot_sync(0xffffffffu, v));
+        if (lane == 0) S.nv = nv;
+        __syncwarp();
+        if (lane < U) {
+          const int pp = lane >> 1, half = lane & 1;
+          if (S.nvis[pp]) {
+            fence_proxy_async();
+            mbar_expect_tx(&S.win_full[lane], KR_WIN_BYTES);
+            tma_load_2d(s_win + lane * KR_SLOT_BYTES, tmN, (S.nx[pp] - 1) & ~3, S.ny[pp] - 1 + 16 * half, &S.win_full[lane]);
+          } else {
+            mbar_arrive(&S.win_full[lane]);
+          }
+        }
+      };
+
+      if (tid < P) {
+        const int i = tid;
+        const float xc = S.Xc[i], yc = S.Yc[i], zc = S.Zc[i];
+        const float mx = (xc / zc) * fx + cx, my = (yc / zc) * fy + cy;
+        const int vis = (mx >= 0) & (my >= 0) & (mx <= swo) & (my <= sho);
+        int x0 = 0, y0 = 0;
+        float4 w = make_float4(0.f, 0.f, 0.f, 0.f);
+        if (vis) {
+          kr_patch_place(mx, my, &x0, &y0, &w);
+          float c[10];
+          sd_coefs(xc, yc, zc, fx, fy, c);
+          float* ab = s_AB[i];
+          ab[0] = c[0]; ab[1] = 0.0f; ab[2] = c[2]; ab[3] = c[4]; ab[4] = c[6]; ab[5] = c[8];
+          ab[6] = 0.0f; ab[7] = c[1]; ab[8] = c[3]; ab[9] = c[5]; ab[10] = c[7]; ab[11] = c[9];
+        }
+        S.rpl[i] = w;
+        S.rx[i] = x0;
+        S.ry[i] = y0;
+        S.rvis[i] = vis;
+      }
+      fence_proxy_async();
+      slot_sync(slot);
+      if (warp == 0) {
+        if (lane < U && S.rvis[lane >> 1]) {
+          const int pp = lane >> 1, half = lane & 1;
+          unsigned char* dst = reinterpret_cast<unsigned char*>(s_sd) + (size_t)pp * KR_SD_BYTES_PER_POINT + half * 3 * KR_SLOT_BYTES;
+          const int x = (S.rx[pp] - 1) & ~3, y = S.ry[pp] - 1 + 16 * half;
+          fence_proxy_async();
+          unsigned long long* bar = &S.gat_full[pp >> 2];
+          mbar_expect_tx_only(bar, 3u * KR_WIN_BYTES);
+          tma_load_2d(dst, tmI, x, y, bar);
+          tma_load_2d(dst + KR_SLOT_BYTES, tmDx, x, y, bar);
+          tma_load_2d(dst + 2 * KR_SLOT_BYTES, tmDy, x, y, bar);
+        }
+        __syncwarp();
+        if (lane < 2) mbar_arrive(&S.gat_full[lane]);
+      }
+      if (chainA && trace) lt1 = clock64();
+      if (prod) {
+        mbar_wait(&S.gat_full[0], lvl & 1);
+        mbar_wait(&S.gat_full[1], lvl & 1);
+      }
+#pragma unroll
+      for (int s = 0; s < KT_UPP; ++s) {
+        const int u = pw + KT_NPROD * s;
+        const bool mine = prod && u < U && S.rvis[u >> 1];
+        const int pp = u >> 1, half = u & 1;
+        float gx[16], gy[16];
+        if (mine) {
+          const float* win = s_sd + (size_t)pp * (KR_SD_BYTES_PER_POINT / 4) + half * 3 * (KR_SLOT_BYTES / 4) +
+                             ((S.rx[pp] - 1) & 3);
+          const float4 w = S.rpl[pp];
+          kr_sample16(win, lane, w, refv[s]);
+          kr_sample16(win + KR_SLOT_BYTES / 4, lane, w, gx);
+          kr_sample16(win + 2 * (KR_SLOT_BYTES / 4), lane, w, gy);
+        }
+        slot_sync(slot);
+        if (mine) {
+          float ab[12];
+#pragma unroll
+          for (int k = 0; k < 12; ++k) ab[k] = s_AB[pp][k];
+          float* dst = s_sd + (size_t)pp * 6 * 1024 + half * 16 * 32 + perm;
+#pragma unroll
+          for (int r = 0; r < 16; ++r) {
+            float sd[6];
+            kx_sd(gx[r], gy[r], ab, sd);
+#pragma unroll
+            for (int k = 0; k < 6; ++k) dst[k * 1024 + r * 32] = sd[k];
+          }
+        }
+      }
+      if (warp < 2 && sl != op.lv_f && !S.rvis[0]) {
+        const int c = lane & 7;
+        const int k = chainA ? (lane >> 3) : 4 + ((lane >> 3) & 1);
+        float4* sdk = reinterpret_cast<float4*>(s_sd) + k * 256 + c;
+#pragma unroll
+        for (int q = 0; q < 4; ++q) {
+          unsigned v[32];
+          tm_ld32(tl + 32 * q, v);
+          tm_wait_ld();
+#pragma unroll
+          for (int r = 0; r < 8; ++r)
+            sdk[(q >> 1) * 128 + (8 * (q & 1) + r) * 8] =
+                make_float4(__uint_as_float(v[4 * r]), __uint_as_float(v[4 * r + 1]), __uint_as_float(v[4 * r + 2]),
+                            __uint_as_float(v[4 * r + 3]));
+        }
+      }
+      slot_sync(slot);
+
+      if (chainA && trace) lt2 = clock64();
+      if (warp < 3) {
+        const int c = lane & 7, g = min(lane >> 3, 2);
+        auto qidx = [](int a, int b) { return a * 6 - (a * (a - 1)) / 2 + (b - a); };
+        const float4* sd4 = reinterpret_cast<const float4*>(s_sd) + c;
+        if (warp == 0) {
+          const int px = 2 * g, py = 2 * g + 1;
+          const float4* X4 = sd4 + px * 256;
+          const float4* Y4 = sd4 + py * 256;
+          float a1 = -0.0f, a2 = -0.0f, a3 = -0.0f;
+          for (int i = 0; i < P; ++i) {
+#pragma unroll 8
+            for (int r = 0; r < 32; ++r) {
+              const float4 x = X4[i * 1536 + r * 8], y = Y4[i * 1536 + r * 8];
+              a1 = a1 + x.x * x.x; a2 = a2 + x.x * y.x; a3 = a3 + y.x * y.x;
+              a1 = a1 + x.y * x.y; a2 = a2 + x.y * y.y; a3 = a3 + y.y * y.y;
+              a1 = a1 + x.z * x.z; a2 = a2 + x.z * y.z; a3 = a3 + y.z * y.z;
+              a1 = a1 + x.w * x.w; a2 = a2 + x.w * y.w; a3 = a3 + y.w * y.w;
+            }
+          }
+          const float r1 = kx_finish(a1), r2 = kx_finish(a2), r3 = kx_finish(a3);
+          if ((lane & 7) == 0 && lane < 24) {
+            S.Hsum[qidx(px, px)] = r1;
+            S.Hsum[qidx(px, py)] = r2;
+            S.Hsum[qidx(py, py)] = r3;
+          }
+        } else {
+          const int px = (g < 2 ? 0 : 2) + (warp - 1), pz = g == 0 ? 2 : 4;
+          const float4* X4 = sd4 + px * 256;
+          const float4* Z4 = sd4 + pz * 256;
+          const float4* W4 = Z4 + 256;
+          float a1 = -0.0f, a2 = -0.0f;
+          for (int i = 0; i < P; ++i) {
+#pragma unroll 8
+            for (int r = 0; r < 32; ++r) {
+              const float4 x = X4[i * 1536 + r * 8], z = Z4[i * 1536 + r * 8], w = W4[i * 1536 + r * 8];
+              a1 = a1 + x.x * z.x; a2 = a2 + x.x * w.x;
+              a1 = a1 + x.y * z.y; a2 = a2 + x.y * w.y;
+              a1 = a1 + x.z * z.z; a2 = a2 + x.z * w.z;
+              a1 = a1 + x.w * z.w; a2 = a2 + x.w * w.w;
+            }
+          }
+          const float r1 = kx_finish(a1), r2 = kx_finish(a2);
+          if ((lane & 7) == 0 && lane < 24) {
+            S.Hsum[qidx(px, pz)] = r1;
+            S.Hsum[qidx(px, pz + 1)] = r2;
+          }
+        }
+      }
+      if (warp < 2) {
+        const int c = lane & 7;
+        const int k = chainA ? (lane >> 3) : 4 + ((lane >> 3) & 1);
+        const float4* sdk = reinterpret_cast<const float4*>(s_sd) + k * 256 + c;
+#pragma unroll 1
+        for (int u = 0; u < U; ++u) {
+          const float4* sd4 = sdk + (u >> 1) * 1536 + (u & 1) * 128;
+#pragma unroll
+          for (int h = 0; h < 2; ++h) {
+            float4 sv[8];
+#pragma unroll
+            for (int r = 0; r < 8; ++r) sv[r] = sd4[(8 * h + r) * 8];
+            tm_st32(tl + 64 * u + 32 * h, sv);
+          }
+        }
+        tm_wait_st();
+      }
+      fence_proxy_async();
+      slot_sync(slot);
+      if (chainA && trace) lt3 = clock64();
+      if (chainA) {
+        lu6_factor_warp(S.Hsum, S.f);
+
+        normdp_init = 1e-10f;
+        const int cont0 = (0 < op.maxiter) & ((1e-10f / 1e-10f) > op.normdp_ratio);
+        if (lane == 0) {
+          S.it = 0;
+          S.cont[gi & 1u] = cont0;
+        }
+        if (cont0) place_and_issue();
+        if (trace) lt4 = clock64();
+      }
+      slot_sync(slot);
+
+      int it = 0;
+      while (S.cont[gi & 1u]) {
+        if (prod) {
+#pragma unroll
+          for (int s = 0; s < KT_UPP; ++s) {
+            const int u = pw + KT_NPROD * s;
+            if (u < U) {
+              const int pp = u >> 1;
+              float* win = reinterpret_cast<float*>(s_win + u * KR_SLOT_BYTES);
+              const int vis = S.nvis[pp];
+              if (vis) {
+                const float4 w = S.npl[pp];
+                const float* wsh = win + ((S.nx[pp] - 1) & 3);
+                mbar_wait_backoff(&S.win_full[u], (upar >> u) & 1u);
+                float a[17], b[17];
+#pragma unroll
+                for (int r = 0; r < 17; ++r) {
+                  a[r] = wsh[r * KR_WROW + lane + 1];
+                  b[r] = wsh[r * KR_WROW + lane];
+                }
+                __syncwarp();
+#pragma unroll
+                for (int r = 0; r < 16; ++r) {
+                  const float pn = ((w.x * a[r + 1] + w.y * b[r + 1]) + w.z * a[r]) + w.w * b[r];
+                  win[r * KR_WROW + perm] = refv[s][r] - pn;
+                }
+              } else {
+#pragma unroll
+                for (int r = 0; r < 16; ++r) win[r * KR_WROW + perm] = 0.0f;
+              }
+              __syncwarp();
+              if (lane == 0) st_release_s(&S.pd_flag[u], gi + 1u);
+            }
+          }
+        } else {
+          const int c = lane & 7;
+          float acc = -0.0f;
+          long long t_c0 = 0, t_c1 = 0, w0 = 0;
+          const unsigned want = gi + 1u;
+          unsigned s0[16], s1[16];
+          float4 d0[4], d1[4];
+          if (chainA && trace) t_c0 = clock64();
+          tm_ld16(tl, s0);
+          while (ld_acquire_s(&S.pd_flag[0]) != want) {}
+          if (chainA && trace) w0 = clock64() - t_c0;
+          {
+            const float4* pd4 = reinterpret_cast<const float4*>(s_win) + c;
+#pragma unroll
+            for (int r = 0; r < 4; ++r) d0[r] = kt_lds128(pd4 + r * (KR_WROW / 4));
+          }
+          tm_wait_ld();
+#pragma unroll 1
+          for (int u = 0; u < U; ++u) {
+            const float4* pd4 = reinterpret_cast<const float4*>(s_win + u * KR_SLOT_BYTES) + c;
+#pragma unroll
+            for (int q = 0; q < 4; ++q) {
+              unsigned(&sc)[16] = (q & 1) ? s1 : s0;
+              unsigned(&sn)[16] = (q & 1) ? s0 : s1;
+              float4(&dc)[4] = (q & 1) ? d1 : d0;
+              float4(&dn)[4] = (q & 1) ? d0 : d1;
+              if (q < 3) {
+                tm_ld16(tl + 64 * u + 16 * (q + 1), sn);
+#pragma unroll
+                for (int r = 0; r < 4; ++r) dn[r] = kt_lds128(pd4 + (4 * (q + 1) + r) * (KR_WROW / 4));
+              } else if (u + 1 < U) {
+                tm_ld16(tl + 64 * (u + 1), sn);
+                while (ld_acquire_s(&S.pd_flag[u + 1]) != want) {}
+                const float4* pn4 = reinterpret_cast<const float4*>(s_win + (u + 1) * KR_SLOT_BYTES) + c;
+#pragma unroll
+                for (int r = 0; r < 4; ++r) dn[r] = kt_lds128(pn4 + r * (KR_WROW / 4));
+              }
+              kt_add4(sc, dc, acc);
+              tm_wait_ld();
+            }
+          }
+          const float res = kx_finish(acc);
+          if (!chainA) {
+            if ((lane & 7) == 0 && lane < 16) S.sum[4 + (lane >> 3)] = res;
+            __syncwarp();
+            if (lane == 0) st_release_s(&S.b_flag, want);
+          } else {
+            if ((lane & 7) == 0) S.sum[lane >> 3] = res;
+            float lu[36];
+#pragma unroll
+            for (int j = 0; j < 36; ++j) lu[j] = S.f.lu[j];
+            const int lu_rank = S.f.rank;
+            while (ld_acquire_s(&S.b_flag) != want) {}
+            if (trace) t_c1 = clock64();
+            __syncwarp();
+            float sumsd[6], dp[6], pr[6], Gr[12];
+#pragma unroll
+            for (int j = 0; j < 6; ++j) sumsd[j] = S.sum[j];
+            lu6_solve_regs(lu, lu_rank, S.f.pr, S.f.qd, S.sum, S.dp);
+            __syncwarp();
+            const long long t_s1 = trace ? clock64() : 0;
+#pragma unroll
+            for (int j = 0; j < 6; ++j) { dp[j] = S.dp[j]; pr[j] = S.p[j] + dp[j]; }
+            Gr[3] = Gr[7] = Gr[11] = 0.0f;
+            se3_exp_f(Gr, pr);
+            const long long t_s2 = trace ? clock64() : 0;
+            const float normdp = ((fabsf(dp[0]) + fabsf(dp[2])) + (fabsf(dp[1]) + fabsf(dp[3]))) +
+                                 (fabsf(dp[4]) + fabsf(dp[5]));
+            __syncwarp();
+            if (lane < 6) S.p[lane] = pr[lane];
+            if (lane < 12) S.G[lane] = Gr[lane];
+            if (it == 0) normdp_init = normdp;
+            const int cont = (it + 1 < op.maxiter) & ((normdp / normdp_init) > op.normdp_ratio);
+            nvsum += S.nv;
+            if (lane == 0) {
+              if (trace && trace_n < prm.trace_cap) {
+                float* rec = prm.trace + ((int64_t)t * prm.trace_cap + trace_n) * ICT_TRACE_FLOATS;
+                rec[0] = (float)sl;
+                rec[1] = (float)it;
+                for (int j = 0; j < 6; ++j) { rec[2 + j] = sumsd[j]; rec[8 + j] = dp[j]; }
+                rec[14] = normdp;
+                rec[15] = (float)S.nv;
+                for (int j = 16; j < ICT_TRACE_FLOATS; ++j) rec[j] = 0.0f;
+                rec[16] = (float)w0;
+                rec[17] = (float)(t_s1 - t_c1);
+                if (it != 0) rec[18] = (float)(t_s2 - t_s1);
+                if (it == 0) {
+                  rec[19] = (float)(lt1 - lt0);
+                  rec[20] = (float)(lt2 - lt1);
+                  rec[21] = (float)(lt3 - lt2);
+                  rec[18] = (float)(lt4 - lt3);
+                }
+                rec[22] = (float)(clock64() - t_c1);
+                rec[23] = (float)(t_c1 - t_c0);
+              }
+              S.it = it + 1;
+              S.cont[(gi + 1u) & 1u] = cont;
+            }
+            if (trace && trace_n < prm.trace_cap) ++trace_n;
+            __syncwarp();
+            if (cont) place_and_issue();
+          }
+        }
+        slot_sync(slot);
+        ++it;
+        ++gi;
+        upar ^= umask;
+      }
+      if (chainA && lane == 0 && prm.iters) prm.iters[(int64_t)t * (op.lv_f - op.lv_l + 1) + (op.lv_f - sl)] = S.it;
+    }
+
+    if (chainA && lane == 0) {
+      getpose_se3(S.p, S.G, donorm, prm.norm + 4 * (int64_t)t, prm.norm[4 * (int64_t)t + 3], prm.p_out + 6 * (int64_t)t);
+      if (prm.npixres) prm.npixres[t] = (long long)nvsum * 1024;
+      if (trace)
+        for (int k = trace_n; k < prm.trace_cap; ++k) {
+          float* rec = prm.trace + ((int64_t)t * prm.trace_cap + k) * ICT_TRACE_FLOATS;
+          for (int j = 0; j < ICT_TRACE_FLOATS; ++j) rec[j] = 0.0f;
+          rec[0] = -1.0f;
+        }
+    }
+  }
+
+  tm_fence_before();
+  __syncthreads();
+  tm_fence_after();
+  if (threadIdx.x < 32)
+    asm volatile("tcgen05.dealloc.cta_group::1.sync.aligned.b32 %0, %1;" ::"r"(s_taddr), "n"(KT_TMEM_COLS) : "memory");
+}
+
+static int kt_pcap(const ict_optparam& op, int max_pts) { return max_pts < op.maxpttrack ? max_pts : op.maxpttrack; }
+
+static cudaError_t kt_prepare(int dev, int* n_sm) {
+  static int state[64] = {};
+  static int sms[64] = {};
+  int& st = state[dev & 63];
+  if (st == 0) {
+    int optin = 0, occ = 0;
+    cudaError_t e = cudaDeviceGetAttribute(&optin, cudaDevAttrMaxSharedMemoryPerBlockOptin, dev);
+    if (e == cudaSuccess) e = cudaDeviceGetAttribute(&sms[dev & 63], cudaDevAttrMultiProcessorCount, dev);
+    if (e != cudaSuccess) return e;
+    cudaFuncAttributes fa;
+    e = cudaFuncGetAttributes(&fa, k_track_rt);
+    if (e != cudaSuccess) return e;
+    st = 2;
+    if (KT_SMEM_BYTES + fa.sharedSizeBytes <= (size_t)optin) {
+      e = cudaFuncSetAttribute(k_track_rt, cudaFuncAttributeMaxDynamicSharedMemorySize, (int)KT_SMEM_BYTES);
+      if (e == cudaSuccess) e = cudaFuncSetAttribute(k_track_rt, cudaFuncAttributePreferredSharedMemoryCarveout, 100);
+      if (e == cudaSuccess) e = cudaOccupancyMaxActiveBlocksPerMultiprocessor(&occ, k_track_rt, KT_THREADS, KT_SMEM_BYTES);
+      if (e != cudaSuccess) return e;
+      if (occ == 1) st = 1;
+    }
+  }
+  *n_sm = sms[dev & 63];
+  return st == 1 ? cudaSuccess : cudaErrorInvalidConfiguration;
+}
+
+bool krt_supported(const ict_optparam& op, int max_pts, int tma_ok) {
+  const int P = kt_pcap(op, max_pts);
+  if (!(tma_ok && op.psz == 32 && !op.dopatchnorm && P >= 1 && P <= KT_PMAX)) return false;
+  int dev = 0, n_sm = 0;
+  if (cudaGetDevice(&dev) != cudaSuccess || kt_prepare(dev, &n_sm) != cudaSuccess) {
+    cudaGetLastError();
+    return false;
+  }
+  return true;
+}
+
+cudaError_t launch_track_rt(const TrackParams& prm, int max_pts, cudaStream_t stream) {
+  if (prm.T <= 0) return cudaSuccess;
+  if (!prm.rt_ticket || !krt_supported(prm.op, max_pts, prm.tma_ok)) return cudaErrorInvalidConfiguration;
+  int dev = 0, n_sm = 0;
+  cudaError_t e = cudaGetDevice(&dev);
+  if (e == cudaSuccess) e = kt_prepare(dev, &n_sm);
+  if (e == cudaSuccess) e = cudaMemsetAsync(prm.rt_ticket, 0, sizeof(unsigned), stream);
+  if (e != cudaSuccess) return e;
+  const int half = (prm.T + 1) / 2;
+  k_track_rt<<<half < n_sm ? half : n_sm, KT_THREADS, KT_SMEM_BYTES, stream>>>(prm);
+  count_launch_external();
+  return cudaGetLastError();
+}
+
+}
diff --git a/invcompcamtrack_b200/csrc/ict_kernels.cu b/invcompcamtrack_b200/csrc/ict_kernels.cu
--- a/invcompcamtrack_b200/csrc/ict_kernels.cu
+++ b/invcompcamtrack_b200/csrc/ict_kernels.cu
@@ -1179,6 +1179,9 @@
   }
   if ((mode & 2) && !prm.force_general && !ict_knob("ICT_EXACT_V1") && kx8_supported(prm.op, max_pts))
     return launch_track_x8(prm, max_pts, stream);
+  if (mode == 2 && !prm.force_general && !prm.knob_no_k2r && !prm.knob_no_k2t && !ict_knob("ICT_EXACT_V1") &&
+      prm.rt_ticket && krt_supported(prm.op, max_pts, prm.tma_ok))
+    return launch_track_rt(prm, max_pts, stream);
   if (mode == 2 && !prm.force_general && !prm.knob_no_k2r && !ict_knob("ICT_EXACT_V1") &&
       kr_supported(prm.op, max_pts, prm.tma_ok))
     return launch_track_r(prm, max_pts, stream);
diff --git a/invcompcamtrack_b200/csrc/ict_kernels.cuh b/invcompcamtrack_b200/csrc/ict_kernels.cuh
--- a/invcompcamtrack_b200/csrc/ict_kernels.cuh
+++ b/invcompcamtrack_b200/csrc/ict_kernels.cuh
@@ -49,8 +49,10 @@
   int state_load;
   unsigned robust;
   int knob_no_k2r;
+  int knob_no_k2t;
   int knob_seq_launches;
   int tma_ok;
+  unsigned* rt_ticket;
   int r_pcap;
   int sum_mode;
   int eigen_packet;
@@ -84,6 +86,9 @@
 size_t kr_smem_bytes(const ict_optparam& op, int max_pts);
 cudaError_t launch_track_r(const TrackParams& prm, int max_pts, cudaStream_t stream);
 
+bool krt_supported(const ict_optparam& op, int max_pts, int tma_ok);
+cudaError_t launch_track_rt(const TrackParams& prm, int max_pts, cudaStream_t stream);
+
 bool kx8_supported(const ict_optparam& op, int max_pts);
 size_t kx8_smem_bytes(const ict_optparam& op, int max_pts);
 cudaError_t launch_track_x8(const TrackParams& prm, int max_pts, cudaStream_t stream);
```
